# JeremyWesthead/deacon-server

Measured on AMD Instinct MI355X. Metric: Mbp/s filtered (k=31,w=15 vs panhuman-1-sized index), decisions bit-exact vs CPU, higher is better.
Workload: dtype u64

## Files before the change

### deacon-server_amd/_native.py

```python
import ctypes as C
import os
import re
import subprocess

_PKG = os.path.dirname(os.path.abspath(__file__))
LIB_PATH = os.environ.get("DCN_LIB_PATH") or os.path.join(_PKG, "lib", "libdeacon_hip.so")
HEADER_PATH = os.path.join(os.path.dirname(_PKG), "include", "deacon_hip.h")

DCN_OK = 0
DCN_ERR_ARG = -1
DCN_ERR_HIP = -2
DCN_ERR_NOMEM = -3
DCN_ERR_IO = -4
DCN_ERR_FORMAT = -5
DCN_ERR_CAPACITY = -6
DCN_ERR_INTERNAL = -7
N_STATS = 6
N_STAGES = 5
STAGE_NAMES = ("pack", "plan", "scan", "distinct", "finish")
STAT_NAMES = ("total_seqs", "filtered_seqs", "total_bp", "output_bp", "filtered_bp", "output_seq_counter")


class DeaconHipError(RuntimeError):
    def __init__(self, code, message):
        super().__init__(f"deacon_hip error {code}: {message}")
        self.code = code
        self.message = message


class Params(C.Structure):
    _fields_ = [
        ("abs_threshold", C.c_uint64),
        ("rel_threshold", C.c_double),
        ("prefix_length", C.c_uint64),
        ("deplete", C.c_uint32),
        ("reserved", C.c_uint32),
    ]


class LocateParams(C.Structure):
    _fields_ = [
        ("max_gap", C.c_uint32),
        ("min_hits", C.c_uint32),
        ("member_mask", C.c_uint32),
        ("reserved", C.c_uint32),
        ("prefix_length", C.c_uint64),
    ]


class TrackParams(C.Structure):
    _fields_ = [
        ("bin_bases", C.c_uint32),
        ("member_mask", C.c_uint32),
        ("depth_cap", C.c_uint32),
        ("reserved", C.c_uint32),
        ("prefix_length", C.c_uint64),
    ]


class TrackBin(C.Structure):
    _fields_ = [
        ("n_positions", C.c_uint32),
        ("n_keys", C.c_uint32),
        ("n_observed", C.c_uint32),
        ("max_depth", C.c_uint32),
        ("sum_depth", C.c_uint64),
    ]


class PlaceParams(C.Structure):
    _fields_ = [
        ("band_bases", C.c_uint32),
        ("min_votes", C.c_uint32),
        ("prefix_length", C.c_uint64),
        ("reserved", C.c_uint32 * 2),
    ]


class Placement(C.Structure):
    _fields_ = [
        ("record", C.c_uint32),
        ("reverse", C.c_uint32),
        ("votes", C.c_uint32),
        ("n_anchors", C.c_uint32),
        ("n_positions", C.c_uint32),
        ("read_start", C.c_uint32),
        ("read_end", C.c_uint32),
        ("reserved", C.c_uint32),
        ("ref_start", C.c_uint64),
        ("ref_end", C.c_uint64),
    ]


class PlaceSplitParams(C.Structure):
    _fields_ = [
        ("band_bases", C.c_uint32),
        ("min_votes", C.c_uint32),
        ("prefix_length", C.c_uint64),
        ("max_placements", C.c_uint32),
        ("reserved", C.c_uint32 * 3),
    ]


class SplitPlacement(C.Structure):
    _fields_ = Placement._fields_ + [
        ("rank", C.c_uint32),
        ("n_placed", C.c_uint32),
        ("rival_votes", C.c_uint32),
        ("mapq", C.c_uint32),
    ]


PLACE_SPLIT_MAX = 8


class PlacePairParams(C.Structure):
    _fields_ = [
        ("band_bases", C.c_uint32),
        ("min_votes", C.c_uint32),
        ("prefix_length", C.c_uint64),
        ("max_placements", C.c_uint32),
        ("max_insert", C.c_uint32),
        ("hist_bin_bases", C.c_uint32),
        ("reserved", C.c_uint32 * 3),
    ]


class PairPlacement(C.Structure):
    _fields_ = SplitPlacement._fields_ + [
        ("flags", C.c_uint32),
        ("pair_votes", C.c_uint32),
        ("tlen", C.c_int64),
    ]


PAIR_HIST_BINS = 256


def build(force=False, jobs=6):
    csrc = os.path.join(_PKG, "csrc")
    cmd = ["make", "-C", csrc, f"-j{jobs}"]
    if force:
        cmd.append("-B")
    subprocess.check_call(cmd, stdout=subprocess.DEVNULL)
    return LIB_PATH


def declared_symbols():
    text = open(HEADER_PATH).read()
    text = re.sub(r"/\*.*?\*/", "", text, flags=re.S)
    return sorted(set(re.findall(r"\b(dcn_[a-z0-9_]+)\s*\(", text)))


_u8p, _u32p, _u64p = C.POINTER(C.c_uint8), C.POINTER(C.c_uint32), C.POINTER(C.c_uint64)
_vp = C.c_void_p

_SIGNATURES = {
    "dcn_abi_version": (C.c_int, [_u32p, _u32p]),
    "dcn_version": (C.c_char_p, []),
    "dcn_last_error": (C.c_char_p, []),
    "dcn_device_count": (C.c_int, [C.POINTER(C.c_int)]),
    "dcn_set_minimizer_variant": (C.c_int, [C.c_uint32, C.c_uint32, C.c_uint32]),
    "dcn_get_minimizer_variant": (C.c_int, [_u32p, _u32p, _u32p]),
    "dcn_index_from_keys": (C.c_int, [_vp, C.c_uint64, C.c_uint8, C.c_uint8, C.c_int, C.POINTER(_vp)]),
    "dcn_index_from_file": (C.c_int, [C.c_char_p, C.c_int, C.POINTER(_vp)]),
    "dcn_index_build": (C.c_int, [_vp, _vp, C.c_uint32, C.c_uint8, C.c_uint8, C.c_float, C.c_uint64, C.c_int,
                                  C.POINTER(_vp)]),
    "dcn_index_keys": (C.c_int, [_vp, _vp, C.c_uint64, _u64p]),
    "dcn_index_union": (C.c_int, [C.POINTER(_vp), C.c_uint32, C.POINTER(_vp)]),
    "dcn_index_diff": (C.c_int, [_vp, _vp, C.POINTER(_vp)]),
    "dcn_index_intersect": (C.c_int, [C.POINTER(_vp), C.c_uint32, C.POINTER(_vp)]),
    "dcn_index_write_file": (C.c_int, [_vp, C.c_char_p]),
    "dcn_index_header": (C.c_int, [_vp, _u8p, _u8p, _u64p]),
    "dcn_index_contains": (C.c_int, [_vp, _vp, C.c_uint64, _vp]),
    "dcn_index_contains_device": (C.c_int, [_vp, _vp, C.c_uint64, _vp, _vp]),
    "dcn_index_probe_ceiling": (C.c_int, [_vp, _vp, C.c_uint64, C.c_uint32, C.POINTER(C.c_double)]),
    "dcn_index_destroy": (None, [_vp]),
    "dcn_ctx_create": (C.c_int, [_vp, C.c_uint64, C.c_uint32, C.POINTER(_vp)]),
    "dcn_ctx_destroy": (None, [_vp]),
    "dcn_filter_batch": (C.c_int, [_vp, _vp, _vp, _vp, C.c_uint32, C.POINTER(Params), _vp, _vp, _vp]),
    "dcn_filter_batch_submit": (C.c_int, [_vp, _vp, _vp, _vp, C.c_uint32, C.POINTER(Params), _vp, _vp, _vp, _u64p]),
    "dcn_filter_batch_wait": (C.c_int, [_vp, C.c_uint64]),
    "dcn_filter_batch_packed": (C.c_int, [_vp, _vp, _vp, _vp, _vp, C.c_uint32, C.POINTER(Params), _vp, _vp, _vp]),
    "dcn_filter_batch_packed_submit": (C.c_int, [_vp, _vp, _vp, _vp, _vp, C.c_uint32, C.POINTER(Params), _vp, _vp, _vp,
                                                 _u64p]),
    "dcn_pack_ascii": (C.c_int, [_vp, C.c_uint64, _vp, _vp, _u32p]),
    "dcn_stats_allreduce": (C.c_int, [C.POINTER(_vp), C.c_int, _u64p]),
    "dcn_comm_available": (C.c_int, []),
    "dcn_comm_unique_id": (C.c_int, [_vp]),
    "dcn_comm_create": (C.c_int, [_vp, C.c_int, C.c_int, C.c_int, C.POINTER(_vp)]),
    "dcn_stats_allreduce_rccl": (C.c_int, [_vp, C.POINTER(_vp), C.c_int, _u64p]),
    "dcn_comm_destroy": (None, [_vp]),
    "dcn_index_device": (C.c_int, [_vp, C.POINTER(C.c_int)]),
    "dcn_index_memory": (C.c_int, [_vp, C.POINTER(C.c_uint64)]),
    "dcn_index_clone": (C.c_int, [_vp, C.c_int, C.POINTER(_vp)]),
    "dcn_filter_batch_device": (C.c_int, [_vp, _vp, _vp, _vp, C.c_uint32, C.c_uint64, C.c_uint32,
                                          C.POINTER(Params), _vp, _vp, _vp]),
    "dcn_ctx_synchronize": (C.c_int, [_vp]),
    "dcn_ctx_reserve_records": (C.c_int, [_vp, C.c_uint64]),
    "dcn_ctx_stream": (_vp, [_vp]),
    "dcn_host_alloc": (C.c_int, [C.c_uint64, C.POINTER(_vp)]),
    "dcn_host_free": (None, [_vp]),
    "dcn_minimizer_hashes_batch": (C.c_int, [_vp, _vp, _vp, C.c_uint32, C.c_uint64, _vp, _vp, _vp, C.c_uint64]),
    "dcn_should_keep_hashes": (C.c_int, [_vp, _vp, _vp, C.c_uint32, C.POINTER(Params), _vp, _vp, _vp]),
    "dcn_ctx_stats": (C.c_int, [_vp, _u64p]),
    "dcn_ctx_reset_stats": (C.c_int, [_vp]),
    "dcn_ctx_set_profiling": (C.c_int, [_vp, C.c_int]),
    "dcn_ctx_profile": (C.c_int, [_vp, C.POINTER(C.c_double), _u64p]),
    "dcn_index_set_create": (C.c_int, [C.POINTER(_vp), C.c_uint32, C.POINTER(_vp)]),
    "dcn_index_set_destroy": (None, [_vp]),
    "dcn_index_set_info": (C.c_int, [_vp, _u32p, _u8p, _u8p, _u64p, _u64p]),
    "dcn_classify_batch": (C.c_int, [_vp, _vp, _vp, _vp, _vp, C.c_uint32, C.POINTER(Params), _vp, _vp, _vp]),
    "dcn_classify_batch_device": (C.c_int, [_vp, _vp, _vp, _vp, _vp, C.c_uint32, C.c_uint64, C.c_uint32,
                                            C.POINTER(Params), _vp, _vp, _vp]),
    "dcn_index_set_coverage_enable": (C.c_int, [_vp, C.c_int]),
    "dcn_index_set_coverage_reset": (C.c_int, [_vp]),
    "dcn_index_set_coverage": (C.c_int, [_vp, _vp, _vp]),
    "dcn_index_set_coverage_keys": (C.c_int, [_vp, C.c_uint32, _vp, C.c_uint64, _u64p]),
    "dcn_index_set_depth_enable": (C.c_int, [_vp, C.c_int]),
    "dcn_index_set_depth_reset": (C.c_int, [_vp]),
    "dcn_index_set_depth_stats": (C.c_int, [_vp, _vp, _vp, _vp]),
    "dcn_index_set_depth_hist": (C.c_int, [_vp, C.c_uint32, C.c_uint32, _vp]),
    "dcn_index_set_depth_keys": (C.c_int, [_vp, C.c_uint32, _vp, _vp, C.c_uint64, _u64p]),
    "dcn_index_set_select": (C.c_int, [_vp, C.c_uint32, C.c_uint32, C.c_uint32, C.c_uint32, C.c_uint32, _u64p,
                                       C.POINTER(_vp)]),
    "dcn_index_set_overlap": (C.c_int, [_vp, _vp, _vp, _vp]),
    "dcn_index_builder_create": (C.c_int, [C.c_uint8, C.c_uint8, C.c_float, C.c_uint64, C.c_int, C.POINTER(_vp)]),
    "dcn_index_builder_add": (C.c_int, [_vp, _vp, _vp, C.c_uint32]),
    "dcn_index_builder_info": (C.c_int, [_vp, _u64p, _u64p, _u64p, _u64p]),
    "dcn_index_builder_hist": (C.c_int, [_vp, C.c_uint32, _vp]),
    "dcn_index_builder_counts": (C.c_int, [_vp, _vp, _vp, C.c_uint64, _u64p]),
    "dcn_index_builder_finish": (C.c_int, [_vp, C.c_uint32, C.c_uint32, _u64p, C.POINTER(_vp)]),
    "dcn_index_builder_destroy": (None, [_vp]),
    "dcn_locate_batch": (C.c_int, [_vp, _vp, _vp, _vp, C.c_uint32, _vp, _vp, _vp, C.c_uint64]),
    "dcn_depth_track_batch": (C.c_int, [_vp, _vp, _vp, _vp, C.c_uint32, _vp, _vp, _vp, C.c_uint64]),
    "dcn_anchor_map_create": (C.c_int, [_vp, C.POINTER(_vp)]),
    "dcn_anchor_map_add": (C.c_int, [_vp, _vp, _vp, _vp, C.c_uint32, _u32p]),
    "dcn_anchor_map_info": (C.c_int, [_vp, _u32p, _u64p, _u64p, _u64p]),
    "dcn_anchor_map_anchors": (C.c_int, [_vp, _vp, _vp, _vp, C.c_uint64, _u64p]),
    "dcn_place_batch": (C.c_int, [_vp, _vp, _vp, _vp, C.c_uint32, _vp, _vp]),
    "dcn_place_split_batch": (C.c_int, [_vp, _vp, _vp, _vp, C.c_uint32, _vp, _vp, _vp, C.c_uint64, _vp]),
    "dcn_place_pair_batch": (C.c_int, [_vp, _vp, _vp, _vp, C.c_uint32, _vp, _vp, _vp]),
}

_lib = None
ABI = (1, 11)


def lib():
    global _lib
    if _lib is not None:
        return _lib
    if not os.path.exists(LIB_PATH):
        raise ImportError(
            f"{LIB_PATH} is missing: build it with __graft_entry__.build() "
            "(make -C deacon-server_amd/csrc). There is no CPU fallback.")
    L = C.CDLL(LIB_PATH)
    for name, (res, args) in _SIGNATURES.items():
        f = getattr(L, name)
        f.restype = res
        f.argtypes = args
    major, minor = C.c_uint32(), C.c_uint32()
    if L.dcn_abi_version(C.byref(major), C.byref(minor)) != 0 or (major.value, minor.value >= ABI[1]) != (ABI[0], True):
        raise ImportError(f"{LIB_PATH} has ABI {major.value}.{minor.value}; these bindings were written against {ABI[0]}.{ABI[1]} "
                          "(include/deacon_hip.h: DCN_ABI_MAJOR / DCN_ABI_MINOR)")
    _lib = L
    return L


def check(rc):
    if rc != DCN_OK:
        msg = lib().dcn_last_error()
        raise DeaconHipError(rc, msg.decode("utf-8", "replace") if msg else "")
    return rc
```

### deacon-server_amd/csrc/ctx.hip

```cpp
#include "dcn_ctx.h"
#include "dcn_host_pool.h"

#include <atomic>
#include <cstdlib>
#include <cstring>
#include <mutex>
#include <new>

using dcn_host::HostPool;

namespace dcn_impl {

int alloc_records(dcn_ctx *c, uint64_t n_records) {
    n_records = (n_records + 63) / 64 * 64;
    if (n_records > (1ull << 29)) return dcn_fail(DCN_ERR_CAPACITY, "more than 2^29 hit records in global sets per batch: use smaller batches");
    if (c->d_set_slots) hipFree(c->d_set_slots);
    c->d_set_slots = nullptr;
    c->rec_capacity = 0;
    DCN_TRY(dev_alloc(&c->d_set_slots, 4 * n_records + 64, "set_slots"));
    c->rec_capacity = n_records;
    return DCN_OK;
}

void free_slot_buffers(dcn_slot &sl) {
    if (sl.owns_buffers) {
        void *dev[] = {sl.d_ascii, sl.d_packed, sl.d_invmask, sl.d_offsets, sl.d_unit_id, sl.d_keep, sl.d_hits, sl.d_total};
        for (void *p : dev)
            if (p) hipFree(p);
    }
    if (sl.d_report) hipFree(sl.d_report);
    if (sl.d_off32) hipFree(sl.d_off32);
    if (sl.d_mask_pairs) hipFree(sl.d_mask_pairs);
    void *host[] = {sl.h_keep, sl.h_hits, sl.h_total, sl.h_report, sl.h_off32, sl.h_mask_pairs};
    for (void *p : host)
        if (p) hipHostFree(p);
    if (sl.done) hipEventDestroy(sl.done);
    for (hipEvent_t e : sl.ev_h2d) hipEventDestroy(e);
    for (hipEvent_t e : sl.ev_comp) hipEventDestroy(e);
    sl = dcn_slot();
}

static void free_ctx(dcn_ctx *c) {
    if (!c) return;
    hipSetDevice(c->device);
    if (c->stream) hipStreamSynchronize(c->stream);
    if (c->copy_stream) hipStreamSynchronize(c->copy_stream);
    if (c->d2h_stream) hipStreamSynchronize(c->d2h_stream);
    if (c->pack_stream) {
        hipStreamSynchronize(c->pack_stream);
        hipStreamDestroy(c->pack_stream);
    }
    for (int i = 0; i < 2; ++i) {
        if (c->pack_done[i]) hipEventDestroy(c->pack_done[i]);
        if (c->buf_free[i]) hipEventDestroy(c->buf_free[i]);
    }
    if (c->plan_done) hipEventDestroy(c->plan_done);
    if (c->d_packed_b) hipFree(c->d_packed_b);
    if (c->d_invmask_b) hipFree(c->d_invmask_b);
    if (c->d_pack_status) hipFree(c->d_pack_status);
    for (auto &sl : c->slots) free_slot_buffers(sl);
    void *dev[] = {c->d_ascii, c->d_offsets, c->d_unit_id, c->d_packed, c->d_invmask,
                   c->d_read_tiles, c->d_read_tile_first, c->d_unit_first_read, c->d_unit_tile_first, c->d_unit_tile_count, c->d_tiles,
                   c->d_keep, c->d_unit_state, c->d_hits, c->d_total, c->d_unit_scratch, c->d_caps,
                   c->d_set_off, c->d_tile_hits, c->d_pending, c->d_big, c->d_rec_hash, c->d_set_slots, c->d_status, c->d_report, c->d_dump_hash,
                   c->d_dump_pos, c->d_dump_count, c->d_dump_valid, c->d_tile_read_pos,
                   c->d_cls_big, c->d_cls_n_big, c->d_cls_match, c->d_cls_hits, c->d_cls_total,
                   c->d_loc_bits, c->d_loc_labels, c->d_loc_counts, c->d_loc_big, c->d_loc_n_big, c->d_loc_block_sums,
                   c->d_loc_seg_offsets, c->d_loc_segs, c->d_trk_bin_offsets, c->d_trk_piece_offsets, c->d_trk_bins,
                   c->d_plc_words, c->d_plc_abits, c->d_plc_big, c->d_plc_n_big, c->d_plc_out,
                   c->d_pls_rbits, c->d_pls_n_rounds, c->d_pls_read_counts, c->d_pls_counts, c->d_pls_block_sums,
                   c->d_pls_offsets, c->d_pls_rounds, c->d_pls_out, c->d_ppr_out, c->d_ppr_hist};
    for (void *p : dev)
        if (p && !((char *)p >= c->d_slab && (char *)p < c->d_slab + c->slab_bytes)) hipFree(p);
    if (c->d_slab) hipFree(c->d_slab);
    for (int i = 0; i < dcn_ctx::N_STAGE; ++i) {
        if (c->h_stage[i]) hipHostFree(c->h_stage[i]);
        if (c->stage_free[i]) hipEventDestroy(c->stage_free[i]);
    }
    for (int i = 0; i < dcn_ctx::N_EV; ++i) {
        if (c->ev_h2d[i]) hipEventDestroy(c->ev_h2d[i]);
        if (c->ev_comp[i]) hipEventDestroy(c->ev_comp[i]);
    }
    if (c->h_report) hipHostFree(c->h_report);
    for (int i = 0; i < dcn_ctx::PROF_RING; ++i)
        for (int j = 0; j <= DCN_N_STAGES; ++j)
            if (c->prof_ev[i][j]) hipEventDestroy(c->prof_ev[i][j]);
    if (c->copy_done) hipEventDestroy(c->copy_done);
    if (c->stream) hipStreamDestroy(c->stream);
    if (c->copy_stream) hipStreamDestroy(c->copy_stream);
    if (c->d2h_stream) hipStreamDestroy(c->d2h_stream);
    delete c;
}

static int prof_harvest(dcn_ctx *c, int only_slot = -1) {
    for (int i = 0; i < dcn_ctx::PROF_RING; ++i) {
        if (!c->prof_used[i] || (only_slot >= 0 && i != only_slot)) continue;
        const int first = c->prof_scan_only[i] ? DCN_STAGE_SCAN : 0, last = c->prof_scan_only[i] ? DCN_STAGE_SCAN : DCN_N_STAGES - 1;
        DCN_HIP(hipEventSynchronize(c->prof_ev[i][last + 1]));
        for (int j = first; j <= last; ++j) {
            float ms = 0.f;
            DCN_HIP(hipEventElapsedTime(&ms, c->prof_ev[i][j], c->prof_ev[i][j + 1]));
            c->prof_ms[j] += ms;
        }
        c->prof_batches++;
        c->prof_used[i] = false;
    }
    return DCN_OK;
}

int prof_begin(dcn_ctx *c, int *slot) {
    *slot = -1;
    if (!c->profiling) return DCN_OK;
    int i = c->prof_next;
    c->prof_next = (i + 1) % dcn_ctx::PROF_RING;
    if (c->prof_used[i]) DCN_TRY(prof_harvest(c, i));
    for (int j = 0; j <= DCN_N_STAGES; ++j)
        if (!c->prof_ev[i][j]) DCN_HIP(hipEventCreate(&c->prof_ev[i][j]));
    c->prof_scan_only[i] = c->profiling == 2;
    if (c->profiling == 1) DCN_HIP(hipEventRecord(c->prof_ev[i][0], c->stream));
    *slot = i;
    return DCN_OK;
}

int check_params(const dcn_params *p) {
    if (!p) return dcn_fail(DCN_ERR_ARG, "params is NULL");
    if (p->reserved != 0) return dcn_fail(DCN_ERR_ARG, "params.reserved must be 0");
    if (p->deplete > 1) return dcn_fail(DCN_ERR_ARG, "params.deplete must be 0 or 1");
    return DCN_OK;
}

static bool ensure_pack_ahead(dcn_ctx *c) {
    if (c->pack_ahead_state != 0) return c->pack_ahead_state > 0;
    c->pack_ahead_state = -1;
    if (!getenv("DCN_PACK_AHEAD") || getenv("DCN_NO_PACK_AHEAD")) return false;
    int prio_low = 0, prio_high = 0;
    (void)hipDeviceGetStreamPriorityRange(&prio_low, &prio_high);
    bool ok = hipStreamCreateWithPriority(&c->pack_stream, hipStreamNonBlocking, prio_high) == hipSuccess;
    ok = ok && hipEventCreateWithFlags(&c->plan_done, hipEventDisableTiming) == hipSuccess;
    for (int i = 0; ok && i < 2; ++i)
        ok = hipEventCreateWithFlags(&c->pack_done[i], hipEventDisableTiming) == hipSuccess &&
             hipEventCreateWithFlags(&c->buf_free[i], hipEventDisableTiming) == hipSuccess;
    ok = ok && hipMalloc((void **)&c->d_packed_b, packed_words(c->max_bases) * sizeof(uint32_t)) == hipSuccess &&
         hipMalloc((void **)&c->d_invmask_b, mask_words(c->max_bases) * sizeof(uint32_t)) == hipSuccess &&
         hipMalloc((void **)&c->d_pack_status, 2 * sizeof(dcn_status)) == hipSuccess;
    if (ok) {
        ok = hipMemset(c->d_packed_b, 0, packed_words(c->max_bases) * sizeof(uint32_t)) == hipSuccess &&
             hipMemset(c->d_invmask_b, 0, mask_words(c->max_bases) * sizeof(uint32_t)) == hipSuccess &&
             hipDeviceSynchronize() == hipSuccess;
    }
    if (!ok) {
        (void)hipGetLastError();
        if (c->d_packed_b) hipFree(c->d_packed_b);
        if (c->d_invmask_b) hipFree(c->d_invmask_b);
        if (c->d_pack_status) hipFree(c->d_pack_status);
        c->d_packed_b = c->d_invmask_b = nullptr;
        c->d_pack_status = nullptr;
        return false;
    }
    c->pack_ahead_state = 1;
    return true;
}

static dcn_scan_args scan_args(const dcn_ctx *c, const dcn_index *index, uint32_t *packed, uint32_t *invmask, uint64_t stream_bases);

int enqueue_batch(dcn_ctx *c, const BatchView &v, const dcn_params *params, bool pack_ahead) {
    hipStream_t st = c->stream;
    const dcn_index *idx = c->index;
    if (c->scratch_dirty) DCN_HIP(hipMemsetAsync(c->d_unit_scratch, 0, (uint64_t)c->max_reads * 4 * sizeof(uint32_t), st));
    c->scratch_dirty = true;
    DCN_HIP(hipMemsetAsync(c->d_status, 0, sizeof(dcn_status), st));

    int prof_slot = -1;
    DCN_TRY(prof_begin(c, &prof_slot));
    uint32_t *packed = v.d_packed + DCN_FRONT_PAD, *invmask = v.d_invmask + DCN_FRONT_PAD;
    int ahead_buf = -1;
    const uint32_t *newline_flag = nullptr;
    if (v.d_ascii && pack_ahead && c->profiling != 1 && ensure_pack_ahead(c)) {
        ahead_buf = c->pack_buf;
        c->pack_buf ^= 1;
        if (ahead_buf == 1) {
            packed = c->d_packed_b + DCN_FRONT_PAD;
            invmask = c->d_invmask_b + DCN_FRONT_PAD;
        }
        dcn_status *ps = c->d_pack_status + ahead_buf;
        DCN_HIP(hipStreamWaitEvent(c->pack_stream, c->buf_free[ahead_buf], 0));
        if (!getenv("DCN_PACK_AHEAD_EARLY")) DCN_HIP(hipStreamWaitEvent(c->pack_stream, c->plan_done, 0));
        DCN_HIP(hipMemsetAsync(ps, 0, sizeof(dcn_status), c->pack_stream));
        DCN_TRY(dcn_launch_pack_beside(v.d_ascii, v.b0, v.b1, packed, invmask, ps, c->pack_stream));
        DCN_HIP(hipEventRecord(c->pack_done[ahead_buf], c->pack_stream));
        DCN_HIP(hipStreamWaitEvent(st, c->pack_done[ahead_buf], 0));
        newline_flag = &ps->any_newline;
    } else if (v.d_ascii) {
        DCN_TRY(dcn_launch_pack(v.d_ascii, v.b0, v.b1, packed, invmask, c->d_status, st));
    }
    DCN_PROF_MARK(DCN_STAGE_PACK);

    const uint32_t n_reads = v.n_reads, n_units = v.n_units;
    dcn_plan_args pa = plan_args(c, idx, v.d_ascii, v.d_offsets, v.d_unit_id, n_reads, n_units, params->prefix_length);
    pa.unit_base = v.unit_base;
    pa.unit_state = c->d_unit_state;
    pa.unit_scratch = c->d_unit_scratch;
    pa.scratch_stride = c->max_reads;
    pa.newline_flag = newline_flag;
    pa.stream_bases = v.stream_bases;
    pa.check_offsets = 1;
    pa.max_tiles = c->max_tiles;
    DCN_TRY(dcn_launch_plan(pa, st));
    if (pack_ahead && c->pack_ahead_state == 1) DCN_HIP(hipEventRecord(c->plan_done, st));
    DCN_PROF_MARK(DCN_STAGE_PLAN);

    const UnitScratch us = unit_scratch(c);
    dcn_scan_args sa = scan_args(c, idx, packed, invmask, v.stream_bases);
    sa.unit_tile_first = c->d_unit_tile_first;
    sa.unit_tile_count = c->d_unit_tile_count;
    sa.abs_threshold = params->abs_threshold;
    sa.rel_threshold = params->rel_threshold;
    sa.deplete = params->deplete;
    sa.early_out_max_items = 0;
    static const bool no_early_out = getenv("DCN_NO_EARLY_OUT") != nullptr, no_early_out_pairs = getenv("DCN_NO_EARLY_OUT_PAIRS") != nullptr;
    if (!v.d_hits && !v.d_total && params->abs_threshold >= 1 && params->abs_threshold <= 4 && !no_early_out) {
        uint32_t lo = 0, hi = 65535;
        while (lo < hi) {
            uint32_t mid = (lo + hi + 1) / 2;
            if (dcn_required_hits(params->abs_threshold, params->rel_threshold, mid) == params->abs_threshold) lo = mid;
            else hi = mid - 1;
        }
        sa.early_out_max_items = lo;
        sa.early_out_pairs = no_early_out_pairs ? 0u : 1u;
    }
    sa.keep = v.d_keep;
    sa.hits = v.d_hits;
    sa.total = v.d_total;
    sa.unit_state = c->d_unit_state;
    sa.g_total = us.g_total;
    sa.g_hitcnt = us.g_hitcnt;
    sa.g_zero = us.g_zero;
    sa.rec_hash = c->d_rec_hash;
    sa.rec_shift = c->rec_shift;
    sa.tile_windows = c->tile_windows;
    sa.tile_hits = c->d_tile_hits;
    sa.pending = c->d_pending;
    sa.status = c->d_status;
    DCN_TRY(dcn_launch_scan(sa, tile_bound(c, n_reads, v.b1 - v.b0), false, st));
    DCN_PROF_MARK(DCN_STAGE_SCAN);

    const bool decisions_only = !v.d_hits && !v.d_total && !getenv("DCN_NO_EARLY_OUT");
    const dcn_distinct_args da = distinct_args(c, n_units, params, c->d_rec_hash, c->rec_shift, decisions_only ? us.g_total : nullptr);
    DCN_TRY(dcn_launch_distinct(da, st));
    DCN_PROF_MARK(DCN_STAGE_DISTINCT);

    const dcn_finish_args fa = finish_args(c, n_units, params, v.d_unit_id ? c->d_unit_first_read : nullptr, v.d_offsets, v.d_keep,
                                           v.d_hits, v.d_total, v.d_report);
    DCN_TRY(dcn_launch_finish(fa, st));
    c->scratch_dirty = false;
    if (pack_ahead && c->pack_ahead_state == 1) DCN_HIP(hipEventRecord(c->buf_free[ahead_buf >= 0 ? ahead_buf : 0], st));
    DCN_PROF_MARK(DCN_STAGE_FINISH);
    if (prof_slot >= 0) c->prof_used[prof_slot] = true;
    return DCN_OK;
}

int grow_run_slots(dcn_ctx *c) {
    if (c->rec_shift == 0) return DCN_OK;
    const bool in_slab = c->d_rec_hash && (char *)c->d_rec_hash >= c->d_slab && (char *)c->d_rec_hash < c->d_slab + c->slab_bytes;
    if (c->d_rec_hash && !in_slab) hipFree(c->d_rec_hash);
    c->d_rec_hash = nullptr;
    const uint32_t old_shift = c->rec_shift;
    c->rec_shift = 0;
    int rc = dev_alloc(&c->d_rec_hash, c->max_bases + 128, "rec_hash (one slot per window)");
    if (rc != DCN_OK) {
        c->rec_shift = old_shift;
        int rc2 = dev_alloc(&c->d_rec_hash, (c->max_bases >> old_shift) + 256, "rec_hash");
        return rc2 != DCN_OK ? rc2 : rc;
    }
    static std::atomic<bool> said{false};
    if (!said.exchange(true) && getenv("DCN_QUIET") == nullptr)
        std::fprintf(stderr, "deacon-hip: a unit's hits outgrew its run of the record array; this context now keeps one slot per window "
                             "(%.2f GB instead of %.2f GB of device memory)\n", (c->max_bases + 128) * 8e-9,
                     ((c->max_bases >> old_shift) + 256) * 8e-9);
    return DCN_OK;
}

int overflow_error(const dcn_ctx *c, uint64_t need) {
    return dcn_fail(DCN_ERR_CAPACITY, "hit-record scratch overflow: need " + std::to_string(need) +
                                          " records, have " + std::to_string(c->rec_capacity) +
                                          " (dcn_ctx_reserve_records)");
}

int sync_and_check(dcn_ctx *c, uint64_t *needed_records) {
    DCN_HIP(hipStreamSynchronize(c->stream));
    if (needed_records) *needed_records = 0;
    if (c->profiling) DCN_TRY(prof_harvest(c));
    if (!c->batch_pending) return DCN_OK;
    c->batch_pending = false;
    DCN_HIP(hipMemcpy(c->h_report, c->d_report, sizeof(dcn_batch_report), hipMemcpyDeviceToHost));
    if (c->h_report->bounds) {
        DCN_HIP(hipMemsetAsync(c->d_report, 0, offsetof(dcn_batch_report, stats), c->stream));
        return dcn_fail(DCN_ERR_INTERNAL, "scan kernel: index out of range in phase B (DCN_DEBUG_BOUNDS build)");
    }
    if (c->h_report->bad_offsets) {
        DCN_HIP(hipMemsetAsync(c->d_report, 0, offsetof(dcn_batch_report, stats), c->stream));
        return dcn_fail(DCN_ERR_ARG, "d_offsets of a batch since the last synchronize were not non-decreasing within [0, n_bases] when the "
                                     "device read them (were they written, and ordered before the context's stream, when "
                                     "dcn_filter_batch_device was called?): the outputs and counters of those batches are undefined");
    }
    if (c->h_report->overflow) {
        const uint64_t need = c->h_report->need;
        const bool runs = (c->h_report->overflow & 2u) != 0, sets = (c->h_report->overflow & 1u) != 0;
        DCN_HIP(hipMemsetAsync(c->d_report, 0, offsetof(dcn_batch_report, stats), c->stream));
        if (runs) DCN_TRY(grow_run_slots(c));
        if (needed_records) *needed_records = sets ? need : 0;
        if (!sets)
            return dcn_fail(DCN_ERR_CAPACITY, "a unit had more hits in one wave than its run of the record array holds; the context "
                                              "now keeps one slot per window: enqueue the batches since the last synchronize again");
        return overflow_error(c, need);
    }
    return DCN_OK;
}

bool is_pinned_host(const void *p) {
    if (!p) return false;
    hipPointerAttribute_t attr;
    if (hipPointerGetAttributes(&attr, p) != hipSuccess) {
        (void)hipGetLastError();
        return false;
    }
    return attr.type == hipMemoryTypeHost;
}

template <typename Fill>
static int staged_h2d_fill(dcn_ctx *c, void *d_dst, uint64_t bytes, uint64_t piece_align, Fill fill) {
    uint8_t *dst = (uint8_t *)d_dst;
    const uint64_t piece = c->stage_bytes / piece_align * piece_align;
    for (uint64_t off = 0; off < bytes; off += piece) {
        const int which = c->stage_next;
        c->stage_next = (which + 1) % dcn_ctx::N_STAGE;
        const uint64_t m = std::min<uint64_t>(piece, bytes - off);
        DCN_HIP(hipEventSynchronize(c->stage_free[which]));
        fill(c->h_stage[which], off, m);
        DCN_HIP(hipMemcpyAsync(dst + off, c->h_stage[which], m, hipMemcpyHostToDevice, c->copy_stream));
        DCN_HIP(hipEventRecord(c->stage_free[which], c->copy_stream));
    }
    return DCN_OK;
}

int staged_h2d(dcn_ctx *c, void *d_dst, const void *h_src, uint64_t bytes, int pinned) {
    if (bytes == 0) return DCN_OK;
    if (pinned < 0) pinned = is_pinned_host(h_src) ? 1 : 0;
    if (pinned) {
        DCN_HIP(hipMemcpyAsync(d_dst, h_src, bytes, hipMemcpyHostToDevice, c->copy_stream));
        return DCN_OK;
    }
    const uint8_t *src = (const uint8_t *)h_src;
    return staged_h2d_fill(c, d_dst, bytes, 64, [&](uint8_t *stage, uint64_t first, uint64_t n) {
        HostPool::get().copy(stage, src + first, n);
    });
}


int slots_busy(const dcn_ctx *c) {
    int n = 0;
    for (const auto &sl : c->slots) n += sl.busy ? 1 : 0;
    return n;
}

static std::mutex g_ctx_devices_mu;
static int g_ctx_per_device[64] = {0};
static void note_ctx_device(int device, int delta) {
    int n_devices = 0;
    {
        std::lock_guard<std::mutex> g(g_ctx_devices_mu);
        if (device >= 0 && device < 64) g_ctx_per_device[device] += delta;
        for (int d = 0; d < 64; ++d) n_devices += g_ctx_per_device[d] > 0;
    }
    if (delta > 0) HostPool::get().ensure_devices(n_devices);
}

int check_idle(const dcn_ctx *c) {
    if (slots_busy(c) || c->batch_pending) return dcn_fail(DCN_ERR_ARG, "batches are in flight on this context: wait for them first");
    return DCN_OK;
}

int check_ctx_matches(const dcn_ctx *c, const dcn_index *other, const char *noun) {
    const dcn_index *ix = c->index;
    const std::string n = noun;
    if (ix->k != other->k || ix->w != other->w)
        return dcn_fail(DCN_ERR_ARG, "the context's index (k=" + std::to_string((int)ix->k) + ", w=" + std::to_string((int)ix->w) +
                                         ") and " + n + " (k=" + std::to_string((int)other->k) + ", w=" + std::to_string((int)other->w) +
                                         ") differ");
    if (ix->device != other->device) return dcn_fail(DCN_ERR_ARG, "the context and " + n + " live on different devices");
    if (ix->variant != other->variant)
        return dcn_fail(DCN_ERR_ARG, "the context's index and " + n + " were created under different minimizer rules");
    return check_idle(c);
}

int check_device_batch(const dcn_ctx *c, uint32_t n_reads, uint64_t n_bases, uint32_t n_units, const uint32_t *d_unit_id) {
    if (n_reads > c->max_reads) return dcn_fail(DCN_ERR_CAPACITY, "n_reads exceeds the context's max_batch_reads");
    if (n_bases > c->max_bases) return dcn_fail(DCN_ERR_CAPACITY, "n_bases exceeds the context's max_batch_bases");
    if (n_units == 0 || n_units > n_reads || (!d_unit_id && n_units != n_reads))
        return dcn_fail(DCN_ERR_ARG, "n_units inconsistent with n_reads / d_unit_id");
    return DCN_OK;
}

int check_offsets_walk(const uint64_t *offsets, uint32_t n, const char *noun, const char *too_long) {
    if (offsets[0] != 0) return dcn_fail(DCN_ERR_ARG, std::string(noun) + "[0] must be 0");
    for (uint32_t r = 0; r < n; ++r) {
        if (offsets[r + 1] < offsets[r]) return dcn_fail(DCN_ERR_ARG, std::string(noun) + " must be non-decreasing");
        if (offsets[r + 1] - offsets[r] > 0xFFFFFFF0ull) return dcn_fail(DCN_ERR_ARG, too_long);
    }
    return DCN_OK;
}

int validate_host_batch(const dcn_ctx *c, const uint64_t *offsets, uint32_t n_reads) {
    if (n_reads > c->max_reads) return dcn_fail(DCN_ERR_CAPACITY, "n_reads exceeds the context's max_batch_reads");
    DCN_TRY(check_idle(c));
    DCN_TRY(check_offsets_walk(offsets, n_reads, "offsets", "read longer than 2^32 bases"));
    if (offsets[n_reads] > c->max_bases) return dcn_fail(DCN_ERR_CAPACITY, "batch exceeds the context's max_batch_bases");
    return DCN_OK;
}

int ensure_dump_buffers(dcn_ctx *c) {
    if (c->d_dump_hash) return DCN_OK;
    DCN_TRY(dev_alloc(&c->d_dump_hash, c->max_bases + 2, "dump_hash"));
    DCN_TRY(dev_alloc(&c->d_dump_pos, c->max_bases + 2, "dump_pos"));
    DCN_TRY(dev_alloc(&c->d_dump_valid, c->max_bases + 2, "dump_valid"));
    DCN_TRY(dev_alloc(&c->d_dump_count, c->max_tiles, "dump_count"));
    return DCN_OK;
}

int ensure_position_bitmap(dcn_ctx *c) {
    if (c->d_loc_bits) return DCN_OK;
    return dev_alloc(&c->d_loc_bits, (c->max_bases + 31) / 32 + 1, "position bitmap");
}

int ensure_position_words(dcn_ctx *c) {
    if (c->d_loc_labels) return DCN_OK;
    return dev_alloc(&c->d_loc_labels, c->max_bases + 2, "position words");
}

UnitScratch unit_scratch(const dcn_ctx *c) {
    uint32_t *const s = c->d_unit_scratch;
    const uint64_t n = c->max_reads;
    return {s, s + n, s + 2 * n, s + 3 * n};
}

int stage_done(dcn_ctx *c) {
    DCN_HIP(hipEventRecord(c->copy_done, c->copy_stream));
    DCN_HIP(hipStreamWaitEvent(c->stream, c->copy_done, 0));
    return DCN_OK;
}

int stage_batch(dcn_ctx *c, const uint8_t *bases, uint64_t n_bases, const uint64_t *offsets, uint32_t n_reads,
                const uint32_t *unit_id_or_null) {
    DCN_TRY(staged_h2d(c, c->d_ascii, bases, n_bases));
    DCN_TRY(staged_h2d(c, c->d_offsets, offsets, (uint64_t)(n_reads + 1) * sizeof(uint64_t)));
    if (unit_id_or_null) DCN_TRY(staged_h2d(c, c->d_unit_id, unit_id_or_null, (uint64_t)n_reads * sizeof(uint32_t)));
    return stage_done(c);
}

dcn_plan_args plan_args(const dcn_ctx *c, const dcn_index *index, const uint8_t *d_ascii, const uint64_t *d_offsets,
                        const uint32_t *d_unit_id, uint32_t n_reads, uint32_t n_units, uint64_t prefix_length) {
    dcn_plan_args pa = {};
    pa.ascii = d_ascii;
    pa.offsets = d_offsets;
    pa.unit_id = d_unit_id;
    pa.n_reads = n_reads;
    pa.n_units = n_units;
    pa.k = index->k;
    pa.w = index->w;
    pa.prefix_length = prefix_length;
    pa.tile_windows = c->tile_windows;
    pa.unit_first_read = c->d_unit_first_read;
    pa.unit_tile_first = c->d_unit_tile_first;
    pa.unit_tile_count = c->d_unit_tile_count;
    pa.tile_cursor = &c->d_status->n_tiles;
    pa.tiles = c->d_tiles;
    pa.status = c->d_status;
    return pa;
}

static dcn_scan_args scan_args(const dcn_ctx *c, const dcn_index *index, uint32_t *packed, uint32_t *invmask, uint64_t stream_bases) {
    dcn_scan_args sa;
    memset(&sa, 0, sizeof(sa));
    sa.packed = packed;
    sa.invmask = invmask;
    sa.tiles = c->d_tiles;
    sa.n_tiles = &c->d_status->n_tiles;
    sa.table = index->view();
    sa.k = index->k;
    sa.variant = index->variant;
    sa.w = index->w;
    sa.stream_bases = stream_bases;
    sa.status = c->d_status;
    return sa;
}

dcn_scan_args dump_scan_args(const dcn_ctx *c, const dcn_index *index, uint64_t n_bases) {
    dcn_scan_args sa = scan_args(c, index, c->d_packed + DCN_FRONT_PAD, c->d_invmask + DCN_FRONT_PAD, n_bases);
    sa.dump_hash = c->d_dump_hash;
    sa.dump_pos = c->d_dump_pos;
    sa.dump_valid = c->d_dump_valid;
    sa.dump_count = c->d_dump_count;
    return sa;
}

uint32_t tile_bound(const dcn_ctx *c, uint32_t n_reads, uint64_t n_bases) {
    return (uint32_t)std::min<uint64_t>((uint64_t)n_reads + n_bases / c->tile_windows + 1, c->max_tiles);
}

dcn_dump_view dump_view(const dcn_ctx *c, uint32_t max_tiles, uint64_t n_bases) {
    dcn_dump_view v = {};
    v.tiles = c->d_tiles;
    v.n_tiles = &c->d_status->n_tiles;
    v.hash = c->d_dump_hash;
    v.valid = c->d_dump_valid;
    v.pos = c->d_dump_pos;
    v.count = c->d_dump_count;
    v.max_tiles = max_tiles;
    v.n_bases = n_bases;
    return v;
}

int dump_front_end(dcn_ctx *c, const dcn_index *index, const uint8_t *d_ascii, const uint64_t *d_offsets,
                   const uint32_t *d_unit_id, uint32_t n_reads, uint32_t n_units, uint64_t n_bases, uint64_t prefix_length,
                   bool plan_checks_offsets, int *prof_slot_out, dcn_dump_view *view) {
    hipStream_t st = c->stream;
    int prof_slot = -1;
    DCN_TRY(prof_begin(c, &prof_slot));
    *prof_slot_out = prof_slot;
    DCN_TRY(dcn_launch_pack(d_ascii, 0, n_bases, c->d_packed + DCN_FRONT_PAD, c->d_invmask + DCN_FRONT_PAD, c->d_status, st));
    DCN_PROF_MARK(DCN_STAGE_PACK);
    dcn_plan_args pa = plan_args(c, index, d_ascii, d_offsets, d_unit_id, n_reads, n_units, prefix_length);
    pa.read_tiles = c->d_read_tiles;
    pa.read_tile_first = c->d_read_tile_first;
    if (plan_checks_offsets) {
        pa.stream_bases = n_bases;
        pa.check_offsets = 1;
        pa.max_tiles = c->max_tiles;
    }
    DCN_TRY(dcn_launch_plan(pa, st));
    DCN_PROF_MARK(DCN_STAGE_PLAN);
    dcn_scan_args sa = dump_scan_args(c, index, n_bases);
    sa.dump_abs = 1;
    const uint32_t max_tiles = tile_bound(c, n_reads, n_bases);
    DCN_TRY(dcn_launch_scan(sa, max_tiles, true, st));
    DCN_PROF_MARK(DCN_STAGE_SCAN);
    *view = dump_view(c, max_tiles, n_bases);
    return DCN_OK;
}

int record_run_end(dcn_ctx *c, int prof_slot) {
    if (prof_slot >= 0) c->prof_used[prof_slot] = true;
    if (c->pack_ahead_state == 1) {
        DCN_HIP(hipEventRecord(c->plan_done, c->stream));
        for (int i = 0; i < 2; ++i) DCN_HIP(hipEventRecord(c->buf_free[i], c->stream));
    }
    return DCN_OK;
}

int finish_run(dcn_ctx *c, int prof_slot) {
    DCN_TRY(record_run_end(c, prof_slot));
    return sync_and_check(c, nullptr);
}

dcn_distinct_args distinct_args(const dcn_ctx *c, uint32_t n_units, const dcn_params *params, const uint64_t *rec_hash,
                                uint32_t rec_shift, uint32_t *g_total_or_null) {
    const UnitScratch us = unit_scratch(c);
    dcn_distinct_args da = {};
    da.tiles = c->d_tiles;
    da.n_tiles = &c->d_status->n_tiles;
    da.unit_tile_first = c->d_unit_tile_first;
    da.unit_tile_count = c->d_unit_tile_count;
    da.unit_state = c->d_unit_state;
    da.tile_hits = c->d_tile_hits;
    da.pending = c->d_pending;
    da.rec_hash = rec_hash;
    da.rec_shift = rec_shift;
    da.g_hitcnt = us.g_hitcnt;
    da.g_distinct = us.g_distinct;
    da.set_off = c->d_set_off;
    da.set_slots = c->d_set_slots;
    da.set_capacity = 4 * c->rec_capacity + 64;
    da.n_units = n_units;
    da.status = c->d_status;
    da.caps = c->d_caps;
    da.big = c->d_big;
    da.g_total = g_total_or_null;
    da.abs_threshold = params->abs_threshold;
    da.rel_threshold = params->rel_threshold;
    return da;
}

dcn_finish_args finish_args(const dcn_ctx *c, uint32_t n_units, const dcn_params *params, const uint32_t *unit_first_read,
                            const uint64_t *offsets, uint8_t *keep, uint32_t *hits, uint32_t *total, dcn_batch_report *report) {
    const UnitScratch us = unit_scratch(c);
    dcn_finish_args fa = {};
    fa.n_units = n_units;
    fa.unit_first_read = unit_first_read;
    fa.offsets = offsets;
    fa.unit_state = c->d_unit_state;
    fa.g_total = us.g_total;
    fa.g_hitcnt = us.g_hitcnt;
    fa.g_distinct = us.g_distinct;
    fa.g_zero = us.g_zero;
    fa.abs_threshold = params->abs_threshold;
    fa.rel_threshold = params->rel_threshold;
    fa.deplete = params->deplete;
    fa.keep = keep;
    fa.hits = hits;
    fa.total = total;
    fa.report = report;
    fa.status = c->d_status;
    return fa;
}

}

using namespace dcn_impl;

extern "C" int dcn_ctx_create(const dcn_index *index, uint64_t max_batch_bases, uint32_t max_batch_reads,
                              dcn_ctx **out) {
    if (!out) return dcn_fail(DCN_ERR_ARG, "out is NULL");
    *out = nullptr;
    if (!index) return dcn_fail(DCN_ERR_ARG, "index is NULL");
    if (max_batch_bases == 0 || max_batch_reads == 0) return dcn_fail(DCN_ERR_ARG, "batch limits must be > 0");
    if (max_batch_reads > 0xFFFFFF00u) return dcn_fail(DCN_ERR_ARG, "max_batch_reads too large");
    dcn_ctx *c = new (std::nothrow) dcn_ctx();
    if (!c) return dcn_fail(DCN_ERR_NOMEM, "host allocation failed");
    c->index = index;
    c->device = index->device;
    c->max_bases = max_batch_bases;
    c->max_reads = max_batch_reads;
    if (const char *tw = getenv("DCN_TILE_WINDOWS")) {
        long v = strtol(tw, nullptr, 10);
        if (v >= 16 && v <= (long)DCN_MAX_TILE_WINDOWS) c->tile_windows = (uint32_t)v;
    }
    uint64_t mt = (uint64_t)max_batch_reads + max_batch_bases / c->tile_windows + 1;
    if (mt > 0xFFFFFF00ull) {
        delete c;
        return dcn_fail(DCN_ERR_ARG, "batch limits imply more than 2^32 tiles");
    }
    c->max_tiles = (uint32_t)mt;
    c->chunk_bases = 64ull << 20;
    if (const char *cb = getenv("DCN_CHUNK_BASES")) {
        long long v = atoll(cb);
        if (v >= 1024) c->chunk_bases = (uint64_t)v;
    }
    int rc = DCN_OK;
    auto fail = [&](int code) {
        free_ctx(c);
        return code;
    };
    if (hipSetDevice(c->device) != hipSuccess) return fail(dcn_fail(DCN_ERR_HIP, "hipSetDevice failed"));
    bool ok = hipStreamCreateWithFlags(&c->stream, hipStreamNonBlocking) == hipSuccess &&
              hipStreamCreateWithFlags(&c->copy_stream, hipStreamNonBlocking) == hipSuccess &&
              hipStreamCreateWithFlags(&c->d2h_stream, hipStreamNonBlocking) == hipSuccess &&
              hipEventCreateWithFlags(&c->copy_done, hipEventDisableTiming) == hipSuccess;
    for (int i = 0; ok && i < dcn_ctx::N_STAGE; ++i)
        ok = hipEventCreateWithFlags(&c->stage_free[i], hipEventDisableTiming) == hipSuccess;
    for (int i = 0; ok && i < dcn_ctx::N_EV; ++i)
        ok = hipEventCreateWithFlags(&c->ev_h2d[i], hipEventDisableTiming) == hipSuccess &&
             hipEventCreateWithFlags(&c->ev_comp[i], hipEventDisableTiming) == hipSuccess;
    if (!ok) return fail(dcn_fail(DCN_ERR_HIP, "stream/event creation failed"));
    c->rec_shift = 2;
    if (index->w <= 7) c->rec_shift = 0;
    if (const char *rs = getenv("DCN_REC_SHIFT")) c->rec_shift = (uint32_t)std::min(3, std::max(0, atoi(rs)));
    uint64_t MR = max_batch_reads;
    const bool slab = getenv("DCN_CTX_SLAB") != nullptr;
    uint64_t slab_off = 0;
    for (int pass = slab ? 0 : 1; pass < 2; ++pass) {
        if (slab && pass == 1) {
            c->slab_bytes = slab_off;
            if (hipMalloc((void **)&c->d_slab, c->slab_bytes) != hipSuccess) {
                c->d_slab = nullptr;
                c->slab_bytes = 0;
                return fail(dcn_fail(DCN_ERR_NOMEM, "hipMalloc of the context slab failed"));
            }
            slab_off = 0;
        }
#define A(ptr, count, what)                                                                                   \
    if (slab) {                                                                                               \
        if (pass == 1) c->ptr = reinterpret_cast<decltype(c->ptr)>(c->d_slab + slab_off);                     \
        slab_off += (std::max<uint64_t>((count), 1) * sizeof(*c->ptr) + (2u << 20) - 1) / (2u << 20) * (2u << 20); \
    } else if ((rc = dev_alloc(&c->ptr, (count), what)) != DCN_OK)                                            \
        return fail(rc)
    A(d_ascii, max_batch_bases + 64, "ascii");
    A(d_offsets, MR + 1, "offsets");
    A(d_unit_id, MR, "unit_id");
    A(d_packed, packed_words(max_batch_bases), "packed");
    A(d_invmask, mask_words(max_batch_bases), "invmask");
    A(d_read_tiles, MR, "read_tiles");
    A(d_read_tile_first, MR + 1, "read_tile_first");
    A(d_unit_first_read, MR + 1, "unit_first_read");
    A(d_unit_tile_first, MR + 1, "unit_tile_first");
    A(d_unit_tile_count, MR + 1, "unit_tile_count");
    A(d_tiles, mt, "tiles");
    A(d_keep, MR, "keep");
    A(d_unit_state, MR, "unit_state");
    A(d_hits, MR, "hits");
    A(d_total, MR, "total");
    A(d_unit_scratch, MR * 4, "unit_scratch");
    A(d_caps, MR, "caps");
    A(d_set_off, MR + 1, "set_off");
    A(d_tile_hits, mt, "tile_hits");
    A(d_pending, MR, "pending");
    A(d_big, MR + mt / 64 + 1, "big");
    A(d_rec_hash, (max_batch_bases >> c->rec_shift) + 256, "rec_hash");
    A(d_status, 1, "status");
    A(d_report, 1, "report");
#undef A
    }
    uint64_t recs = std::min<uint64_t>(std::max<uint64_t>(max_batch_bases / 16, 1u << 16), 1ull << 29);
    if (const char *rc_env = getenv("DCN_RECORD_CAPACITY")) recs = std::min<uint64_t>(std::max<uint64_t>(strtoull(rc_env, nullptr, 10), 64), 1ull << 29);
    if ((rc = alloc_records(c, recs)) != DCN_OK) return fail(rc);
    c->stage_bytes = std::min<uint64_t>(std::max<uint64_t>(max_batch_bases + 64, 4096), 32ull << 20);
    if (const char *sb = getenv("DCN_STAGE_BYTES"))
        c->stage_bytes = std::min<uint64_t>(std::max<uint64_t>(strtoull(sb, nullptr, 10), 4096), 32ull << 20);
    for (int i = 0; i < dcn_ctx::N_STAGE; ++i)
        if (hipHostMalloc((void **)&c->h_stage[i], c->stage_bytes, hipHostMallocDefault) != hipSuccess)
            return fail(dcn_fail(DCN_ERR_NOMEM, "pinned staging allocation failed"));
    if (hipHostMalloc((void **)&c->h_report, sizeof(dcn_batch_report), hipHostMallocDefault) != hipSuccess)
        return fail(dcn_fail(DCN_ERR_NOMEM, "pinned status allocation failed"));
    if (hipMemset(c->d_packed, 0, packed_words(max_batch_bases) * sizeof(uint32_t)) != hipSuccess ||
        hipMemset(c->d_invmask, 0, mask_words(max_batch_bases) * sizeof(uint32_t)) != hipSuccess ||
        hipMemset(c->d_status, 0, sizeof(dcn_status)) != hipSuccess ||
        hipMemset(c->d_unit_scratch, 0, (uint64_t)max_batch_reads * 4 * sizeof(uint32_t)) != hipSuccess ||
        hipMemset(c->d_report, 0, sizeof(dcn_batch_report)) != hipSuccess ||
        hipDeviceSynchronize() != hipSuccess)
        return fail(dcn_fail(DCN_ERR_HIP, "hipMemset failed"));
    note_ctx_device(c->device, +1);
    *out = c;
    return DCN_OK;
}

extern "C" void dcn_ctx_destroy(dcn_ctx *ctx) {
    if (ctx) note_ctx_device(ctx->device, -1);
    free_ctx(ctx);
}

extern "C" void *dcn_ctx_stream(dcn_ctx *ctx) { return ctx ? (void *)ctx->stream : nullptr; }

extern "C" int dcn_ctx_reserve_records(dcn_ctx *ctx, uint64_t n_records) {
    if (!ctx) return dcn_fail(DCN_ERR_ARG, "ctx is NULL");
    if (slots_busy(ctx)) return dcn_fail(DCN_ERR_ARG, "host batches are in flight: wait for them first");
    DCN_HIP(hipSetDevice(ctx->device));
    DCN_HIP(hipStreamSynchronize(ctx->stream));
    if (n_records <= ctx->rec_capacity) return DCN_OK;
    return alloc_records(ctx, n_records);
}

extern "C" int dcn_ctx_synchronize(dcn_ctx *ctx) {
    if (!ctx) return dcn_fail(DCN_ERR_ARG, "ctx is NULL");
    DCN_HIP(hipSetDevice(ctx->device));
    return sync_and_check(ctx, nullptr);
}

extern "C" int dcn_filter_batch_device(dcn_ctx *ctx, const uint8_t *d_bases, const uint64_t *d_offsets,
                                       const uint32_t *d_unit_id, uint32_t n_reads, uint64_t n_bases,
                                       uint32_t n_units, const dcn_params *params, uint8_t *d_keep, uint32_t *d_hits,
                                       uint32_t *d_total) {
    if (!ctx) return dcn_fail(DCN_ERR_ARG, "ctx is NULL");
    DCN_TRY(check_params(params));
    if (n_reads == 0) return DCN_OK;
    if (!d_bases || !d_offsets || !d_keep) return dcn_fail(DCN_ERR_ARG, "d_bases/d_offsets/d_keep is NULL");
    DCN_TRY(check_device_batch(ctx, n_reads, n_bases, n_units, d_unit_id));
    if (ctx->slots[0].busy) return dcn_fail(DCN_ERR_ARG, "a host batch is in flight on this context: wait for it first");
    DCN_HIP(hipSetDevice(ctx->device));
    BatchView v;
    v.d_ascii = d_bases;
    v.d_packed = ctx->d_packed;
    v.d_invmask = ctx->d_invmask;
    v.d_offsets = d_offsets;
    v.d_unit_id = d_unit_id;
    v.n_reads = n_reads;
    v.n_units = n_units;
    v.b0 = 0;
    v.b1 = n_bases;
    v.stream_bases = n_bases;
    v.d_keep = d_keep;
    v.d_hits = d_hits;
    v.d_total = d_total;
    v.d_report = ctx->d_report;
    DCN_TRY(enqueue_batch(ctx, v, params, true));
    ctx->batch_pending = true;
    return DCN_OK;
}

extern "C" int dcn_ctx_set_profiling(dcn_ctx *ctx, int enable) {
    if (!ctx) return dcn_fail(DCN_ERR_ARG, "ctx is NULL");
    DCN_HIP(hipSetDevice(ctx->device));
    DCN_HIP(hipStreamSynchronize(ctx->stream));
    for (int i = 0; i < dcn_ctx::PROF_RING; ++i) ctx->prof_used[i] = false;
    for (int j = 0; j < DCN_N_STAGES; ++j) ctx->prof_ms[j] = 0.0;
    ctx->prof_batches = 0;
    ctx->profiling = enable == 2 ? 2 : (enable != 0 ? 1 : 0);
    return DCN_OK;
}

extern "C" int dcn_ctx_profile(dcn_ctx *ctx, double stage_ms[DCN_N_STAGES], uint64_t *n_batches) {
    if (!ctx || !stage_ms) return dcn_fail(DCN_ERR_ARG, "ctx/stage_ms is NULL");
    if (ctx->profiling) {
        DCN_HIP(hipSetDevice(ctx->device));
        DCN_TRY(prof_harvest(ctx));
    }
    for (int j = 0; j < DCN_N_STAGES; ++j) stage_ms[j] = ctx->prof_ms[j];
    if (n_batches) *n_batches = ctx->prof_batches;
    return DCN_OK;
}

extern "C" int dcn_ctx_stats(dcn_ctx *ctx, uint64_t counters[DCN_N_STATS]) {
    if (!ctx || !counters) return dcn_fail(DCN_ERR_ARG, "ctx/counters is NULL");
    DCN_HIP(hipSetDevice(ctx->device));
    DCN_HIP(hipStreamSynchronize(ctx->stream));
    DCN_HIP(hipMemcpy(ctx->h_report, ctx->d_report, sizeof(dcn_batch_report), hipMemcpyDeviceToHost));
    for (int i = 0; i < DCN_N_STATS; ++i) counters[i] = ctx->h_report->stats[i] + ctx->host_stats[i];
    return DCN_OK;
}

extern "C" int dcn_ctx_reset_stats(dcn_ctx *ctx) {
    if (!ctx) return dcn_fail(DCN_ERR_ARG, "ctx is NULL");
    DCN_HIP(hipSetDevice(ctx->device));
    DCN_HIP(hipStreamSynchronize(ctx->stream));
    DCN_HIP(hipMemsetAsync(ctx->d_report->stats, 0, sizeof(unsigned long long) * DCN_N_STATS, ctx->stream));
    DCN_HIP(hipStreamSynchronize(ctx->stream));
    for (int i = 0; i < DCN_N_STATS; ++i) ctx->host_stats[i] = 0;
    return DCN_OK;
}

extern "C" int dcn_stats_allreduce(dcn_ctx *const *ctxs, int n_ctx, uint64_t counters[DCN_N_STATS]) {
    if (!counters || (n_ctx > 0 && !ctxs) || n_ctx < 0) return dcn_fail(DCN_ERR_ARG, "ctxs/counters is NULL");
    for (int i = 0; i < DCN_N_STATS; ++i) counters[i] = 0;
    for (int j = 0; j < n_ctx; ++j) {
        uint64_t one[DCN_N_STATS];
        DCN_TRY(dcn_ctx_stats(ctxs[j], one));
        for (int i = 0; i < DCN_N_STATS; ++i) counters[i] += one[i];
    }
    return DCN_OK;
}
```

### deacon-server_amd/csrc/dcn_ctx.h

```cpp
#pragma once

#include "dcn_dump_sweep.h"
#include "dcn_internal.h"
#include "dcn_plan.h"

#include <algorithm>
#include <functional>
#include <vector>

struct dcn_split_round;

struct dcn_mask_range {
    uint64_t g0 = 0, g1 = 0, pairs_off = 0;
    uint32_t n = 0;
};

struct dcn_chunk {
    uint32_t r0 = 0, r1 = 0, u0 = 0, u1 = 0;
    uint64_t b0 = 0, b1 = 0;
    uint64_t max_len = 0;
    std::vector<dcn_mask_range> mask_ranges;
};

struct dcn_slot {
    bool allocated = false, busy = false, owns_buffers = false;
    uint64_t ticket = 0;
    uint8_t *d_ascii = nullptr;
    uint32_t *d_packed = nullptr, *d_invmask = nullptr;
    uint64_t *d_offsets = nullptr;
    uint32_t *d_off32 = nullptr, *h_off32 = nullptr;
    bool off32 = false;
    bool lean = false;
    uint2 *d_mask_pairs = nullptr, *h_mask_pairs = nullptr;
    uint64_t mask_pairs_cap = 0, mask_pairs_used = 0;
    uint32_t *d_unit_id = nullptr;
    uint8_t *d_keep = nullptr;
    uint32_t *d_hits = nullptr, *d_total = nullptr;
    dcn_batch_report *d_report = nullptr;
    uint8_t *h_keep = nullptr;
    uint32_t *h_hits = nullptr, *h_total = nullptr;
    dcn_batch_report *h_report = nullptr;
    hipEvent_t done = nullptr;
    std::vector<hipEvent_t> ev_h2d, ev_comp;
    dcn_params params = {};
    bool device_pack = false;
    bool has_units = false, counts = false;
    uint32_t n_reads = 0, n_units = 0;
    uint64_t n_bases = 0;
    uint8_t *u_keep = nullptr;
    uint32_t *u_hits = nullptr, *u_total = nullptr;
    bool keep_direct = false, hits_direct = false, total_direct = false;
    std::vector<dcn_chunk> chunks;
};

struct dcn_ctx {
    const dcn_index *index = nullptr;
    int device = 0;
    hipStream_t stream = nullptr, copy_stream = nullptr, d2h_stream = nullptr;
    hipStream_t pack_stream = nullptr;
    uint32_t *d_packed_b = nullptr, *d_invmask_b = nullptr;
    dcn_status *d_pack_status = nullptr;
    hipEvent_t pack_done[2] = {}, buf_free[2] = {}, plan_done = nullptr;
    int pack_buf = 0, pack_ahead_state = 0;
    static constexpr int N_STAGE = 3, N_EV = 8, N_SLOTS = 2;
    hipEvent_t copy_done = nullptr, stage_free[N_STAGE] = {};
    hipEvent_t ev_h2d[N_EV] = {}, ev_comp[N_EV] = {};
    int ev_next = 0, stage_next = 0;
    uint64_t max_bases = 0;
    uint32_t max_reads = 0;
    uint32_t tile_windows = 256;
    uint32_t max_tiles = 0;
    uint64_t chunk_bases = 0;
    uint8_t *d_ascii = nullptr;
    uint64_t *d_offsets = nullptr;
    uint32_t *d_unit_id = nullptr;
    uint32_t *d_packed = nullptr, *d_invmask = nullptr;
    uint32_t *d_read_tiles = nullptr, *d_read_tile_first = nullptr;
    uint32_t *d_unit_first_read = nullptr, *d_unit_tile_first = nullptr, *d_unit_tile_count = nullptr;
    dcn_tile *d_tiles = nullptr;
    uint8_t *d_keep = nullptr, *d_unit_state = nullptr;
    uint32_t *d_hits = nullptr, *d_total = nullptr;
    uint32_t *d_unit_scratch = nullptr;
    bool scratch_dirty = false;
    uint32_t *d_caps = nullptr, *d_set_off = nullptr;
    uint64_t *d_rec_hash = nullptr;
    uint32_t rec_shift = 0;
    char *d_slab = nullptr;
    uint64_t slab_bytes = 0;
    uint32_t *d_tile_hits = nullptr, *d_pending = nullptr;
    uint2 *d_big = nullptr;
    uint64_t rec_capacity = 0;
    uint64_t *d_set_slots = nullptr;
    dcn_status *d_status = nullptr;
    dcn_batch_report *d_report = nullptr;
    dcn_batch_report *h_report = nullptr;
    uint64_t host_stats[DCN_N_STATS] = {};
    uint8_t *h_stage[N_STAGE] = {};
    uint64_t stage_bytes = 0;
    dcn_slot slots[N_SLOTS];
    uint64_t next_ticket = 1;
    uint64_t *d_dump_hash = nullptr;
    uint32_t *d_dump_pos = nullptr, *d_dump_count = nullptr, *d_tile_read_pos = nullptr;
    uint8_t *d_dump_valid = nullptr;
    uint32_t *d_cls_big = nullptr, *d_cls_n_big = nullptr;
    uint32_t *d_cls_match = nullptr, *d_cls_hits = nullptr, *d_cls_total = nullptr;
    uint32_t cls_hits_members = 0;
    uint32_t *d_loc_bits = nullptr, *d_loc_labels = nullptr;
    uint32_t *d_loc_counts = nullptr, *d_loc_big = nullptr, *d_loc_n_big = nullptr;
    unsigned long long *d_loc_block_sums = nullptr;
    uint64_t *d_loc_seg_offsets = nullptr;
    dcn_segment *d_loc_segs = nullptr;
    uint64_t loc_seg_cap = 0;
    uint64_t *d_trk_bin_offsets = nullptr, *d_trk_piece_offsets = nullptr;
    dcn_track_bin *d_trk_bins = nullptr;
    uint64_t trk_bin_cap = 0;
    uint64_t *d_plc_words = nullptr;
    uint32_t *d_plc_abits = nullptr, *d_plc_big = nullptr, *d_plc_n_big = nullptr;
    dcn_placement *d_plc_out = nullptr;
    uint32_t *d_pls_rbits = nullptr, *d_pls_n_rounds = nullptr, *d_pls_read_counts = nullptr, *d_pls_counts = nullptr;
    unsigned long long *d_pls_block_sums = nullptr;
    uint64_t *d_pls_offsets = nullptr;
    dcn_split_round *d_pls_rounds = nullptr;
    dcn_split_placement *d_pls_out = nullptr;
    uint64_t pls_round_cap = 0, pls_out_cap = 0;
    dcn_pair_placement *d_ppr_out = nullptr;
    unsigned long long *d_ppr_hist = nullptr;
    bool batch_pending = false;
    bool lean = false;
    static constexpr int PROF_RING = 64;
    int profiling = 0;
    hipEvent_t prof_ev[PROF_RING][DCN_N_STAGES + 1] = {};
    bool prof_used[PROF_RING] = {}, prof_scan_only[PROF_RING] = {};
    int prof_next = 0;
    double prof_ms[DCN_N_STAGES] = {};
    uint64_t prof_batches = 0;
};

bool dcn_host_pack_is_wide();
bool dcn_host_pack_groups(const uint8_t *ascii, uint64_t n_bases, uint64_t g0, uint64_t g1, uint32_t *packed,
                          uint32_t *mask);

#define DCN_TRY(expr)              \
    do {                           \
        int _rc = (expr);          \
        if (_rc != DCN_OK) return _rc; \
    } while (0)

#define DCN_PROF_MARK(stage)                                                                                      \
    do {                                                                                                          \
        if (prof_slot >= 0 && (c->profiling == 1 || (stage) == DCN_STAGE_PLAN || (stage) == DCN_STAGE_SCAN))      \
            DCN_HIP(hipEventRecord(c->prof_ev[prof_slot][(stage) + 1], st));                                      \
    } while (0)

#pragma GCC visibility push(hidden)
namespace dcn_impl {

template <typename T>
int dev_alloc(T **p, uint64_t count, const char *what) {
    hipError_t e = hipMalloc((void **)p, std::max<uint64_t>(count, 1) * sizeof(T));
    if (e != hipSuccess) {
        *p = nullptr;
        return dcn_fail(DCN_ERR_NOMEM, std::string("hipMalloc ") + what + ": " + hipGetErrorString(e));
    }
    return DCN_OK;
}

template <typename T>
int dev_alloc_zeroed(T **p, uint64_t count, const char *what) {
    *p = nullptr;
    T *d = nullptr;
    hipError_t e = hipMalloc((void **)&d, count * sizeof(T));
    if (e == hipSuccess) e = hipMemset(d, 0, count * sizeof(T));
    if (e == hipSuccess) e = hipDeviceSynchronize();
    if (e != hipSuccess) {
        if (d) hipFree(d);
        return dcn_hip_fail(e, what);
    }
    *p = d;
    return DCN_OK;
}

struct DevMem {
    void *p = nullptr;
    ~DevMem() {
        if (p) hipFree(p);
    }
    int alloc(uint64_t bytes, bool zero, const char *what) {
        hipError_t e = hipMalloc(&p, std::max<uint64_t>(bytes, 8));
        if (e == hipSuccess && zero) e = hipMemset(p, 0, std::max<uint64_t>(bytes, 8));
        return e == hipSuccess ? DCN_OK : dcn_hip_fail(e, what);
    }
    int clear(const char *what) {
        const hipError_t e = hipMemset(p, 0, 8);
        return e == hipSuccess ? DCN_OK : dcn_hip_fail(e, what);
    }
    int read(void *h, uint64_t bytes, const char *what) const {
        const hipError_t e = hipMemcpy(h, p, bytes, hipMemcpyDeviceToHost);
        return e == hipSuccess ? DCN_OK : dcn_hip_fail(e, what);
    }
    template <typename T>
    T *as() const {
        return (T *)p;
    }
};

inline int read_count(const DevMem &d_n, const char *what, unsigned long long *n) { return d_n.read(n, sizeof(*n), what); }

inline uint64_t packed_words(uint64_t max_bases) { return DCN_FRONT_PAD + 2 * ((max_bases + 31) / 32) + DCN_TAIL_PAD; }
inline uint64_t mask_words(uint64_t max_bases) { return DCN_FRONT_PAD + (max_bases + 31) / 32 + DCN_TAIL_PAD; }

struct BatchView {
    const uint8_t *d_ascii = nullptr;
    uint32_t *d_packed = nullptr, *d_invmask = nullptr;
    const uint64_t *d_offsets = nullptr;
    const uint32_t *d_unit_id = nullptr;
    uint32_t unit_base = 0;
    uint32_t n_reads = 0, n_units = 0;
    uint64_t b0 = 0, b1 = 0;
    uint64_t stream_bases = 0;
    uint8_t *d_keep = nullptr;
    uint32_t *d_hits = nullptr, *d_total = nullptr;
    dcn_batch_report *d_report = nullptr;
};

int same_params(const dcn_index *a, const dcn_index *b);
int check_kw(uint8_t k, uint8_t w);

constexpr uint32_t DCN_BUILD_MAX_PIECES = 1u << 16;
uint64_t build_chunk_bases();
using build_sweep_fn = std::function<int(uint64_t nb, bool continues)>;
struct build_times {
    double front_end_s = 0, staging_s = 0, growth_s = 0, finish_s = 0, finish_table_s = 0;
};
double build_now();
int build_timing_begin(dcn_ctx *c);
int build_times_print(const char *which, dcn_ctx *c, const build_times &t);
int build_run_chunks(dcn_ctx *c, const dcn_index *idx, const uint8_t *bases, const uint64_t *offsets, uint32_t n_seqs,
                     uint64_t chunk_bases, const build_sweep_fn &sweep, build_times *times = nullptr);

int check_set(const dcn_index *set);

int alloc_records(dcn_ctx *c, uint64_t n_records);
void free_slot_buffers(dcn_slot &sl);
int prof_begin(dcn_ctx *c, int *slot);
int check_params(const dcn_params *p);
int enqueue_batch(dcn_ctx *c, const BatchView &v, const dcn_params *params, bool pack_ahead = false);
int grow_run_slots(dcn_ctx *c);
int overflow_error(const dcn_ctx *c, uint64_t need);
int sync_and_check(dcn_ctx *c, uint64_t *needed_records);
bool is_pinned_host(const void *p);
int staged_h2d(dcn_ctx *c, void *d_dst, const void *h_src, uint64_t bytes, int pinned = -1);
int slots_busy(const dcn_ctx *c);

int check_idle(const dcn_ctx *c);
int check_ctx_matches(const dcn_ctx *c, const dcn_index *other, const char *noun);
int check_device_batch(const dcn_ctx *c, uint32_t n_reads, uint64_t n_bases, uint32_t n_units, const uint32_t *d_unit_id);
int check_offsets_walk(const uint64_t *offsets, uint32_t n, const char *noun, const char *too_long);
int validate_host_batch(const dcn_ctx *c, const uint64_t *offsets, uint32_t n_reads);

int ensure_dump_buffers(dcn_ctx *c);
int ensure_position_bitmap(dcn_ctx *c);
int ensure_position_words(dcn_ctx *c);
struct UnitScratch {
    uint32_t *g_total, *g_hitcnt, *g_distinct, *g_zero;
};
UnitScratch unit_scratch(const dcn_ctx *c);
int stage_batch(dcn_ctx *c, const uint8_t *bases, uint64_t n_bases, const uint64_t *offsets, uint32_t n_reads,
                const uint32_t *unit_id_or_null);
int stage_done(dcn_ctx *c);
dcn_plan_args plan_args(const dcn_ctx *c, const dcn_index *index, const uint8_t *d_ascii, const uint64_t *d_offsets,
                        const uint32_t *d_unit_id, uint32_t n_reads, uint32_t n_units, uint64_t prefix_length);
dcn_scan_args dump_scan_args(const dcn_ctx *c, const dcn_index *index, uint64_t n_bases);
uint32_t tile_bound(const dcn_ctx *c, uint32_t n_reads, uint64_t n_bases);
dcn_dump_view dump_view(const dcn_ctx *c, uint32_t max_tiles, uint64_t n_bases);

int dump_front_end(dcn_ctx *c, const dcn_index *index, const uint8_t *d_ascii, const uint64_t *d_offsets,
                   const uint32_t *d_unit_id, uint32_t n_reads, uint32_t n_units, uint64_t n_bases, uint64_t prefix_length,
                   bool plan_checks_offsets, int *prof_slot, dcn_dump_view *view);
int record_run_end(dcn_ctx *c, int prof_slot);
int finish_run(dcn_ctx *c, int prof_slot);
dcn_distinct_args distinct_args(const dcn_ctx *c, uint32_t n_units, const dcn_params *params, const uint64_t *rec_hash,
                                uint32_t rec_shift, uint32_t *g_total_or_null);
dcn_finish_args finish_args(const dcn_ctx *c, uint32_t n_units, const dcn_params *params, const uint32_t *unit_first_read,
                            const uint64_t *offsets, uint8_t *keep, uint32_t *hits, uint32_t *total, dcn_batch_report *report);

}
#pragma GCC visibility pop
```

### deacon-server_amd/csrc/dcn_internal.h

```cpp
#pragma once

#include <hip/hip_runtime.h>
#include <stdint.h>

#include <string>

#include "../../include/deacon_hip.h"

void dcn_set_error(const std::string &msg);
int dcn_fail(int code, const std::string &msg);

#define DCN_HIP(expr)                                                                              \
    do {                                                                                           \
        hipError_t _e = (expr);                                                                    \
        if (_e != hipSuccess)                                                                      \
            return dcn_fail(_e == hipErrorOutOfMemory ? DCN_ERR_NOMEM : DCN_ERR_HIP,               \
                            std::string(#expr) + ": " + hipGetErrorString(_e));                    \
    } while (0)

inline int dcn_hip_fail(hipError_t e, const char *what) {
    return dcn_fail(e == hipErrorOutOfMemory ? DCN_ERR_NOMEM : DCN_ERR_HIP, std::string(what) + ": " + hipGetErrorString(e));
}

template <typename F>
int dcn_device_tally(uint64_t count, unsigned long long *h, const char *what, F sweep) {
    unsigned long long *d = nullptr;
    hipError_t e = hipMalloc((void **)&d, count * sizeof(unsigned long long));
    if (e != hipSuccess) return dcn_hip_fail(e, what);
    int rc = DCN_OK;
    e = hipMemset(d, 0, count * sizeof(unsigned long long));
    if (e == hipSuccess) rc = sweep(d);
    if (e == hipSuccess && rc == DCN_OK) e = hipMemcpy(h, d, count * sizeof(unsigned long long), hipMemcpyDeviceToHost);
    hipFree(d);
    if (rc != DCN_OK) return rc;
    return e == hipSuccess ? DCN_OK : dcn_hip_fail(e, what);
}

void dcn_host_parallel_copy(void *dst, const void *src, size_t n);

#ifndef DCN_GROUP_SLOTS
#define DCN_GROUP_SLOTS 2
#endif
constexpr int DCN_SLOTS_PER_KEY = DCN_GROUP_SLOTS == 2 ? 4 : 2;
constexpr int DCN_SLOTS_PER_KEY_ROOMY = 2 * DCN_SLOTS_PER_KEY;
constexpr uint64_t DCN_ROOMY_MAX_GROUPS = 1ull << 31;

struct dcn_table_view {
    const uint64_t *slots;
    uint32_t group_shift;
    uint32_t group_mask;
    uint32_t has_zero;
};

constexpr uint32_t DCN_VARIANT_DEFAULT = (1u << 16) | (16u << 8) | 0u;
uint32_t dcn_current_variant();

struct dcn_index {
    uint32_t variant = dcn_current_variant();
    int device = 0;
    uint8_t k = 0, w = 0;
    uint64_t n_keys = 0;
    uint64_t n_groups = 0;
    uint64_t *d_slots = nullptr;
    bool has_zero = false;
    uint32_t *d_labels = nullptr;
    uint32_t n_members = 0;
    uint32_t zero_label = 0;
    uint32_t *d_cov = nullptr;
    uint64_t cov_words = 0;
    uint64_t cov_keys[32] = {};
    uint32_t *d_depth = nullptr;
    uint64_t depth_words = 0;
    uint64_t *d_anchor = nullptr;
    uint32_t anchor_records = 0;
    dcn_table_view view() const {
        dcn_table_view v;
        v.slots = d_slots;
        uint32_t bits = 0;
        while ((1ull << bits) < n_groups) ++bits;
        v.group_shift = 32 - bits;
        v.group_mask = (uint32_t)(n_groups - 1);
        v.has_zero = has_zero ? 1u : 0u;
        return v;
    }
};

__host__ __device__ inline uint32_t dcn_group_of(uint64_t key, uint32_t group_shift, uint32_t group_mask) {
    uint32_t lo = (uint32_t)key, hi = (uint32_t)(key >> 32);
    uint32_t x = (lo ^ ((hi << 15) | (hi >> 17))) * 0x9E3779B1u;
    return group_shift >= 32 ? 0u : ((x >> group_shift) & group_mask);
}

constexpr int DCN_WAVE = 64;
constexpr int DCN_LCAP = 40;
constexpr uint32_t DCN_FRONT_PAD = 64;
constexpr uint32_t DCN_TAIL_PAD = 256;
constexpr uint32_t DCN_MAX_TILE_WINDOWS = 2048;

struct dcn_tile {
    uint64_t scan_start;
    uint32_t unit;
    uint32_t nwf;
    __host__ __device__ uint32_t n_windows() const { return nwf & 0x3FFFFFFFu; }
    __host__ __device__ uint32_t carry() const { return nwf >> 31; }
    __host__ __device__ bool whole_unit() const { return (nwf >> 30) & 1u; }
};
static_assert(sizeof(dcn_tile) == 16, "tile descriptor");

struct dcn_status {
    uint32_t rec_overflow;
    uint32_t n_tiles;
    uint32_t any_records;
    uint32_t n_big;
    uint32_t any_scattered;
    uint32_t n_pending;
    uint32_t any_newline;
    uint32_t bounds;
    uint32_t run_overflow;
    uint32_t bad_offsets;
    unsigned long long set_cursor;
};

struct dcn_batch_report {
    uint32_t overflow;
    uint32_t bounds;
    uint32_t bad_offsets;
    uint32_t reserved_;
    unsigned long long need;
    unsigned long long stats[DCN_N_STATS];
};

struct dcn_scan_args {
    const uint32_t *packed;
    const uint32_t *invmask;
    const dcn_tile *tiles;
    const uint32_t *tile_read_pos;
    const uint32_t *n_tiles;
    uint32_t *unit_tile_first;
    uint32_t *unit_tile_count;
    dcn_table_view table;
    uint32_t k, w;
    uint64_t stream_bases;
    uint64_t abs_threshold;
    double rel_threshold;
    uint32_t deplete;
    uint32_t early_out_max_items;
    uint32_t early_out_pairs;
    uint8_t *keep;
    uint32_t *hits, *total;
    uint8_t *unit_state;
    uint32_t *g_total;
    uint32_t *g_hitcnt;
    uint32_t *g_zero;
    uint64_t *rec_hash;
    uint32_t rec_shift;
    uint32_t tile_windows;
    uint32_t *tile_hits;
    uint32_t *pending;
    dcn_status *status;
    uint64_t *dump_hash;
    uint32_t *dump_pos;
    uint8_t *dump_valid;
    uint32_t *dump_count;
    uint32_t dump_abs;
    uint32_t variant;
    uint32_t nt_rot;
    uint32_t cmp_mask;
    uint32_t nt_combine_xor;
};

int dcn_launch_pack(const uint8_t *d_ascii, uint64_t base_begin, uint64_t base_end, uint32_t *d_packed,
                    uint32_t *d_invmask, dcn_status *status, hipStream_t stream, bool index_side = false,
                    uint32_t block_threads = 256);
int dcn_launch_pack_beside(const uint8_t *d_ascii, uint64_t base_begin, uint64_t base_end, uint32_t *d_packed, uint32_t *d_invmask,
                           dcn_status *status, hipStream_t stream);
int dcn_launch_scan(const dcn_scan_args &args, uint32_t max_tiles, bool dump, hipStream_t stream);

int dcn_table_build(dcn_index *idx, const uint64_t *host_keys, uint64_t n);
int dcn_table_contains(const dcn_index *idx, const uint64_t *host_keys, uint64_t n, uint8_t *out);
int dcn_table_contains_device(const dcn_index *idx, const uint64_t *d_keys, uint64_t n, uint8_t *d_out,
                              hipStream_t stream);
int dcn_table_probe_ceiling(const dcn_index *idx, const uint64_t *d_keys, uint64_t n, uint32_t reps, double *best,
                            hipStream_t stream);
int dcn_table_insert_varint9(dcn_index *idx, const uint64_t *d_raw, uint64_t n, unsigned long long *d_new,
                             uint32_t *d_zero, uint32_t *d_bad, hipStream_t stream);
uint64_t dcn_table_groups_for(uint64_t n_keys);
int dcn_table_alloc(dcn_index *idx, uint64_t n_keys_capacity);
int dcn_table_reserve(dcn_index *idx, uint64_t n_keys_capacity);
int dcn_table_insert_dump(dcn_index *idx, const uint64_t *d_hash, const uint8_t *d_valid, const uint32_t *d_abs_pos,
                          uint64_t n_slots, const uint8_t *d_ascii, float entropy_threshold, hipStream_t stream);
int dcn_table_count_valid(const uint8_t *d_valid, uint64_t n, uint64_t *count, hipStream_t stream);
int dcn_table_export(const dcn_index *idx, uint64_t *host_out, uint64_t capacity, uint64_t *n_out);
int dcn_table_merge(dcn_index *dst, const dcn_index *src, const dcn_index *minus);
hipError_t dcn_table_malloc(uint64_t **p, uint64_t bytes);
int dcn_table_clone_by_keys(const dcn_index *src, dcn_index *dst);


__host__ __device__ inline uint64_t dcn_required_hits(uint64_t abs_threshold, double rel_threshold,
                                                      uint64_t total) {
    uint64_t rel_required = 0;
    if (total != 0) {
        double r = round(rel_threshold * (double)total);
        if (!(r > 0.0)) rel_required = 0;
        else if (r >= 18446744073709551616.0) rel_required = ~0ull;
        else rel_required = (uint64_t)r;
        if (rel_required < 1) rel_required = 1;
    }
    return abs_threshold > rel_required ? abs_threshold : rel_required;
}

__host__ __device__ inline bool dcn_decide(uint64_t hits, uint64_t total, uint64_t abs_threshold,
                                           double rel_threshold, uint32_t deplete) {
    uint64_t required = dcn_required_hits(abs_threshold, rel_threshold, total);
    return deplete ? (hits < required) : (hits >= required);
}
```

### deacon-server_amd/csrc/plan.hip

```cpp
#include "dcn_internal.h"
#include "dcn_plan.h"
#include "dcn_probe.h"

#include <algorithm>

namespace {

__device__ inline uint32_t effective_windows(const uint8_t *ascii, uint64_t off, uint64_t len, uint64_t prefix,
                                             uint32_t k, uint32_t l) {
    if (len < k) return 0;
    uint64_t n = (prefix > 0 && len > prefix) ? prefix : len;
    if (ascii && n > 0 && ascii[off + n - 1] == '\n') n -= 1;
    return n >= l ? (uint32_t)(n - l + 1) : 0;
}

__device__ inline void write_tile(const dcn_plan_args &a, uint32_t first, uint32_t j, uint64_t off, uint32_t nwin,
                                  uint32_t unit, bool whole_unit = false) {
    uint32_t wstart = j * a.tile_windows;
    uint32_t carry = j > 0 ? 1u : 0u;
    if (a.check_offsets && first + j >= a.max_tiles) {
        a.status->bad_offsets = 1;
        return;
    }
    dcn_tile t;
    t.scan_start = off + wstart - carry;
    t.unit = unit;
    t.nwf = min(a.tile_windows, nwin - wstart) | (carry << 31) | (whole_unit ? 1u << 30 : 0u);
    a.tiles[first + j] = t;
    if (a.tile_read_pos) a.tile_read_pos[first + j] = wstart - carry;
}

template <uint32_t PLAN_CH>
__global__ __launch_bounds__(256) void plan_kernel(dcn_plan_args a) {
    constexpr uint32_t PLAN_READS = 256 * PLAN_CH;
    constexpr uint32_t OWN = 4;
    __shared__ uint32_t s_tiles[PLAN_READS];
    __shared__ uint32_t s_first[PLAN_READS];
    __shared__ uint32_t s_wave[4], s_wave1[4];
    __shared__ uint32_t s_base;
    __shared__ uint32_t long_reads[PLAN_READS];
    __shared__ uint32_t n_long;
    const uint32_t tid = threadIdx.x;
    const uint32_t block_first = blockIdx.x * PLAN_READS;
    const uint32_t block_end = min(a.n_reads, block_first + PLAN_READS);
    if (tid == 0) n_long = 0;
    const uint8_t *ascii = (a.ascii && (a.newline_flag ? *a.newline_flag : a.status->any_newline)) ? a.ascii : nullptr;
    uint32_t nwin[PLAN_CH], nt[PLAN_CH], loc[PLAN_CH];
    const bool two_classes = a.unit_id == nullptr;
    uint32_t carry = 0;
    uint32_t carry1 = 0;
#pragma unroll
    for (uint32_t c = 0; c < PLAN_CH; ++c) {
        const uint32_t r = block_first + c * 256 + tid;
        nwin[c] = 0;
        nt[c] = 0;
        if (r < a.n_reads) {
            uint64_t off = a.offsets[r], end = a.offsets[r + 1];
            if (a.check_offsets && (end < off || end > a.stream_bases)) {
                a.status->bad_offsets = 1;
                end = off = 0;
            }
            nwin[c] = effective_windows(ascii, off, end - off, a.prefix_length, a.k, a.k + a.w - 1);
            nt[c] = (nwin[c] + a.tile_windows - 1) / a.tile_windows;
        }
        const bool single = two_classes && nt[c] == 1;
        const uint32_t own = single ? 0u : nt[c], own1 = single ? 1u : 0u;
        uint32_t inc = own, inc1 = own1;
#pragma unroll
        for (int d = 1; d < 64; d <<= 1) {
            uint32_t o = __shfl_up(inc, d, 64), o1 = __shfl_up(inc1, d, 64);
            if ((int)(tid & 63) >= d) {
                inc += o;
                inc1 += o1;
            }
        }
        __syncthreads();
        if ((tid & 63) == 63) {
            s_wave[tid >> 6] = inc;
            s_wave1[tid >> 6] = inc1;
        }
        __syncthreads();
        uint32_t wave_base = 0, chunk_total = 0, wave_base1 = 0, chunk_total1 = 0;
#pragma unroll
        for (uint32_t i = 0; i < 4; ++i) {
            if (i < (tid >> 6)) {
                wave_base += s_wave[i];
                wave_base1 += s_wave1[i];
            }
            chunk_total += s_wave[i];
            chunk_total1 += s_wave1[i];
        }
        loc[c] = single ? (0x80000000u | (carry1 + wave_base1 + inc1 - 1u)) : (carry + wave_base + inc - own);
        carry += chunk_total;
        carry1 += chunk_total1;
        s_tiles[c * 256 + tid] = nt[c];
    }
    if (tid == 0) s_base = (carry + carry1) ? atomicAdd(a.tile_cursor, carry + carry1) : 0u;
    __syncthreads();
#pragma unroll
    for (uint32_t c = 0; c < PLAN_CH; ++c) {
        if (loc[c] & 0x80000000u) loc[c] = carry + (loc[c] & 0x7FFFFFFFu);
        s_first[c * 256 + tid] = s_base + loc[c];
    }
    __syncthreads();
#pragma unroll
    for (uint32_t c = 0; c < PLAN_CH; ++c) {
        const uint32_t r = block_first + c * 256 + tid;
        if (r >= a.n_reads) continue;
        const uint32_t first = s_base + loc[c];
        if (a.read_tiles) {
            a.read_tiles[r] = nt[c];
            a.read_tile_first[r] = first;
        }
        uint32_t u = r;
        bool unit_head = true;
        if (a.unit_id) {
            u = a.unit_id[r] - a.unit_base;
            if (a.check_offsets) {
                const uint32_t prev = r ? a.unit_id[r - 1] : a.unit_base - 1u;
                if (u >= a.n_units || a.unit_id[r] - prev > 1u || (r == a.n_reads - 1 && u != a.n_units - 1)) {
                    a.status->bad_offsets = 1;
                    if (u >= a.n_units) u = 0;
                }
            }
            unit_head = r == 0 || a.unit_id[r - 1] != a.unit_id[r];
            if (unit_head) a.unit_first_read[u] = r;
            if (r == a.n_reads - 1) a.unit_first_read[a.n_units] = a.n_reads;
        }
        if (unit_head) {
            uint32_t count = nt[c];
            if (a.unit_id) {
                uint32_t q = r + 1;
                while (q < a.n_reads && a.unit_id[q] - a.unit_base == u) {
                    if (q >= block_end) {
                        count = 0xFFFFFFFFu;
                        break;
                    }
                    count += s_tiles[q - block_first];
                    ++q;
                }
            }
            if (a.unit_id || nt[c] != 1) {
                a.unit_tile_first[u] = first;
                a.unit_tile_count[u] = count;
            }
            if (a.unit_state) a.unit_state[u] = 0;
        }
        const uint64_t off = a.offsets[r];
        for (uint32_t j = 0; j < min(nt[c], OWN); ++j) write_tile(a, first, j, off, nwin[c], u, !a.unit_id && nt[c] == 1);
        if (nt[c] > OWN) long_reads[atomicAdd(&n_long, 1u)] = c * 256 + tid;
    }
    __syncthreads();
    for (uint32_t q = 0; q < n_long; ++q) {
        const uint32_t li = long_reads[q], lr = block_first + li;
        const uint32_t lnt = s_tiles[li], lfirst = s_first[li];
        uint32_t lu = a.unit_id ? a.unit_id[lr] - a.unit_base : lr;
        if (a.check_offsets && lu >= a.n_units) lu = 0;
        const uint64_t loff = a.offsets[lr];
        const uint32_t lnwin = effective_windows(ascii, loff, a.offsets[lr + 1] - loff, a.prefix_length, a.k, a.k + a.w - 1);
        for (uint32_t j = OWN + tid; j < lnt; j += blockDim.x) write_tile(a, lfirst, j, loff, lnwin, lu);
    }
}

#ifndef DCN_LDS_SET_LOG2
#define DCN_LDS_SET_LOG2 11
#endif
constexpr uint32_t DCN_LDS_SET_SLOTS = 1u << DCN_LDS_SET_LOG2;
constexpr uint32_t DCN_LDS_SET_MAX = DCN_LDS_SET_SLOTS * 7 / 10 - 33;
constexpr uint32_t DCN_LDS_WALK_MAX_TILES = 1024;

__device__ inline uint32_t set_slot_of(uint64_t h, uint32_t cap) {
    uint32_t lo = (uint32_t)h, hi = (uint32_t)(h >> 32);
    return ((lo ^ ((hi << 13) | (hi >> 19))) * 0x85EBCA6Bu) & (cap - 1);
}

__global__ __launch_bounds__(64) void unit_distinct_kernel(dcn_distinct_args a) {
    __shared__ unsigned long long set[DCN_LDS_SET_SLOTS];
    if (a.status->run_overflow) return;
    const uint32_t NP = a.status->n_pending;
    const uint32_t lane = threadIdx.x;
    uint32_t nu = 0, nfirst = 0, ncount = 0, nH = 0, ntot = 0;
    auto fetch = [&](uint32_t i) {
        if (i < NP) {
            nu = a.pending[i];
            nfirst = a.unit_tile_first[nu];
            ncount = a.unit_tile_count[nu];
            nH = a.g_hitcnt[nu];
            ntot = a.g_total ? a.g_total[nu] : 0u;
        }
    };
    fetch(blockIdx.x);
    for (uint32_t i = blockIdx.x; i < NP; i += gridDim.x) {
        const uint32_t u = nu, first = nfirst, count = ncount, H = nH, tot = ntot;
        fetch(i + gridDim.x);
        if (H == 0) {
            if (lane == 0) a.caps[u] = 0;
            continue;
        }
        uint32_t enough = 0xFFFFFFFFu;
        if (a.g_total) {
            const uint64_t req = dcn_required_hits(a.abs_threshold, a.rel_threshold, tot);
            if ((uint64_t)H < req) {
                if (lane == 0) {
                    a.g_distinct[u] = 0;
                    a.caps[u] = 0;
                }
                continue;
            }
            enough = req > 0xFFFFFFFEull ? 0xFFFFFFFEu : (uint32_t)req;
        }
        const uint32_t Hset = H < enough ? H : enough;
        if (count == 0xFFFFFFFFu || Hset > DCN_LDS_SET_MAX || count > DCN_LDS_WALK_MAX_TILES) {
            uint32_t cap = 64;
            while (cap < 2u * H && cap < (1u << 31)) cap <<= 1;
            unsigned long long off = 0;
            if (lane == 0) off = atomicAdd(&a.status->set_cursor, (unsigned long long)cap);
            off = (unsigned long long)__shfl((long long)off, 0, 64);
            const bool fits = off + cap <= a.set_capacity;
            const uint32_t n_items = count == 0xFFFFFFFFu ? 0u : (count + 63) / 64;
            uint32_t item0 = 0;
            if (lane == 0) {
                a.set_off[u] = (uint32_t)off;
                a.caps[u] = fits ? cap : 0u;
                if (!fits) a.status->rec_overflow = 1;
                else if (n_items) item0 = atomicAdd(&a.status->n_big, n_items);
                if (fits && count == 0xFFFFFFFFu) a.status->any_scattered = 1;
            }
            item0 = __shfl(item0, 0, 64);
            if (fits)
                for (uint32_t q = lane; q < n_items; q += 64) a.big[item0 + q] = make_uint2(u, 64 * q);
            continue;
        }
        const uint32_t most = enough == 0xFFFFFFFFu ? Hset : (Hset + 256u < H ? Hset + 256u : H);
        uint32_t cap = 64;
        while (cap < 2u * most && cap < DCN_LDS_SET_SLOTS) cap <<= 1;
        auto tile_run = [&](uint32_t t, uint32_t &n, uint64_t &slot0) {
            n = 0;
            slot0 = 0;
            if (t < count) {
                n = a.tile_hits[first + t];
                const dcn_tile tl = a.tiles[first + t];
                slot0 = (tl.scan_start + tl.carry()) >> a.rec_shift;
            }
        };
        uint32_t n;
        uint64_t slot0;
        tile_run(lane, n, slot0);
        for (uint32_t q = lane; q < cap; q += 64) set[q] = 0;
        __syncthreads();
        uint32_t distinct = 0;
        for (uint32_t t0 = 0; t0 < count && distinct < enough; t0 += 64) {
            if (t0) tile_run(t0 + lane, n, slot0);
            unsigned long long runs = __ballot(n != 0);
            while (runs && distinct < enough) {
                const int r = __ffsll((long long)runs) - 1;
                runs &= runs - 1;
                const uint32_t rn = __shfl(n, r, 64);
                const uint64_t rs = (uint64_t)__shfl((long long)slot0, r, 64);
                for (uint32_t j0 = 0; j0 < rn && distinct < enough; j0 += 256) {
                    uint64_t h[4];
#pragma unroll
                    for (int q = 0; q < 4; ++q) {
                        const uint32_t j = j0 + q * 64 + lane;
                        h[q] = j < rn ? a.rec_hash[rs + j] : 0ull;
                    }
#pragma unroll
                    for (int q = 0; q < 4; ++q) {
                        bool fresh = false;
                        if (h[q] != 0) {
                            uint32_t sl = set_slot_of(h[q], cap);
                            for (;;) {
                                unsigned long long old = atomicCAS(&set[sl], 0ull, (unsigned long long)h[q]);
                                if (old == 0) {
                                    fresh = true;
                                    break;
                                }
                                if (old == h[q]) break;
                                sl = (sl + 1) & (cap - 1);
                            }
                        }
                        distinct += (uint32_t)__popcll(__ballot(fresh));
                    }
                }
            }
        }
        __syncthreads();
        if (lane == 0) {
            a.g_distinct[u] = distinct;
            a.caps[u] = 0;
        }
    }
}

__device__ inline uint32_t insert_run(const uint64_t *rec_hash, uint64_t slot0, uint32_t n, unsigned long long *region,
                                      uint32_t cap, uint32_t lane) {
    uint32_t fresh_n = 0;
    for (uint32_t j0 = 0; j0 < n; j0 += 256) {
        uint64_t h[4];
        uint32_t sl[4];
        unsigned long long old[4];
#pragma unroll
        for (int q = 0; q < 4; ++q) {
            const uint32_t j = j0 + q * 64 + lane;
            h[q] = j < n ? rec_hash[slot0 + j] : 0ull;
        }
#pragma unroll
        for (int q = 0; q < 4; ++q) {
            sl[q] = set_slot_of(h[q], cap);
            old[q] = h[q] ? atomicCAS(&region[sl[q]], 0ull, (unsigned long long)h[q]) : h[q];
        }
#pragma unroll
        for (int q = 0; q < 4; ++q) {
            bool fresh = false;
            if (h[q] != 0) {
                unsigned long long o = old[q];
                for (;;) {
                    if (o == 0) {
                        fresh = true;
                        break;
                    }
                    if (o == h[q]) break;
                    sl[q] = (sl[q] + 1) & (cap - 1);
                    o = atomicCAS(&region[sl[q]], 0ull, (unsigned long long)h[q]);
                }
            }
            fresh_n += (uint32_t)__popcll(__ballot(fresh));
        }
    }
    return fresh_n;
}

__global__ __launch_bounds__(256) void distinct_clear_kernel(uint64_t *set_slots, uint64_t capacity, const dcn_status *status) {
    if (status->set_cursor == 0 || status->rec_overflow || status->run_overflow) return;
    uint64_t total = status->set_cursor;
    if (total > capacity) total = capacity;
    uint64_t stride = (uint64_t)gridDim.x * blockDim.x;
    for (uint64_t i = (uint64_t)blockIdx.x * blockDim.x + threadIdx.x; i < total; i += stride) set_slots[i] = 0;
}

__global__ __launch_bounds__(256) void big_insert_kernel(dcn_distinct_args a) {
    if (a.status->set_cursor == 0 || a.status->rec_overflow || a.status->run_overflow) return;
    const uint32_t NB = a.status->n_big;
    const uint32_t lane = threadIdx.x & 63;
    const uint32_t gwave = (blockIdx.x * blockDim.x + threadIdx.x) >> 6, n_waves = (gridDim.x * blockDim.x) >> 6;
    for (uint32_t bi = gwave; bi < NB; bi += n_waves) {
        const uint2 item = a.big[bi];
        const uint32_t u = item.x;
        const uint32_t first = a.unit_tile_first[u], count = a.unit_tile_count[u];
        const uint32_t cap = a.caps[u];
        unsigned long long *region = (unsigned long long *)(a.set_slots + a.set_off[u]);
        const uint32_t t = item.y + lane;
        uint32_t n = 0;
        uint64_t slot0 = 0;
        if (t < count) {
            n = a.tile_hits[first + t];
            const dcn_tile tl = a.tiles[first + t];
            slot0 = (tl.scan_start + tl.carry()) >> a.rec_shift;
        }
        uint32_t fresh_n = 0;
        unsigned long long runs = __ballot(n != 0);
        while (runs) {
            const int r = __ffsll((long long)runs) - 1;
            runs &= runs - 1;
            fresh_n += insert_run(a.rec_hash, (uint64_t)__shfl((long long)slot0, r, 64), __shfl(n, r, 64), region, cap, lane);
        }
        if (lane == 0 && fresh_n) atomicAdd(&a.g_distinct[u], fresh_n);
    }
    if (a.status->any_scattered == 0) return;
    const uint32_t NT = *a.n_tiles;
    for (uint32_t t = gwave; t < NT; t += n_waves) {
        const dcn_tile tl = a.tiles[t];
        if (a.unit_state[tl.unit] || a.unit_tile_count[tl.unit] != 0xFFFFFFFFu) continue;
        const uint32_t cap = a.caps[tl.unit];
        const uint32_t n = a.tile_hits[t];
        if (!cap || !n) continue;
        const uint32_t fresh_n = insert_run(a.rec_hash, (tl.scan_start + tl.carry()) >> a.rec_shift, n,
                                            (unsigned long long *)(a.set_slots + a.set_off[tl.unit]), cap, lane);
        if (lane == 0 && fresh_n) atomicAdd(&a.g_distinct[tl.unit], fresh_n);
    }
}

__global__ __launch_bounds__(256) void finish_kernel(dcn_finish_args a) {
    unsigned long long st[DCN_N_STATS] = {0, 0, 0, 0, 0, 0};
    const uint32_t stride = gridDim.x * blockDim.x;
    for (uint32_t u0 = blockIdx.x * blockDim.x + threadIdx.x; u0 < a.n_units; u0 += 4 * stride) {
        uint8_t state[4], kept[4];
        uint32_t r0[4], r1[4];
        uint64_t o0[4], o1[4];
#pragma unroll
        for (int q = 0; q < 4; ++q) {
            const uint32_t u = u0 + q * stride;
            state[q] = 2;
            if (u < a.n_units) {
                state[q] = a.unit_state[u];
                kept[q] = a.keep[u];
                r0[q] = a.unit_first_read ? a.unit_first_read[u] : u;
                r1[q] = a.unit_first_read ? a.unit_first_read[u + 1] : u + 1;
            }
        }
#pragma unroll
        for (int q = 0; q < 4; ++q) {
            o0[q] = o1[q] = 0;
            if (state[q] != 2 && a.offsets && !a.status->bad_offsets) {
                o0[q] = a.offsets[r0[q]];
                o1[q] = a.offsets[r1[q]];
            }
        }
#pragma unroll
        for (int q = 0; q < 4; ++q) {
            if (state[q] == 2) continue;
            const uint32_t u = u0 + q * stride;
            bool keep;
            if (state[q]) {
                keep = kept[q] != 0;
            } else {
                uint32_t tot = a.g_total[u], hc = a.g_distinct[u] + (a.g_zero[u] ? 1u : 0u);
                a.g_total[u] = 0;
                a.g_hitcnt[u] = 0;
                a.g_distinct[u] = 0;
                a.g_zero[u] = 0;
                keep = dcn_decide(hc, tot, a.abs_threshold, a.rel_threshold, a.deplete);
                a.keep[u] = keep ? 1 : 0;
                if (a.hits) a.hits[u] = hc;
                if (a.total) a.total[u] = tot;
            }
            if (a.offsets) {
                unsigned long long nseq = r1[q] - r0[q], bp = o1[q] - o0[q];
                st[DCN_STAT_TOTAL_SEQS] += nseq;
                st[DCN_STAT_TOTAL_BP] += bp;
                if (keep) {
                    st[DCN_STAT_OUTPUT_BP] += bp;
                    st[DCN_STAT_OUTPUT_SEQ_COUNTER] += nseq;
                } else {
                    st[DCN_STAT_FILTERED_SEQS] += nseq;
                    st[DCN_STAT_FILTERED_BP] += bp;
                }
            }
        }
    }
    if (a.status->bounds && blockIdx.x == 0 && threadIdx.x == 0) a.report->bounds = a.status->bounds;
    if (a.status->bad_offsets) {
        if (blockIdx.x == 0 && threadIdx.x == 0) a.report->bad_offsets = 1;
        return;
    }
    if (a.status->rec_overflow || a.status->run_overflow) {
        if (blockIdx.x == 0 && threadIdx.x == 0) {
            atomicOr(&a.report->overflow, (a.status->rec_overflow ? 1u : 0u) | (a.status->run_overflow ? 2u : 0u));
            if (a.status->rec_overflow) atomicMax(&a.report->need, (a.status->set_cursor + 3) / 4);
        }
        return;
    }
    if (!a.offsets) return;
    __shared__ unsigned long long red[DCN_N_STATS][4];
    int lane = threadIdx.x & 63, wave = threadIdx.x >> 6;
#pragma unroll
    for (int c = 0; c < DCN_N_STATS; ++c) {
        unsigned long long v = st[c];
#pragma unroll
        for (int d = 32; d >= 1; d >>= 1) v += __shfl_xor(v, d, 64);
        if (lane == 0) red[c][wave] = v;
    }
    __syncthreads();
    if (threadIdx.x < DCN_N_STATS) {
        unsigned long long v = red[threadIdx.x][0] + red[threadIdx.x][1] + red[threadIdx.x][2] + red[threadIdx.x][3];
        if (v) atomicAdd(&a.report->stats[threadIdx.x], v);
    }
}

__global__ __launch_bounds__(256) void probe_hashes_kernel(dcn_probe_hashes_args a) {
    uint64_t stride = (uint64_t)gridDim.x * blockDim.x;
    for (uint64_t i = (uint64_t)blockIdx.x * blockDim.x + threadIdx.x; i < a.n_hashes; i += stride) {
        uint64_t h = a.hashes[i];
        if (h == 0) {
            if (a.table.has_zero) {
                uint32_t lo = 0, hi = a.n_units - 1;
                while (lo < hi) {
                    uint32_t mid = lo + (hi - lo + 1) / 2;
                    if (a.hash_offsets[mid] <= i) lo = mid;
                    else hi = mid - 1;
                }
                a.g_zero[lo] = 1;
            }
        } else if (!dcn_table_contains_dev(a.table, h)) {
            a.hashes[i] = 0;
        }
    }
}

__global__ __launch_bounds__(256) void hash_units_kernel(dcn_probe_hashes_args a) {
    uint32_t u = blockIdx.x * blockDim.x + threadIdx.x;
    if (u == 0) {
        *a.n_tiles = a.n_units;
        a.status->any_records = 1;
        a.status->n_pending = a.n_units;
    }
    if (u >= a.n_units) return;
    const uint64_t n = a.hash_offsets[u + 1] - a.hash_offsets[u];
    dcn_tile t;
    t.scan_start = a.hash_offsets[u];
    t.unit = u;
    t.nwf = (uint32_t)n & 0x3FFFFFFFu;
    a.tiles[u] = t;
    a.tile_hits[u] = (uint32_t)n;
    a.unit_tile_first[u] = u;
    a.unit_tile_count[u] = 1;
    a.unit_state[u] = 0;
    a.pending[u] = u;
    a.g_total[u] = (uint32_t)n;
    a.g_hitcnt[u] = (uint32_t)n;
    a.g_distinct[u] = 0;
    a.g_zero[u] = 0;
}

inline uint32_t blocks_for(uint64_t n, uint32_t cap = 256 * 16) {
    uint64_t b = (n + 255) / 256;
    if (b < 1) b = 1;
    return (uint32_t)(b > cap ? cap : b);
}

}

int dcn_launch_plan(const dcn_plan_args &a, hipStream_t stream) {
    if (a.n_reads >= (1u << 19))
        hipLaunchKernelGGL(plan_kernel<8>, dim3((a.n_reads + 2047) / 2048), dim3(256), 0, stream, a);
    else
        hipLaunchKernelGGL(plan_kernel<1>, dim3((a.n_reads + 255) / 256), dim3(256), 0, stream, a);
    DCN_HIP(hipGetLastError());
    return DCN_OK;
}

int dcn_launch_distinct(const dcn_distinct_args &a, hipStream_t stream) {
    hipLaunchKernelGGL(unit_distinct_kernel, dim3(std::max(1u, std::min(a.n_units, 256u * 10u))), dim3(64), 0, stream, a);
    hipLaunchKernelGGL(distinct_clear_kernel, dim3(1024), dim3(256), 0, stream, a.set_slots, a.set_capacity, a.status);
    hipLaunchKernelGGL(big_insert_kernel, dim3(2048), dim3(256), 0, stream, a);
    DCN_HIP(hipGetLastError());
    return DCN_OK;
}

int dcn_launch_finish(const dcn_finish_args &a, hipStream_t stream) {
    hipLaunchKernelGGL(finish_kernel, dim3(blocks_for(a.n_units, 1024)), dim3(256), 0, stream, a);
    DCN_HIP(hipGetLastError());
    return DCN_OK;
}

int dcn_launch_probe_hashes(const dcn_probe_hashes_args &a, hipStream_t stream) {
    hipLaunchKernelGGL(hash_units_kernel, dim3((a.n_units + 255) / 256), dim3(256), 0, stream, a);
    if (a.n_hashes)
        hipLaunchKernelGGL(probe_hashes_kernel, dim3(blocks_for(a.n_hashes)), dim3(256), 0, stream, a);
    DCN_HIP(hipGetLastError());
    return DCN_OK;
}
```

### deacon-server_amd/csrc/scan.hip

```cpp
#include "dcn_internal.h"
#include "dcn_probe.h"

#include <atomic>

namespace {

__device__ __constant__ uint32_t NT_F[4] = {0x95c60474u, 0x62a02b4cu, 0x82572324u, 0x4be24456u};

__device__ inline uint32_t rotl32(uint32_t x, uint32_t r) { return __funnelshift_l(x, x, r); }

#ifndef DCN_WAVE_OPS_SHFL
#define DCN_WAVE_OPS_SHFL 0
#endif
template <bool MAX>
__device__ inline uint32_t wave_scan_dpp(uint32_t v) {
    auto op = [](uint32_t x, uint32_t y) { return MAX ? max(x, y) : x + y; };
    v = op(v, (uint32_t)__builtin_amdgcn_update_dpp(0, (int)v, 0x111, 0xf, 0xf, false));
    v = op(v, (uint32_t)__builtin_amdgcn_update_dpp(0, (int)v, 0x112, 0xf, 0xf, false));
    v = op(v, (uint32_t)__builtin_amdgcn_update_dpp(0, (int)v, 0x114, 0xf, 0xf, false));
    v = op(v, (uint32_t)__builtin_amdgcn_update_dpp(0, (int)v, 0x118, 0xf, 0xf, false));
    v = op(v, (uint32_t)__builtin_amdgcn_update_dpp(0, (int)v, 0x142, 0xa, 0xf, false));
    v = op(v, (uint32_t)__builtin_amdgcn_update_dpp(0, (int)v, 0x143, 0xc, 0xf, false));
    return v;
}

__device__ inline uint32_t wave_inclusive_scan_u32(uint32_t v, int lane) {
#if DCN_WAVE_OPS_SHFL
#pragma unroll
    for (int d = 1; d < 64; d <<= 1) {
        uint32_t o = __shfl_up(v, d, 64);
        if (lane >= d) v += o;
    }
    return v;
#else
    (void)lane;
    return wave_scan_dpp<false>(v);
#endif
}

__device__ inline uint32_t wave_max_u32(uint32_t v) {
#if DCN_WAVE_OPS_SHFL
#pragma unroll
    for (int d = 32; d >= 1; d >>= 1) v = max(v, __shfl_xor(v, d, 64));
    return v;
#else
    return (uint32_t)__builtin_amdgcn_readlane((int)wave_scan_dpp<true>(v), 63);
#endif
}

__device__ inline uint32_t wave_last_u32(uint32_t incl) {
#if DCN_WAVE_OPS_SHFL
    return __shfl(incl, 63, 64);
#else
    return (uint32_t)__builtin_amdgcn_readlane((int)incl, 63);
#endif
}

#ifndef DCN_LIST_BY_LANE
#define DCN_LIST_BY_LANE 1
#endif
#if DCN_LIST_BY_LANE
#define DCN_LIST_AT(lane_, entry_) list[lane_][entry_]
#else
#define DCN_LIST_AT(lane_, entry_) list[entry_][lane_]
#endif
constexpr int DCN_LSTRIDE = 42;
static_assert(DCN_LSTRIDE >= DCN_LCAP && (DCN_LSTRIDE / 2) % 2 == 1 && DCN_LSTRIDE % 2 == 0, "odd dword stride");
constexpr int DCN_RCAP = 256;

struct WaveShared {
    uint4 tab[16];
#if DCN_LIST_BY_LANE
    uint16_t list[DCN_WAVE][DCN_LSTRIDE];
#else
    uint16_t list[DCN_LCAP + 2][DCN_WAVE];
#endif
    uint64_t ring_hash[DCN_RCAP];
    uint32_t total[DCN_WAVE];
    uint32_t hits[DCN_WAVE];
    uint32_t items[DCN_WAVE];
    uint16_t hraw[DCN_WAVE];
    uint32_t ucap[DCN_WAVE];
    uint32_t unit_of[DCN_WAVE];
    uint16_t start[DCN_WAVE + 2];
    uint32_t uhits[DCN_WAVE];
    uint64_t run_base[DCN_WAVE];
    uint8_t local[DCN_WAVE];
    uint8_t lok[DCN_WAVE];
};

#ifndef DCN_EXP
#define DCN_EXP 0
#endif
#ifndef DCN_MIN_WAVES
#define DCN_MIN_WAVES 4
#endif
#ifndef DCN_FAST_EXTRA_ROUNDS
#define DCN_FAST_EXTRA_ROUNDS 4
#endif
#ifndef DCN_MIN_WAVES_FAST
#define DCN_MIN_WAVES_FAST 4
#endif

template <bool B>
struct BoolTag {
    static constexpr bool value = B;
};
template <int N>
struct IntTag {
    static constexpr int value = N;
};
#ifndef DCN_EXPORT_UNIFORM
#define DCN_EXPORT_UNIFORM 0
#endif
#ifndef DCN_PIPE_B
#define DCN_PIPE_B 0
#endif
#ifndef DCN_U_FINAL
#define DCN_U_FINAL 1
#endif

template <int W, bool K128, bool DUMP, bool FAST, bool VAR = false>
__global__ __launch_bounds__(DCN_WAVE, FAST ? DCN_MIN_WAVES_FAST : DCN_MIN_WAVES) void scan_kernel(dcn_scan_args a) {
    static_assert(!VAR || (W == 0 && !FAST), "the variant path is the generic-w counting / dump kernel");
    __shared__ WaveShared sh;
    extern __shared__ __align__(16) uint2 dyn_ring[];

    const int lane = threadIdx.x;
    const uint32_t NT = a.status->bad_offsets ? 0u : *a.n_tiles;
    const uint32_t wave_first = blockIdx.x * DCN_WAVE;
    if (wave_first >= NT) return;
    const uint32_t k = a.k;
    const uint32_t w = W > 0 ? (uint32_t)W : a.w;
    const uint32_t l = k + w - 1;

    const uint32_t tile_idx = wave_first + lane;
    const bool have_tile = tile_idx < NT;
    dcn_tile t = a.tiles[have_tile ? tile_idx : NT - 1];
    if (!have_tile) t.nwf = 0;
    const uint32_t carry = t.carry();
    const uint32_t nwc = t.n_windows() ? t.n_windows() + carry : 0;
    const uint32_t tile_read_pos = (DUMP && have_tile && a.tile_read_pos) ? a.tile_read_pos[tile_idx] : 0u;
    const uint32_t unit_prev = __shfl_up(t.unit, 1, 64);
    const uint64_t start_prev = (uint64_t)__shfl_up((long long)t.scan_start, 1, 64);
    const bool head = lane == 0 || t.unit != unit_prev || t.scan_start < start_prev;
    const unsigned long long head_mask = __ballot(head);
    const uint32_t uslot = (uint32_t)__popcll(head_mask & ((2ull << lane) - 1)) - 1;
    sh.total[lane] = 0;
    sh.hits[lane] = 0;
    sh.items[lane] = 0;
    sh.hraw[lane] = 0;
    sh.lok[lane] = 0;
    sh.uhits[lane] = 0;
    sh.ucap[lane] = 0;
    if (head) {
        sh.unit_of[uslot] = t.unit;
        sh.run_base[uslot] = (t.scan_start + carry) >> a.rec_shift;
        bool loc = false;
        if (!DUMP) {
            if (t.whole_unit()) {
                loc = true;
            } else {
                uint32_t first = a.unit_tile_first[t.unit], count = a.unit_tile_count[t.unit];
                loc = count != 0xFFFFFFFFu && first >= wave_first && first + count <= wave_first + DCN_WAVE;
            }
        }
        sh.local[uslot] = loc ? 1 : 0;
    }
    const uint32_t ROT = VAR ? a.nt_rot : 1u;
    const uint32_t ROTR = (32u - ROT) & 31u;
    if (lane < 16) {
        uint32_t in = lane & 3, out = lane >> 2;
        uint4 e;
        e.x = NT_F[in];
        e.y = rotl32(NT_F[in ^ 2], (ROT * (k - 1)) & 31);
        e.z = rotl32(NT_F[out], (ROT * k) & 31);
        e.w = rotl32(NT_F[out ^ 2], ROTR);
        sh.tab[lane] = e;
    }
    __syncthreads();
    if (!DUMP) {
        const uint32_t head_lane = 63u - (uint32_t)__clzll(head_mask & ((2ull << lane) - 1));
        const uint64_t first_win = (uint64_t)__shfl((long long)(t.scan_start + carry), head_lane, 64);
        const uint32_t slack = t.n_windows() < a.tile_windows ? l - 1 : 0u;
        if (have_tile && t.n_windows()) atomicMax(&sh.ucap[uslot], (uint32_t)(t.scan_start + carry + t.n_windows() + slack - first_win));
        __syncthreads();
        if (head) sh.ucap[uslot] = (uint32_t)(((first_win + sh.ucap[uslot]) >> a.rec_shift) - (first_win >> a.rec_shift));
        __syncthreads();
    }

    const uint32_t *packed = a.packed;
    const int64_t s = (int64_t)t.scan_start;

    uint32_t fw = 0, rc = 0, tg = 0;
    {
        const int64_t q_in = s >> 4;
        const uint32_t sh_in = (uint32_t)(s & 15) * 2;
        uint32_t cur = 0;
        for (uint32_t tt = 0; tt + 1 < k; ++tt) {
            if ((tt & 15) == 0) cur = __funnelshift_r(packed[q_in + (tt >> 4)], packed[q_in + (tt >> 4) + 1], sh_in);
            uint32_t c = (cur >> (2 * (tt & 15))) & 3;
            uint4 e = sh.tab[c];
            fw = rotl32(fw, VAR ? ROT : 1u) ^ e.x;
            rc = rotl32(rc, VAR ? ROTR : 31u) ^ e.y;
            tg += c >> 1;
        }
    }
    uint32_t zprev = 0, wprev = 0;

    uint32_t cnt = 0;
    uint32_t emitted_before = 0;
    bool first_pending = carry;
    uint32_t prev = 0xFFFFFFFFu;
    uint32_t n_ring = 0;
    bool go_global = false;
    bool any_rec = false;
    const uint32_t nk = nwc ? nwc + w - 1 : 0;
    const uint32_t jmax = wave_max_u32(nk);

    auto flush = [&](auto u_tag, bool final_flush) {
        constexpr int U = decltype(u_tag)::value;
#ifdef DCN_PHASEB_PRIO
        __builtin_amdgcn_s_setprio(DCN_PHASEB_PRIO);
#endif
        const uint32_t skip0 = (first_pending && cnt > 0) ? 1u : 0u;
        const uint32_t us_skip = uslot | (skip0 << 8);
        const uint32_t cnt_eff = cnt - skip0;
        uint32_t incl = wave_inclusive_scan_u32(cnt_eff, lane);
        uint32_t M = wave_last_u32(incl);
        sh.start[lane] = (uint16_t)(incl - cnt_eff);
        if (lane == 63) sh.start[64] = (uint16_t)M;
        if (!DUMP && cnt_eff) atomicAdd(&sh.items[uslot], cnt_eff);
        if (!final_flush) go_global = true;
        __syncthreads();
        if (!DUMP && head) {
            bool ok = sh.local[uslot] && !go_global && sh.items[uslot] <= (uint32_t)(DCN_RCAP - DCN_WAVE);
            sh.lok[uslot] = ok ? 1 : 0;
        }
        __syncthreads();
        constexpr int NPW = K128 ? 5 : 3;
        constexpr int NMW = K128 ? 3 : 2;
        constexpr bool PIPE = DCN_PIPE_B && U == 1;
        struct Item {
            bool act;
            uint32_t lo, idx, rel, o_uslot;
            uint64_t p;
            uint32_t mw[NMW], pw[NPW];
        };
        auto fetch = [&](uint32_t E, Item &it) {
            const uint32_t e = E + lane;
            it.act = e < M;
            uint32_t l_ = 0, h_ = 63;
#pragma unroll
            for (int step = 0; step < 6; ++step) {
                const uint32_t mid = (l_ + h_ + 1) >> 1;
                const bool le = sh.start[mid] <= e;
                l_ = le ? mid : l_;
                h_ = le ? h_ : mid - 1;
            }
            it.lo = l_;
            it.idx = it.act ? e - sh.start[l_] : 0;
            const uint32_t o_pk = __shfl(us_skip, l_, 64);
            const uint32_t o_skip = o_pk >> 8;
#ifdef DCN_DEBUG_BOUNDS
            if (it.act && (l_ > 63u || it.idx + o_skip >= (uint32_t)DCN_LCAP + 2u)) {
                a.status->bounds = 1;
                it.act = false;
                it.idx = 0;
            }
#endif
            it.rel = sh.DCN_LIST_AT(l_, it.idx + o_skip);
            const long long o_s = __shfl((long long)s, l_, 64);
            it.o_uslot = o_pk & 0xFFu;
            it.p = (uint64_t)(o_s + it.rel);
#ifdef DCN_DEBUG_BOUNDS
            if (it.act && it.p + k > a.stream_bases) {
                a.status->bounds = 2;
                it.act = false;
                it.p = 0;
            }
#endif
            if (it.act) {
                const uint32_t *mp = a.invmask + (it.p >> 5);
                const uint32_t *pp = packed + (it.p >> 4);
#pragma unroll
                for (int q = 0; q < NMW; ++q) it.mw[q] = mp[q];
#pragma unroll
                for (int q = 0; q < NPW; ++q) it.pw[q] = pp[q];
            }
        };
        Item cur, nxt;
        if (PIPE && M) fetch(0, cur);
        for (uint32_t E = 0; E < ((DCN_EXP & 2) ? 0u : M); E += DCN_WAVE * U) {
            bool act[U];
            uint32_t lo[U], hi[U];
#pragma unroll
            for (int u = 0; u < U; ++u) {
                act[u] = E + u * DCN_WAVE + lane < M;
                lo[u] = 0;
                hi[u] = 63;
            }
            if (!PIPE) {
#pragma unroll
            for (int it = 0; it < 6; ++it) {
#pragma unroll
                for (int u = 0; u < U; ++u) {
                    uint32_t e = E + u * DCN_WAVE + lane;
                    uint32_t mid = (lo[u] + hi[u] + 1) >> 1;
                    bool le = sh.start[mid] <= e;
                    lo[u] = le ? mid : lo[u];
                    hi[u] = le ? hi[u] : mid - 1;
                }
            }
            }
            uint64_t p[U];
            uint32_t o_uslot[U], idx[U], rel[U];
            uint32_t mw[U][NMW], pw[U][NPW];
            if (PIPE) {
                act[0] = cur.act;
                lo[0] = cur.lo;
                idx[0] = cur.idx;
                rel[0] = cur.rel;
                o_uslot[0] = cur.o_uslot;
                p[0] = cur.p;
#pragma unroll
                for (int q = 0; q < NMW; ++q) mw[0][q] = cur.mw[q];
#pragma unroll
                for (int q = 0; q < NPW; ++q) pw[0][q] = cur.pw[q];
            }
#pragma unroll
            for (int u = 0; u < (PIPE ? 0 : U); ++u) {
                uint32_t e = E + u * DCN_WAVE + lane;
                idx[u] = act[u] ? e - sh.start[lo[u]] : 0;
                const uint32_t o_pk = __shfl(us_skip, lo[u], 64);
                const uint32_t o_skip = o_pk >> 8;
#ifdef DCN_DEBUG_BOUNDS
                if (act[u] && (lo[u] > 63u || idx[u] + o_skip >= (uint32_t)DCN_LCAP + 2u)) {
                    a.status->bounds = 1;
                    act[u] = false;
                    idx[u] = 0;
                }
#endif
                rel[u] = sh.DCN_LIST_AT(lo[u], idx[u] + o_skip);
                long long o_s = __shfl((long long)s, lo[u], 64);
                o_uslot[u] = o_pk & 0xFFu;
                p[u] = (uint64_t)(o_s + rel[u]);
#ifdef DCN_DEBUG_BOUNDS
                if (act[u] && p[u] + k > a.stream_bases) {
                    a.status->bounds = 2;
                    act[u] = false;
                    p[u] = 0;
                }
#endif
            }
#pragma unroll
            for (int u = 0; u < (PIPE ? 0 : U); ++u) {
                if (act[u]) {
                    const uint32_t *mp = a.invmask + (p[u] >> 5);
                    const uint32_t *pp = packed + (p[u] >> 4);
#pragma unroll
                    for (int q = 0; q < NMW; ++q) mw[u][q] = (DCN_EXP & 16) ? 0u : mp[q];
#pragma unroll
                    for (int q = 0; q < NPW; ++q) pw[u][q] = pp[q];
                }
            }
            bool valid[U];
            uint64_t hash[U];
#pragma unroll
            for (int u = 0; u < U; ++u) {
                valid[u] = false;
                hash[u] = 0;
                if (act[u]) {
                    uint32_t msh = (uint32_t)(p[u] & 31);
                    if constexpr (K128) {
                        uint64_t mbits = ((uint64_t)__funnelshift_r(mw[u][1], mw[u][NMW - 1], msh) << 32) |
                                         __funnelshift_r(mw[u][0], mw[u][1], msh);
                        valid[u] = (mbits & ((~0ull) >> (64 - k))) == 0;
                    } else {
                        valid[u] = (__funnelshift_r(mw[u][0], mw[u][1], msh) & (0xFFFFFFFFu >> (32 - k))) == 0;
                    }
                    uint32_t psh = (uint32_t)(p[u] & 15) * 2;
                    uint64_t lo64 = ((uint64_t)__funnelshift_r(pw[u][1], pw[u][2], psh) << 32) |
                                    __funnelshift_r(pw[u][0], pw[u][1], psh);
                    if constexpr (K128) {
                        uint64_t hi64 = ((uint64_t)__funnelshift_r(pw[u][3], pw[u][NPW - 1], psh) << 32) |
                                        __funnelshift_r(pw[u][2], pw[u][3], psh);
                        hash[u] = dcn_kmer_hash128_bits(lo64, hi64, k);
                    } else {
                        hash[u] = dcn_kmer_hash64_bits(lo64, k);
                    }
                }
            }
            if (DUMP) {
#pragma unroll
                for (int u = 0; u < U; ++u) {
                    uint32_t o_eb = __shfl(emitted_before, lo[u], 64);
                    uint32_t o_rp = __shfl(tile_read_pos, lo[u], 64);
                    uint32_t o_carry = __shfl(carry, lo[u], 64);
                    long long o_s = __shfl((long long)s, lo[u], 64);
                    if (act[u]) {
                        uint64_t slot = (uint64_t)o_s + o_carry + o_eb + idx[u];
                        a.dump_hash[slot] = valid[u] ? hash[u] : 0;
                        a.dump_pos[slot] = a.dump_abs ? (uint32_t)p[u] : o_rp + rel[u];
                        a.dump_valid[slot] = valid[u] ? 1 : 0;
                    }
                }
                if (PIPE) {
                    if (E + DCN_WAVE < M) fetch(E + DCN_WAVE, nxt);
                    cur = nxt;
                }
                continue;
            }
            uint32_t grp[U];
            dcn_group g[U];
#pragma unroll
            for (int u = 0; u < U; ++u) {
                grp[u] = dcn_group_of(hash[u], a.table.group_shift, a.table.group_mask);
                if (valid[u] && !(DCN_EXP & 1)) g[u] = dcn_load_group(a.table, grp[u]);
            }
            if (PIPE && E + DCN_WAVE < M) fetch(E + DCN_WAVE, nxt);
            bool hit[U];
#pragma unroll
            for (int u = 0; u < U; ++u) {
                hit[u] = false;
                if (valid[u]) {
                    if (DCN_EXP & 1) {
                        hit[u] = (hash[u] & 1) != 0;
                    } else if (hash[u] == 0) {
                        hit[u] = a.table.has_zero != 0;
                    } else {
                        int r = dcn_group_resolve(g[u], hash[u]);
                        while (r < 0) {
                            grp[u] = (grp[u] + 1) & a.table.group_mask;
                            r = dcn_group_resolve(dcn_load_group(a.table, grp[u]), hash[u]);
                        }
                        hit[u] = r == 1;
                    }
                } else if (act[u]) {
                    atomicSub(&sh.total[o_uslot[u]], 1u);
                }
            }
#pragma unroll
            for (int u = 0; u < U; ++u) {
                const bool lok = hit[u] && sh.lok[o_uslot[u]];
                const unsigned long long hb = __ballot(lok);
                if (hb) {
                    const unsigned long long lt = (1ull << lane) - 1;
                    const uint32_t nh = (uint32_t)__popcll(hb);
                    const uint32_t rank = (uint32_t)__popcll(hb & lt);
                    const uint32_t x = n_ring + rank;
                    if (lok) sh.ring_hash[x & (DCN_RCAP - 1)] = hash[u];
                    const unsigned long long below = hb & lt;
                    const uint32_t prev_lane = below ? 63u - (uint32_t)__clzll(below) : (uint32_t)lane;
                    const uint32_t prev_us = __shfl(o_uslot[u], prev_lane, 64);
                    const bool run_head = lok && (below == 0 || prev_us != o_uslot[u]);
                    const unsigned long long hm_all = __ballot(run_head);
                    const unsigned long long hm = hm_all & (lt | (1ull << lane));
                    const uint32_t head_lane = hm ? 63u - (uint32_t)__clzll(hm) : 0u;
                    const uint32_t rank_head = (uint32_t)__popcll(hb & ((1ull << head_lane) - 1));
                    const uint32_t run = lok ? sh.hraw[o_uslot[u]] + (rank - rank_head) : 0u;
                    __syncthreads();
                    bool dup = false;
                    for (uint32_t d0 = 0; __any(d0 < ((DCN_EXP & 8) ? 0u : run)); d0 += 4) {
                        uint64_t v0 = sh.ring_hash[(x - d0 - 1) & (DCN_RCAP - 1)];
                        uint64_t v1 = sh.ring_hash[(x - d0 - 2) & (DCN_RCAP - 1)];
                        uint64_t v2 = sh.ring_hash[(x - d0 - 3) & (DCN_RCAP - 1)];
                        uint64_t v3 = sh.ring_hash[(x - d0 - 4) & (DCN_RCAP - 1)];
                        dup |= (d0 + 0 < run && v0 == hash[u]) | (d0 + 1 < run && v1 == hash[u]) |
                               (d0 + 2 < run && v2 == hash[u]) | (d0 + 3 < run && v3 == hash[u]);
                    }
                    const unsigned long long db = __ballot(dup);
                    if (run_head) {
                        const unsigned long long later = hm_all & ~((2ull << lane) - 1);
                        const unsigned long long upto = later ? ((1ull << (__ffsll((long long)later) - 1)) - 1) : ~0ull;
                        const unsigned long long rm = hb & upto & ~lt;
                        sh.hraw[o_uslot[u]] += (uint32_t)__popcll(rm);
                        sh.hits[o_uslot[u]] += (uint32_t)__popcll(rm & ~db);
                    }
                    n_ring += nh;
                    __syncthreads();
                }
                {
                    const bool rec = hit[u] && !lok;
                    const unsigned long long rb = (DCN_EXP & 256) ? 0ull : __ballot(rec);
#if DCN_EXPORT_UNIFORM
                    const uint32_t us0 = rb ? (uint32_t)__builtin_amdgcn_readlane((int)o_uslot[u], __ffsll((long long)rb) - 1) : 0u;
                    const bool one_unit = rb && __ballot(rec && o_uslot[u] != us0) == 0;
                    if (one_unit) {
                        const unsigned long long lt = (1ull << lane) - 1;
                        any_rec = true;
                        const uint32_t base = sh.uhits[us0];
                        if (rec) {
                            const uint32_t at = base + (uint32_t)__popcll(rb & lt);
                            if (at < sh.ucap[us0]) {
                                if (!(DCN_EXP & 512)) a.rec_hash[sh.run_base[us0] + at] = hash[u];
                            } else {
                                a.status->run_overflow = 1;
                            }
                            if (hash[u] == 0) a.g_zero[sh.unit_of[us0]] = 1;
                            if ((rb & lt) == 0) sh.uhits[us0] = base + (uint32_t)__popcll(rb);
                        }
                    } else
#endif
                    if (rb) {
                        const unsigned long long lt = (1ull << lane) - 1;
                        const unsigned long long below = rb & lt;
                        const uint32_t prev_lane = below ? 63u - (uint32_t)__clzll(below) : (uint32_t)lane;
                        const uint32_t prev_us = __shfl(o_uslot[u], prev_lane, 64);
                        const bool run_head = rec && (below == 0 || prev_us != o_uslot[u]);
                        const unsigned long long hm_all = __ballot(run_head);
                        const unsigned long long hm = hm_all & (lt | (1ull << lane));
                        const uint32_t head_lane = hm ? 63u - (uint32_t)__clzll(hm) : 0u;
                        const uint32_t rank = (uint32_t)__popcll(below) - (uint32_t)__popcll(rb & ((1ull << head_lane) - 1));
                        any_rec = true;
                        if (rec) {
                            const uint32_t at = sh.uhits[o_uslot[u]] + rank;
                            if (at < sh.ucap[o_uslot[u]]) {
                                if (!(DCN_EXP & 512)) a.rec_hash[sh.run_base[o_uslot[u]] + at] = hash[u];
                            } else {
                                a.status->run_overflow = 1;
                            }
                            if (hash[u] == 0) a.g_zero[sh.unit_of[o_uslot[u]]] = 1;
                        }
                        if (run_head) {
                            const unsigned long long later = hm_all & ~((2ull << lane) - 1);
                            const unsigned long long upto = later ? ((1ull << (__ffsll((long long)later) - 1)) - 1) : ~0ull;
                            sh.uhits[o_uslot[u]] += (uint32_t)__popcll(rb & upto & ~lt);
                        }
                    }
                }
            }
            if (PIPE) cur = nxt;
        }
        if (!DUMP && cnt_eff) atomicAdd(&sh.total[uslot], cnt_eff);
        emitted_before += cnt_eff;
        if (skip0) first_pending = false;
        cnt = 0;
        __syncthreads();
#ifdef DCN_PHASEB_PRIO
        __builtin_amdgcn_s_setprio(0);
#endif
    };

    constexpr uint32_t STEP = W > 0 ? (uint32_t)W : 8u;
    static_assert(STEP < DCN_LCAP && STEP <= 16, "a block's bits must fit one word and the list must outlast a block");
    uint32_t ringL[STEP], ringR[STEP];
    uint32_t pl = 0xFFFFFFFFu, pr = 0;
    if (W > 0) {
#pragma unroll
        for (uint32_t r = 0; r < STEP; ++r) {
            ringL[r] = 0xFFFFFFFFu;
            ringR[r] = 0;
        }
    } else if (VAR) {
        for (uint32_t r = 0; r < w; ++r)
            reinterpret_cast<ulonglong2 *>(dyn_ring)[r * DCN_WAVE + lane] = make_ulonglong2(~0ull, 0ull);
    } else {
        for (uint32_t r = 0; r < w; ++r) dyn_ring[r * DCN_WAVE + lane] = make_uint2(0xFFFFFFFFu, 0u);
    }
    uint32_t gslot = 0;
    uint32_t keymask = 0xFFFF0000u;
    asm volatile("" : "+v"(keymask));
    const uint32_t lhalf = l >> 1;

    int64_t b_in = 2 * (s + (int64_t)(k - 1)), b_k = 2 * s, b_l = 2 * (s - (int64_t)(w - 1));
    int64_t wi_in = b_in >> 5, wi_k = b_k >> 5, wi_l = b_l >> 5;
    uint32_t so_in = (uint32_t)(b_in & 31), so_k = (uint32_t)(b_k & 31), so_l = (uint32_t)(b_l & 31);
    uint32_t ra_in = packed[wi_in], rb_in = packed[wi_in + 1];
    uint32_t ra_k = packed[wi_k], rb_k = packed[wi_k + 1];
    uint32_t ra_l = packed[wi_l], rb_l = packed[wi_l + 1];
    uint32_t w_in = __funnelshift_r(ra_in, rb_in, so_in);
    uint32_t w_k = __funnelshift_r(ra_k, rb_k, so_k);
    uint32_t w_l = __funnelshift_r(ra_l, rb_l, so_l);
    auto advance_streams = [&]() {
        so_in += 2 * STEP; wi_in += so_in >> 5; so_in &= 31;
        so_k += 2 * STEP; wi_k += so_k >> 5; so_k &= 31;
        so_l += 2 * STEP; wi_l += so_l >> 5; so_l &= 31;
        if (DCN_EXP & 128) {
            ra_in = rb_in ^ 0x5A5A5A5Au; rb_in = ra_k + 0x1234567u; ra_k = rb_l; rb_k = ra_l ^ ra_in; ra_l = rb_k; rb_l = rb_in;
            return;
        }
        ra_in = packed[wi_in]; rb_in = packed[wi_in + 1];
        if (DCN_EXP & 64) {
            ra_k = ra_in; rb_k = rb_in; ra_l = ra_in; rb_l = rb_in;
        } else {
            ra_k = packed[wi_k]; rb_k = packed[wi_k + 1];
            ra_l = packed[wi_l]; rb_l = packed[wi_l + 1];
        }
    };
    advance_streams();
    {
        if (W > 0) {
            uint32_t m = (w - 1) >= 16 ? 0xAAAAAAAAu : (0xAAAAAAAAu & ((1u << (2 * (w - 1))) - 1u));
            tg += __popc(w_l & m);
        } else {
            for (uint32_t b = 1; b < w; ++b) {
                int64_t p = s - (int64_t)b;
                tg += (packed[p >> 4] >> (2 * (uint32_t)(p & 15) + 1)) & 1u;
            }
        }
    }
    uint4 e_nx = sh.tab[(w_in & 3) | ((w_k & 3) << 2)];

    auto block = [&](auto first_tag, const uint32_t jb) {
        constexpr bool FIRST = decltype(first_tag)::value;
        const uint32_t te = (w_in & 0x33333333u) | ((w_k & 0x33333333u) << 2);
        const uint32_t to = ((w_in >> 2) & 0x33333333u) | (w_k & 0xCCCCCCCCu);
        uint32_t nw_in = 0, nw_k = 0, nw_l = 0;
#pragma unroll
        for (uint32_t r = 0; r < STEP; ++r) {
            const uint32_t j = jb + r;
            const uint4 e = e_nx;
            if (r + 1 < STEP) {
                const uint32_t tsel = ((r + 1) & 1) ? to : te;
                const uint32_t n = (r + 1) >> 1;
                const uint32_t addr16 = n == 0 ? ((tsel << 4) & 0xF0u) : ((tsel >> (4 * n - 4)) & 0xF0u);
                e_nx = *reinterpret_cast<const uint4 *>(reinterpret_cast<const char *>(sh.tab) + addr16);
            } else {
                nw_in = __funnelshift_r(ra_in, rb_in, so_in);
                nw_k = __funnelshift_r(ra_k, rb_k, so_k);
                nw_l = __funnelshift_r(ra_l, rb_l, so_l);
                e_nx = sh.tab[(nw_in & 3) | ((nw_k & 3) << 2)];
                advance_streams();
            }
            const uint32_t hi_in = (w_in >> (2 * r + 1)) & 1;
            const uint32_t hl = (w_l >> (2 * r + 1)) & 1;
            fw = __builtin_amdgcn_bitop3_b32(rotl32(fw, VAR ? ROT : 1u), zprev, e.x, 0x96);
            rc = __builtin_amdgcn_bitop3_b32(rotl32(rc, VAR ? ROTR : 31u), wprev, e.y, 0x96);
            zprev = e.z;
            wprev = e.w;
            const uint32_t h = (VAR && a.nt_combine_xor) ? (fw ^ rc) : (fw + rc);
            const uint32_t jlow = j & 0xFFFFu;
            const uint32_t lk = __builtin_amdgcn_bitop3_b32(h, keymask, jlow, 0xEA);
            const uint32_t rk = __builtin_amdgcn_bitop3_b32(h, keymask, jlow, 0xAE);
            uint32_t lmin, rmax;
            if constexpr (W > 0) {
                ringL[r] = lk;
                ringR[r] = rk;
                pl = min(pl, lk);
                pr = max(pr, rk);
                if (r == W - 1) {
#pragma unroll
                    for (int qq = W - 2; qq >= 0; --qq) {
                        ringL[qq] = min(ringL[qq], ringL[qq + 1]);
                        ringR[qq] = max(ringR[qq], ringR[qq + 1]);
                    }
                    lmin = ringL[0];
                    rmax = ringR[0];
                    pl = 0xFFFFFFFFu;
                    pr = 0;
                } else {
                    lmin = min(pl, ringL[(r + 1) % STEP]);
                    rmax = max(pr, ringR[(r + 1) % STEP]);
                }
            } else if constexpr (VAR) {
                ulonglong2 *ring64 = reinterpret_cast<ulonglong2 *>(dyn_ring);
                ring64[gslot * DCN_WAVE + lane] = make_ulonglong2(((unsigned long long)(h & a.cmp_mask) << 32) | j,
                                                                  ((unsigned long long)(~h & a.cmp_mask) << 32) | j);
                gslot = gslot + 1 == w ? 0 : gslot + 1;
                unsigned long long lmin64 = ~0ull, rmax64 = 0ull;
                for (uint32_t qq = 0; qq < w; ++qq) {
                    ulonglong2 v = ring64[qq * DCN_WAVE + lane];
                    lmin64 = v.x < lmin64 ? v.x : lmin64;
                    rmax64 = v.y > rmax64 ? v.y : rmax64;
                }
                lmin = (uint32_t)lmin64;
                rmax = (uint32_t)rmax64;
            } else {
                dyn_ring[gslot * DCN_WAVE + lane] = make_uint2(lk, rk);
                gslot = gslot + 1 == w ? 0 : gslot + 1;
                lmin = 0xFFFFFFFFu;
                rmax = 0;
                for (uint32_t qq = 0; qq < w; ++qq) {
                    uint2 v = dyn_ring[qq * DCN_WAVE + lane];
                    lmin = min(lmin, v.x);
                    rmax = max(rmax, v.y);
                }
            }
            tg += hi_in;
            if constexpr (W > 0) {
                if (!FIRST || r == STEP - 1) {
                    const uint32_t sel = ((tg > lhalf) ? lmin : rmax) & 0xFFFFu;
                    const bool emit = FIRST ? (nwc > 0) : ((j - (w - 1) < nwc) && sel != prev);
                    if (!(DCN_EXP & 4)) sh.DCN_LIST_AT(lane, cnt) = (uint16_t)sel;
                    cnt += emit ? 1u : 0u;
                    prev = sel;
                }
            } else {
                const uint32_t sel = ((tg > lhalf) ? lmin : rmax) & 0xFFFFu;
                const uint32_t i = j - (w - 1);
                const bool in_range = i < nwc;
                const bool emit = in_range && sel != prev;
                sh.DCN_LIST_AT(lane, cnt) = (uint16_t)sel;
                cnt += emit ? 1u : 0u;
                prev = in_range ? sel : prev;
            }
            tg -= hl;
        }
        w_in = nw_in;
        w_k = nw_k;
        w_l = nw_l;
    };

    if (jmax > 0) {
        block(BoolTag<true>{}, 0);
        if (__any(cnt > DCN_LCAP - STEP)) flush(IntTag<1>{}, false);
        for (uint32_t jb = STEP; jb < jmax; jb += STEP) {
            block(BoolTag<false>{}, jb);
            if (__any(cnt > DCN_LCAP - STEP)) flush(IntTag<1>{}, false);
        }
    }
    if (FAST && !DUMP && !go_global) {
        const uint32_t skip0 = (first_pending && cnt > 0) ? 1u : 0u;
        const uint32_t cnt_eff = cnt - skip0;
        const unsigned long long tile_mask = __ballot(have_tile);
        const unsigned long long up1 = lane < 63 ? 1ull << (lane + 1) : 0ull, down1 = lane > 0 ? 1ull << (lane - 1) : 0ull;
        const bool prev_head = (head_mask & down1) != 0;
        const bool next_mate = (tile_mask & up1) != 0 && (head_mask & up1) == 0;
        const uint32_t uh = head ? (uint32_t)lane : (uint32_t)lane - 1u;
        const uint32_t partner = head ? (next_mate ? (uint32_t)lane + 1u : (uint32_t)lane) : (uint32_t)lane - 1u;
        const uint32_t partner_cnt = __shfl(cnt_eff, partner, 64);
        const uint32_t cnt_unit = cnt_eff + (partner != (uint32_t)lane ? partner_cnt : 0u);
        const bool own = !have_tile || ((head || (prev_head && a.early_out_pairs)) && sh.local[uslot] && cnt_unit <= a.early_out_max_items);
        if (__all(own)) {
            const uint32_t need = (uint32_t)a.abs_threshold;
            uint64_t seen0 = 0, seen1 = 0, seen2 = 0;
            uint32_t nh = 0;
            auto probe_item = [&](uint64_t p, bool actv, uint64_t &hash) -> bool {
                bool hit = false;
                hash = 0;
                if (actv) {
                    const uint32_t *mp = a.invmask + (p >> 5);
                    const uint32_t *pp = packed + (p >> 4);
                    const uint32_t m0 = mp[0], m1 = mp[1], m2 = K128 ? mp[2] : 0u;
                    uint32_t pw[K128 ? 5 : 3];
#pragma unroll
                    for (int q = 0; q < (K128 ? 5 : 3); ++q) pw[q] = pp[q];
                    const uint32_t msh = (uint32_t)(p & 31);
                    bool valid;
                    if constexpr (K128) {
                        const uint64_t mbits = ((uint64_t)__funnelshift_r(m1, m2, msh) << 32) | __funnelshift_r(m0, m1, msh);
                        valid = (mbits & ((~0ull) >> (64 - k))) == 0;
                    } else {
                        valid = (__funnelshift_r(m0, m1, msh) & (0xFFFFFFFFu >> (32 - k))) == 0;
                    }
                    const uint32_t psh = (uint32_t)(p & 15) * 2;
                    const uint64_t lo64 = ((uint64_t)__funnelshift_r(pw[1], pw[2], psh) << 32) | __funnelshift_r(pw[0], pw[1], psh);
                    if constexpr (K128) {
                        const uint64_t hi64 = ((uint64_t)__funnelshift_r(pw[3], pw[4], psh) << 32) | __funnelshift_r(pw[2], pw[3], psh);
                        hash = dcn_kmer_hash128_bits(lo64, hi64, k);
                    } else {
                        hash = dcn_kmer_hash64_bits(lo64, k);
                    }
                    if (valid) {
                        if (hash == 0) {
                            hit = a.table.has_zero != 0;
                        } else {
                            uint32_t grp = dcn_group_of(hash, a.table.group_shift, a.table.group_mask);
                            int r = dcn_group_resolve(dcn_load_group(a.table, grp), hash);
                            while (r < 0) {
                                grp = (grp + 1) & a.table.group_mask;
                                r = dcn_group_resolve(dcn_load_group(a.table, grp), hash);
                            }
                            hit = r == 1;
                        }
                    }
                }
                return hit;
            };
            auto note_hit = [&](uint64_t hash) {
                const bool dup = (nh > 0 && hash == seen0) | (nh > 1 && hash == seen1) | (nh > 2 && hash == seen2);
                if (!dup) {
                    seen2 = nh == 2 ? hash : seen2;
                    seen1 = nh == 1 ? hash : seen1;
                    seen0 = nh == 0 ? hash : seen0;
                    ++nh;
                }
            };
            const uint32_t maxc = wave_max_u32(cnt_eff);
            const uint32_t R1 = min(need + (uint32_t)DCN_FAST_EXTRA_ROUNDS, maxc);
            for (uint32_t j = 0; j < R1; ++j) {
                const bool actv = j < cnt_eff && nh < need;
                if (!__any(actv)) break;
                uint64_t hash;
                const uint32_t rel = sh.DCN_LIST_AT(lane, (actv ? j : 0u) + skip0);
                const bool hit = probe_item((uint64_t)(s + rel), actv, hash);
                const bool p_hit = __shfl((int)hit, partner, 64) != 0;
                const uint64_t p_hash = (uint64_t)__shfl((long long)hash, partner, 64);
                const bool paired_lane = partner != (uint32_t)lane;
                const bool h1 = head ? hit : p_hit, h2 = head ? (paired_lane && p_hit) : hit;
                const uint64_t v1 = head ? hash : p_hash, v2 = head ? p_hash : hash;
                if (h1 && nh < need) note_hit(v1);
                if (h2 && nh < need) note_hit(v2);
            }
            const uint32_t rem = (nh < need && cnt_eff > R1) ? cnt_eff - R1 : 0u;
            const uint32_t incl = wave_inclusive_scan_u32(rem, lane);
            const uint32_t M = wave_last_u32(incl);
            if (M) {
                sh.start[lane] = (uint16_t)(incl - rem);
                if (lane == 63) sh.start[64] = (uint16_t)M;
                __syncthreads();
                for (uint32_t E = 0; E < M; E += DCN_WAVE) {
                    const uint32_t e = E + lane;
                    const bool act = e < M;
                    uint32_t lo = 0, hi = 63;
#pragma unroll
                    for (int it = 0; it < 6; ++it) {
                        const uint32_t mid = (lo + hi + 1) >> 1;
                        const bool le = sh.start[mid] <= e;
                        lo = le ? mid : lo;
                        hi = le ? hi : mid - 1;
                    }
                    const uint32_t idx = act ? e - sh.start[lo] + R1 : 0u;
                    const uint32_t o_skip = __shfl(skip0, lo, 64);
                    const uint32_t o_nh = __shfl(nh, lo, 64);
                    const long long o_s = __shfl((long long)s, lo, 64);
                    const uint32_t rel = sh.DCN_LIST_AT(lo, idx + o_skip);
                    uint64_t hash;
                    const bool hit = probe_item((uint64_t)(o_s + rel), act && o_nh < need, hash);
                    unsigned long long hb = __ballot(hit);
                    while (hb) {
                        const int src = __ffsll((long long)hb) - 1;
                        hb &= hb - 1;
                        const uint64_t h = (uint64_t)__shfl((long long)hash, src, 64);
                        const uint32_t o = __shfl(lo, src, 64);
                        const uint32_t o_uh = __shfl(uh, o, 64);
                        if (uh == o_uh && nh < need) note_hit(h);
                    }
                }
            }
            if (have_tile && head) {
                a.keep[t.unit] = (a.deplete ? nh < need : nh >= need) ? 1 : 0;
                a.unit_state[t.unit] = 1;
            }
            return;
        }
    }
    flush(IntTag<DCN_U_FINAL>{}, true);
    if (DUMP) {
        if (have_tile) a.dump_count[tile_idx] = emitted_before;
        return;
    }

    if (any_rec && lane == 0) a.status->any_records = 1;
    {
        const bool pending = have_tile && !sh.lok[uslot] && !(DCN_EXP & 1024);
        bool enrol = false;
        if (pending) {
            const uint32_t th = head ? sh.uhits[uslot] : 0u;
            a.tile_hits[tile_idx] = th;
            if (th) enrol = atomicAdd(&a.g_hitcnt[t.unit], th) == 0u;
        }
        const unsigned long long em = __ballot(enrol);
        if (em) {
            uint32_t base = 0;
            if (lane == 0) base = atomicAdd(&a.status->n_pending, (uint32_t)__popcll(em));
            base = __shfl(base, 0, 64);
            if (enrol) {
                a.pending[base + (uint32_t)__popcll(em & ((1ull << lane) - 1))] = t.unit;
                if (t.whole_unit()) {
                    a.unit_tile_first[t.unit] = tile_idx;
                    a.unit_tile_count[t.unit] = 1;
                }
            }
        }
    }

    if (head && have_tile) {
        uint32_t tot = sh.total[uslot];
        if (sh.lok[uslot]) {
            uint32_t hc = sh.hits[uslot];
            a.keep[t.unit] = dcn_decide(hc, tot, a.abs_threshold, a.rel_threshold, a.deplete) ? 1 : 0;
            if (a.hits) a.hits[t.unit] = hc;
            if (a.total) a.total[t.unit] = tot;
            a.unit_state[t.unit] = 1;
        } else if (tot) {
            atomicAdd(&a.g_total[t.unit], tot);
        }
    }
}

template <int W, bool VAR = false>
int launch_w(const dcn_scan_args &args, uint32_t blocks, bool dump, bool k128, size_t dyn, hipStream_t stream) {
#define DCN_LAUNCH(K128_, DUMP_, FAST_)                                                               \
    do {                                                                                              \
        auto kern = scan_kernel<W, K128_, DUMP_, FAST_ && !VAR, VAR>;                                 \
        if (dyn > 0) {                                                                                \
            hipError_t e = hipFuncSetAttribute(reinterpret_cast<const void *>(kern),                  \
                                               hipFuncAttributeMaxDynamicSharedMemorySize, (int)dyn); \
            if (e != hipSuccess) return dcn_fail(DCN_ERR_HIP, std::string("dyn LDS: ") + hipGetErrorString(e)); \
        }                                                                                             \
        hipLaunchKernelGGL(kern, dim3(blocks), dim3(DCN_WAVE), dyn, stream, args);                    \
    } while (0)
    const bool fast = !dump && args.early_out_max_items != 0;
    if (k128) {
        if (dump) DCN_LAUNCH(true, true, false);
        else if (fast) DCN_LAUNCH(true, false, true);
        else DCN_LAUNCH(true, false, false);
    } else {
        if (dump) DCN_LAUNCH(false, true, false);
        else if (fast) DCN_LAUNCH(false, false, true);
        else DCN_LAUNCH(false, false, false);
    }
#undef DCN_LAUNCH
    DCN_HIP(hipGetLastError());
    return DCN_OK;
}

}

namespace {
std::atomic<uint32_t> g_variant{DCN_VARIANT_DEFAULT};
}

uint32_t dcn_current_variant() { return g_variant.load(); }

int dcn_set_minimizer_variant(uint32_t nt_rot, uint32_t cmp_bits, uint32_t combine) {
    if (nt_rot < 1 || nt_rot > 31) return dcn_fail(DCN_ERR_ARG, "minimizer variant: rotation must be 1..31");
    if (cmp_bits != 16 && cmp_bits != 32) return dcn_fail(DCN_ERR_ARG, "minimizer variant: 16 or 32 hash bits are compared");
    if (combine > 1) return dcn_fail(DCN_ERR_ARG, "minimizer variant: combine is 0 (fw + rc) or 1 (fw ^ rc)");
    g_variant.store((nt_rot << 16) | (cmp_bits << 8) | combine);
    return DCN_OK;
}

int dcn_get_minimizer_variant(uint32_t *nt_rot, uint32_t *cmp_bits, uint32_t *combine) {
    const uint32_t v = g_variant.load();
    if (nt_rot) *nt_rot = v >> 16;
    if (cmp_bits) *cmp_bits = (v >> 8) & 0xFF;
    if (combine) *combine = v & 0xFF;
    return DCN_OK;
}

int dcn_launch_scan(const dcn_scan_args &args_in, uint32_t max_tiles, bool dump, hipStream_t stream) {
    if (max_tiles == 0) return DCN_OK;
    uint32_t blocks = (max_tiles + DCN_WAVE - 1) / DCN_WAVE;
    bool k128 = args_in.k > 32;
    const uint32_t v = args_in.variant ? args_in.variant : DCN_VARIANT_DEFAULT;
    if (v != DCN_VARIANT_DEFAULT) {
        dcn_scan_args args = args_in;
        args.nt_rot = v >> 16;
        args.cmp_mask = ((v >> 8) & 0xFF) == 32 ? 0xFFFFFFFFu : 0xFFFF0000u;
        args.nt_combine_xor = v & 0xFF;
        args.early_out_max_items = 0;
        if (args.w > 128) return dcn_fail(DCN_ERR_ARG, "minimizer variant: w <= 128 (two u64 keys per window slot in LDS)");
        size_t dyn = (size_t)args.w * DCN_WAVE * sizeof(ulonglong2);
        return launch_w<0, true>(args, blocks, dump, k128, dyn, stream);
    }
    const dcn_scan_args &args = args_in;
    switch (args.w) {
    case 15: return launch_w<15>(args, blocks, dump, k128, 0, stream);
    case 11: return launch_w<11>(args, blocks, dump, k128, 0, stream);
    case 1: return launch_w<1>(args, blocks, dump, k128, 0, stream);
    default: {
        size_t dyn = (size_t)args.w * DCN_WAVE * sizeof(uint2);
        return launch_w<0>(args, blocks, dump, k128, dyn, stream);
    }
    }
}
```

### deacon-server_amd/filter.py

```python
import ctypes as C
import os

import numpy as np

from . import _native as N
from ._native import DeaconHipError, Params

DEFAULT_KMER_LENGTH = 31
DEFAULT_WINDOW_SIZE = 15


def _ptr(a):
    return a.ctypes.data_as(C.c_void_p) if a is not None else None


def _as_u8(seq):
    if isinstance(seq, np.ndarray):
        return np.ascontiguousarray(seq, dtype=np.uint8)
    if isinstance(seq, str):
        seq = seq.encode()
    return np.frombuffer(bytes(seq), dtype=np.uint8)


def concat_reads(reads):
# ... 439 lines not shown


class Locator(_Context):

    def __init__(self, index, max_gap=None, min_hits=1, prefix_length=0, member_mask=0xFFFFFFFF,
                 max_batch_bases=1 << 26, max_batch_reads=1 << 20):
        self.index = index
        w = index.w if hasattr(index, "w") else index.window_size
        self.max_gap = 2 * int(w) - 1 if max_gap is None else int(max_gap)
        self.min_hits = int(min_hits)
        self.prefix_length = int(prefix_length)
        self.member_mask = int(member_mask)
        super().__init__(index._h, max_batch_bases, max_batch_reads)

    def _params(self):
        return N.LocateParams(self.max_gap, self.min_hits, self.member_mask, 0, self.prefix_length)

    def locate_batch(self, bases, offsets):
        bases, offsets, n_reads = _batch(bases, offsets)
        seg_offsets = np.zeros(n_reads + 1, np.uint64)
        p = self._params()
        cap = getattr(self, "_last_total", 0)
        segs = np.zeros(max(cap, 1), SEGMENT_DTYPE)
        for _ in range(2):
            rc = N.lib().dcn_locate_batch(self._h, self.index._h, _ptr(bases) if len(bases) else None, _ptr(offsets),
                                          n_reads, C.byref(p), _ptr(seg_offsets), _ptr(segs) if cap else None, cap)
            if rc != N.DCN_ERR_CAPACITY:
                break
            cap = int(seg_offsets[n_reads])
            segs = np.zeros(cap, SEGMENT_DTYPE)
        N.check(rc)
        self._last_total = int(seg_offsets[n_reads])
        return seg_offsets, segs[:int(seg_offsets[n_reads])]


TRACK_BIN_DTYPE = np.dtype([("n_positions", np.uint32), ("n_keys", np.uint32), ("n_observed", np.uint32),
                            ("max_depth", np.uint32), ("sum_depth", np.uint64)])


class DepthTracker(_Context):

    def __init__(self, index_set, max_batch_bases=1 << 26, max_batch_reads=1 << 20, bin_bases=1000, member=None,
                 depth_cap=0, prefix_length=0):
        self.index_set = index_set
        self.bin_bases = int(bin_bases)
        if member is None:
            self.member_mask = (1 << index_set.n) - 1
        elif isinstance(member, (int, np.integer)):
            if int(member) < 0:
                raise ValueError(f"member {member} out of range")
            self.member_mask = 1 << int(member)
        else:
            self.member_mask = index_set._mask(member)
        self.depth_cap = int(depth_cap)
        self.prefix_length = int(prefix_length)
        if not (0 <= self.bin_bases <= 0xFFFFFFFF and 0 <= self.member_mask <= 0xFFFFFFFF and 0 <= self.depth_cap <= 0xFFFFFFFF):
            raise ValueError("bin_bases / member / depth_cap out of range")
        super().__init__(index_set._h, max_batch_bases, max_batch_reads)

    def _params(self):
        return N.TrackParams(self.bin_bases, self.member_mask, self.depth_cap, 0, self.prefix_length)

    def track_batch(self, bases, offsets):
        bases, offsets, n_reads = _batch(bases, offsets)
        bin_offsets = np.zeros(n_reads + 1, np.uint64)
        p = self._params()
        rc = N.lib().dcn_depth_track_batch(self._h, self.index_set._h, _ptr(bases) if len(bases) else None, _ptr(offsets),
                                           n_reads, C.byref(p), _ptr(bin_offsets), None, 0)
        if rc != N.DCN_ERR_CAPACITY:
            N.check(rc)
            return bin_offsets, np.zeros(0, TRACK_BIN_DTYPE)
        total = int(bin_offsets[n_reads])
        bins = np.zeros(total, TRACK_BIN_DTYPE)
        N.check(N.lib().dcn_depth_track_batch(self._h, self.index_set._h, _ptr(bases) if len(bases) else None,
                                              _ptr(offsets), n_reads, C.byref(p), _ptr(bin_offsets), _ptr(bins), total))
        return bin_offsets, bins

    def track(self, seqs):
        seqs = list(seqs)
        bases, offsets = concat_reads(seqs)
        bo, bins = self.track_batch(bases, offsets)
        return [bins[int(bo[r]):int(bo[r + 1])] for r in range(len(seqs))]


PLACEMENT_DTYPE = np.dtype([("record", np.uint32), ("reverse", np.uint32), ("votes", np.uint32), ("n_anchors", np.uint32),
                            ("n_positions", np.uint32), ("read_start", np.uint32), ("read_end", np.uint32),
                            ("reserved", np.uint32), ("ref_start", np.uint64), ("ref_end", np.uint64)])
UNPLACED = 0xFFFFFFFF
SPLIT_PLACEMENT_DTYPE = np.dtype(PLACEMENT_DTYPE.descr + [("rank", np.uint32), ("n_placed", np.uint32),
                                                          ("rival_votes", np.uint32), ("mapq", np.uint32)])
PAIR_PLACEMENT_DTYPE = np.dtype(SPLIT_PLACEMENT_DTYPE.descr + [("flags", np.uint32), ("pair_votes", np.uint32),
                                                               ("tlen", np.int64)])
PAIR_PROPER, PAIR_RESCUED, PAIR_MATE_PLACED = 1, 2, 4


class AnchorMap(Index):

    def __init__(self, index):
        h = C.c_void_p()
        N.check(N.lib().dcn_anchor_map_create(index._h, C.byref(h)))
        super().__init__(h, index.device)
        self._ctx = None

    def clone(self, device):
        h = C.c_void_p()
        N.check(N.lib().dcn_index_clone(self._h, int(device), C.byref(h)))
        return Index(h, int(device))

    def _context(self, n_bases, n_reads):
        have_bases, have_reads = (self._ctx.max_batch_bases, self._ctx.max_batch_reads) if self._ctx else (0, 0)
        if self._ctx and n_bases <= have_bases and n_reads <= have_reads:
            return self._ctx
        if self._ctx:
            self._ctx.close()
        self._ctx = _Context(self._h, max(int(n_bases), have_bases, 1 << 20), max(int(n_reads), have_reads, 1 << 10))
        return self._ctx

    def add(self, bases, offsets):
        bases, offsets, n = _batch(bases, offsets)
        first = C.c_uint32()
        ctx = self._context(int(offsets[-1]) if n > 0 else 0, n)
        N.check(N.lib().dcn_anchor_map_add(self._h, ctx._h, _ptr(bases) if len(bases) else None, _ptr(offsets), n, C.byref(first)))
        return first.value

    def add_records(self, records):
        bases, offsets = concat_reads(list(records))
        return self.add(bases, offsets)

    def info(self):
        r, k, a, p = C.c_uint32(), C.c_uint64(), C.c_uint64(), C.c_uint64()
        N.check(N.lib().dcn_anchor_map_info(self._h, C.byref(r), C.byref(k), C.byref(a), C.byref(p)))
        return {"records": r.value, "keys": k.value, "anchors": a.value, "repeats": p.value}

    def anchors(self):
        n = C.c_uint64()
        rc = N.lib().dcn_anchor_map_anchors(self._h, None, None, None, 0, C.byref(n))
        if rc != N.DCN_ERR_CAPACITY:
            N.check(rc)
        cap = int(n.value)
        keys, rec, pos = np.zeros(max(cap, 1), np.uint64), np.zeros(max(cap, 1), np.uint32), np.zeros(max(cap, 1), np.uint32)
        N.check(N.lib().dcn_anchor_map_anchors(self._h, _ptr(keys), _ptr(rec), _ptr(pos), cap, C.byref(n)))
        return keys[:cap], rec[:cap], pos[:cap]

    def close(self):
        if getattr(self, "_ctx", None):
            self._ctx.close()
            self._ctx = None
        super().close()


class Placer(_Context):

    def __init__(self, anchor_map, max_batch_bases=1 << 26, max_batch_reads=1 << 20, band_bases=256, min_votes=2,
                 prefix_length=0):
        self.anchor_map = anchor_map
        self.band_bases = int(band_bases)
        self.min_votes = int(min_votes)
        self.prefix_length = int(prefix_length)
        super().__init__(anchor_map._h, max_batch_bases, max_batch_reads)

    def _params(self):
        return N.PlaceParams(self.band_bases, self.min_votes, self.prefix_length, (C.c_uint32 * 2)(0, 0))

    def place_batch(self, bases, offsets):
        bases, offsets, n_reads = _batch(bases, offsets)
        out = np.zeros(max(n_reads, 1), PLACEMENT_DTYPE)
        p = self._params()
        N.check(N.lib().dcn_place_batch(self._h, self.anchor_map._h, _ptr(bases) if len(bases) else None, _ptr(offsets),
                                        n_reads, C.byref(p), _ptr(out)))
        return out[:n_reads]

    def place(self, reads):
        bases, offsets = concat_reads(list(reads))
        return self.place_batch(bases, offsets)

    def place_split_batch(self, bases, offsets, max_placements=4, capacity=None):
        bases, offsets, n_reads = _batch(bases, offsets)
        cap = n_reads * int(max_placements) if capacity is None else int(capacity)
        place_offsets = np.zeros(n_reads + 1, np.uint64)
        out = np.zeros(max(cap, 1), SPLIT_PLACEMENT_DTYPE)
        counts = np.zeros((max(n_reads, 1), 2), np.uint32)
        p = N.PlaceSplitParams(self.band_bases, self.min_votes, self.prefix_length, int(max_placements), (C.c_uint32 * 3)(0, 0, 0))
        N.check(N.lib().dcn_place_split_batch(self._h, self.anchor_map._h, _ptr(bases) if len(bases) else None, _ptr(offsets),
                                              n_reads, C.byref(p), _ptr(place_offsets), _ptr(out) if cap else None, cap,
                                              _ptr(counts)))
        return place_offsets, out[:int(place_offsets[n_reads])], counts[:n_reads]

    def place_split(self, reads, max_placements=4):
        reads = list(reads)
        bases, offsets = concat_reads(reads)
        po, rows, _ = self.place_split_batch(bases, offsets, max_placements)
        return [rows[int(po[r]):int(po[r + 1])] for r in range(len(reads))]

    def place_pair_batch(self, bases, offsets, max_placements=4, max_insert=1000, hist_bin_bases=8, want_hist=True):
        bases, offsets, n_reads = _batch(bases, offsets)
        out = np.zeros(max(n_reads, 1), PAIR_PLACEMENT_DTYPE)
        hist = np.zeros(N.PAIR_HIST_BINS, np.uint64) if want_hist else None
        p = N.PlacePairParams(self.band_bases, self.min_votes, self.prefix_length, int(max_placements), int(max_insert),
                              int(hist_bin_bases), (C.c_uint32 * 3)(0, 0, 0))
        N.check(N.lib().dcn_place_pair_batch(self._h, self.anchor_map._h, _ptr(bases) if len(bases) else None, _ptr(offsets),
                                             n_reads, C.byref(p), _ptr(out), _ptr(hist) if want_hist else None))
        return out[:n_reads], hist

    def place_pairs(self, reads1, reads2, **kw):
        reads1, reads2 = list(reads1), list(reads2)
        if len(reads1) != len(reads2):
            raise ValueError("place_pairs: the two lists must have one mate each per pair")
        bases, offsets = concat_reads([m for pair in zip(reads1, reads2) for m in pair])
        return self.place_pair_batch(bases, offsets, **kw)


class FilterProcessor(_Context):

    def __init__(self, index, abs_threshold=2, rel_threshold=0.01, prefix_length=0, deplete=False,
                 max_batch_bases=1 << 26, max_batch_reads=1 << 20):
        self.index = index
        self.abs_threshold = int(abs_threshold)
        self.rel_threshold = float(rel_threshold)
        self.prefix_length = int(prefix_length)
        self.deplete = bool(deplete)
        super().__init__(index._h, max_batch_bases, max_batch_reads)

    def _params(self):
        return Params(self.abs_threshold, self.rel_threshold, self.prefix_length, 1 if self.deplete else 0, 0)

    def filter_batch(self, bases, offsets, unit_id=None, counts=True):
        bases, offsets, n_reads = _batch(bases, offsets)
        if unit_id is not None:
            unit_id = np.ascontiguousarray(unit_id, dtype=np.uint32)
            n_units = int(unit_id[-1]) + 1 if n_reads else 0
        else:
            n_units = n_reads
        keep = np.zeros(max(n_units, 1), np.uint8)
        p = self._params()
        if not counts:
            N.check(N.lib().dcn_filter_batch(self._h, _ptr(bases) if len(bases) else None, _ptr(offsets),
                                             _ptr(unit_id), n_reads, C.byref(p), _ptr(keep), None, None))
            return keep[:n_units].astype(bool)
        hits = np.zeros(max(n_units, 1), np.uint32)
        total = np.zeros(max(n_units, 1), np.uint32)
        N.check(N.lib().dcn_filter_batch(self._h, _ptr(bases) if len(bases) else None, _ptr(offsets),
                                         _ptr(unit_id), n_reads, C.byref(p), _ptr(keep), _ptr(hits), _ptr(total)))
        return keep[:n_units].astype(bool), hits[:n_units], total[:n_units]

    def _outputs(self, offsets, unit_id, counts, out):
        n_reads = len(offsets) - 1
        n_units = (int(unit_id[-1]) + 1 if n_reads else 0) if unit_id is not None else n_reads
        if out is not None:
            keep, hits, total = out
        else:
            keep = np.zeros(max(n_units, 1), np.uint8)
            hits = np.zeros(max(n_units, 1), np.uint32) if counts else None
            total = np.zeros(max(n_units, 1), np.uint32) if counts else None
        return n_reads, n_units, keep, hits, total

    def submit(self, bases, offsets, unit_id=None, counts=True, out=None):
        bases, offsets, _ = _batch(bases, offsets)
        if unit_id is not None:
            unit_id = np.ascontiguousarray(unit_id, dtype=np.uint32)
        n_reads, n_units, keep, hits, total = self._outputs(offsets, unit_id, counts, out)
        p = self._params()
        t = C.c_uint64()
        N.check(N.lib().dcn_filter_batch_submit(self._h, _ptr(bases) if len(bases) else None, _ptr(offsets),
                                                _ptr(unit_id), n_reads, C.byref(p), _ptr(keep), _ptr(hits),
                                                _ptr(total), C.byref(t)))
        return PendingBatch(self, t.value, n_units, keep, hits, total, (bases, offsets, unit_id, p))

    def submit_packed(self, packed, invmask, offsets, unit_id=None, counts=True, out=None):
        packed = np.ascontiguousarray(packed, dtype=np.uint32)
        invmask = np.ascontiguousarray(invmask, dtype=np.uint32)
        offsets = np.ascontiguousarray(offsets, dtype=np.uint64)
        if unit_id is not None:
            unit_id = np.ascontiguousarray(unit_id, dtype=np.uint32)
        n_reads, n_units, keep, hits, total = self._outputs(offsets, unit_id, counts, out)
        g = (int(offsets[-1]) + 31) // 32 if n_reads else 0
        if len(packed) < 2 * g or len(invmask) < g:
            raise ValueError("packed / invmask must hold whole 32-base groups of the batch")
        p = self._params()
        t = C.c_uint64()
        N.check(N.lib().dcn_filter_batch_packed_submit(self._h, _ptr(packed), _ptr(invmask), _ptr(offsets),
                                                       _ptr(unit_id), n_reads, C.byref(p), _ptr(keep), _ptr(hits),
                                                       _ptr(total), C.byref(t)))
        return PendingBatch(self, t.value, n_units, keep, hits, total, (packed, invmask, offsets, unit_id, p))

    def filter_batch_packed(self, packed, invmask, offsets, unit_id=None, counts=True):
        return self.submit_packed(packed, invmask, offsets, unit_id, counts).wait()

    def filter_reads(self, reads, paired=False):
        bases, offsets = concat_reads(reads)
        unit_id = (np.arange(len(reads), dtype=np.uint32) // 2) if paired else None
        return self.filter_batch(bases, offsets, unit_id)

    def filter_batch_device(self, d_bases, d_offsets, n_reads, n_bases, d_keep, d_hits=None, d_total=None,
                            d_unit_id=None, n_units=None):
        p = self._params()
        if n_units is None:
            n_units = n_reads
        N.check(N.lib().dcn_filter_batch_device(self._h, d_bases, d_offsets, d_unit_id, n_reads, n_bases, n_units,
                                                C.byref(p), d_keep, d_hits, d_total))

    def reserve_records(self, n_records):
        N.check(N.lib().dcn_ctx_reserve_records(self._h, int(n_records)))

    def should_keep_sequence(self, seq):
        keep, hits, total = self.filter_reads([seq])
        return bool(keep[0]), int(hits[0]), int(total[0])

    def should_keep_pair(self, seq1, seq2):
        keep, hits, total = self.filter_reads([seq1, seq2], paired=True)
        return bool(keep[0]), int(hits[0]), int(total[0])

    def reset_stats(self):
        N.check(N.lib().dcn_ctx_reset_stats(self._h))

    def set_profiling(self, enable=True):
        N.check(N.lib().dcn_ctx_set_profiling(self._h, 2 if enable == 2 else (1 if enable else 0)))

    def summary(self, elapsed_seconds):
        s = self.stats()
        seqs_in, bp_in = s["total_seqs"], s["total_bp"]
        seqs_out, bp_out = seqs_in - s["filtered_seqs"], s["output_bp"]

        def prop(a, b):
            return a / b if b else 0.0

        return {
            "k": self.index.kmer_length, "w": self.index.window_size,
            "abs_threshold": self.abs_threshold, "rel_threshold": self.rel_threshold,
            "prefix_length": self.prefix_length, "deplete": self.deplete,
            "seqs_in": seqs_in, "seqs_out": seqs_out, "seqs_out_proportion": prop(seqs_out, seqs_in),
            "seqs_removed": s["filtered_seqs"], "seqs_removed_proportion": prop(s["filtered_seqs"], seqs_in),
            "bp_in": bp_in, "bp_out": bp_out, "bp_out_proportion": prop(bp_out, bp_in),
            "bp_removed": s["filtered_bp"], "bp_removed_proportion": prop(s["filtered_bp"], bp_in),
            "time": elapsed_seconds,
            "seqs_per_second": int(seqs_in / elapsed_seconds) if elapsed_seconds > 0 else 0,
            "bp_per_second": int(bp_in / elapsed_seconds) if elapsed_seconds > 0 else 0,
        }

    def minimizer_hashes_batch(self, bases, offsets, prefix_length=None):
        bases, offsets, n_reads = _batch(bases, offsets)
        pl = self.prefix_length if prefix_length is None else int(prefix_length)
        out_off = np.zeros(n_reads + 1, np.uint64)
        cap = max(int(len(bases)), 1)
        hashes = np.zeros(cap, np.uint64)
        pos = np.zeros(cap, np.uint32)
        N.check(N.lib().dcn_minimizer_hashes_batch(self._h, _ptr(bases) if len(bases) else None, _ptr(offsets),
                                                   n_reads, pl, _ptr(out_off), _ptr(hashes), _ptr(pos), cap))
        n = int(out_off[-1])
        return out_off, hashes[:n], pos[:n]

    def should_keep_hashes(self, hashes, hash_offsets):
        hashes = np.ascontiguousarray(hashes, dtype=np.uint64)
        hash_offsets = np.ascontiguousarray(hash_offsets, dtype=np.uint64)
        n_units = len(hash_offsets) - 1
        keep = np.zeros(max(n_units, 1), np.uint8)
        hits = np.zeros(max(n_units, 1), np.uint32)
        total = np.zeros(max(n_units, 1), np.uint32)
        p = self._params()
        N.check(N.lib().dcn_should_keep_hashes(self._h, _ptr(hashes) if len(hashes) else None, _ptr(hash_offsets),
                                               n_units, C.byref(p), _ptr(keep), _ptr(hits), _ptr(total)))
        return keep[:n_units].astype(bool), hits[:n_units], total[:n_units]


def stats_allreduce(processors):
    arr = (C.c_void_p * len(processors))(*[p._h for p in processors])
    c = (C.c_uint64 * N.N_STATS)()
    N.check(N.lib().dcn_stats_allreduce(arr, len(processors), c))
    return dict(zip(N.STAT_NAMES, (int(x) for x in c)))


def get_minimizer_hashes_and_positions(processor, seq, prefix_length=0):
    bases, offsets = concat_reads([seq])
    _, h, p = processor.minimizer_hashes_batch(bases, offsets, prefix_length)
    return h, p


def _should_keep(processor, per_unit_hashes, abs_threshold, rel_threshold, deplete):
    lens = np.fromiter((len(h) for h in per_unit_hashes), dtype=np.uint64, count=len(per_unit_hashes))
    off = np.zeros(len(per_unit_hashes) + 1, np.uint64)
    np.cumsum(lens, out=off[1:])
    flat = (np.concatenate([np.asarray(h, dtype=np.uint64) for h in per_unit_hashes])
            if len(per_unit_hashes) and off[-1] else np.zeros(0, np.uint64))
    saved = (processor.abs_threshold, processor.rel_threshold, processor.deplete)
    processor.abs_threshold, processor.rel_threshold, processor.deplete = int(abs_threshold), float(rel_threshold), bool(deplete)
    try:
        keep, hits, total = processor.should_keep_hashes(flat, off)
    finally:
        processor.abs_threshold, processor.rel_threshold, processor.deplete = saved
    return [(bool(k), int(h), int(t)) for k, h, t in zip(keep, hits, total)]


def unpaired_should_keep(processor, input_minimizers, abs_threshold, rel_threshold, deplete):
    return _should_keep(processor, input_minimizers, abs_threshold, rel_threshold, deplete)


def paired_should_keep(processor, input_minimizers, abs_threshold, rel_threshold, deplete):
    return _should_keep(processor, input_minimizers, abs_threshold, rel_threshold, deplete)
```

### include/deacon_hip.h

```cpp
#ifndef DEACON_HIP_H
#define DEACON_HIP_H

#include <stddef.h>
#include <stdint.h>

#ifdef __cplusplus
extern "C" {
#endif

#define DCN_OK 0
#define DCN_ERR_ARG (-1)
#define DCN_ERR_HIP (-2)
#define DCN_ERR_NOMEM (-3)
#define DCN_ERR_IO (-4)
#define DCN_ERR_FORMAT (-5)
#define DCN_ERR_CAPACITY (-6)
#define DCN_ERR_INTERNAL (-7)

typedef struct dcn_index dcn_index;
typedef struct dcn_ctx dcn_ctx;

typedef struct dcn_params {
    uint64_t abs_threshold;
    double rel_threshold;
    uint64_t prefix_length;
    uint32_t deplete;
    uint32_t reserved;
} dcn_params;

enum {
    DCN_STAT_TOTAL_SEQS = 0,
    DCN_STAT_FILTERED_SEQS = 1,
    DCN_STAT_TOTAL_BP = 2,
    DCN_STAT_OUTPUT_BP = 3,
    DCN_STAT_FILTERED_BP = 4,
    DCN_STAT_OUTPUT_SEQ_COUNTER = 5,
    DCN_N_STATS = 6
};

#define DCN_ABI_MAJOR 1
#define DCN_ABI_MINOR 11
int dcn_abi_version(uint32_t *major, uint32_t *minor);
const char *dcn_version(void);
const char *dcn_last_error(void);
int dcn_device_count(int *count);

int dcn_set_minimizer_variant(uint32_t nt_rot, uint32_t cmp_bits, uint32_t combine );
int dcn_get_minimizer_variant(uint32_t *nt_rot, uint32_t *cmp_bits, uint32_t *combine);


int dcn_index_from_keys(const uint64_t *keys, uint64_t n, uint8_t k, uint8_t w, int device, dcn_index **out);

int dcn_index_from_file(const char *path, int device, dcn_index **out);

int dcn_index_build(const uint8_t *bases, const uint64_t *offsets, uint32_t n_seqs, uint8_t k, uint8_t w,
                    float entropy_threshold, uint64_t capacity_keys, int device, dcn_index **out);

int dcn_index_keys(const dcn_index *index, uint64_t *out, uint64_t capacity, uint64_t *n);

int dcn_index_write_file(const dcn_index *index, const char *path);

int dcn_index_union(const dcn_index *const *inputs, uint32_t n, dcn_index **out);

int dcn_index_diff(const dcn_index *first, const dcn_index *second, dcn_index **out);

int dcn_index_intersect(const dcn_index *const *inputs, uint32_t n, dcn_index **out);

int dcn_index_header(const dcn_index *index, uint8_t *k, uint8_t *w, uint64_t *n_keys);

int dcn_index_device(const dcn_index *index, int *device);

int dcn_index_memory(const dcn_index *index, uint64_t *table_bytes);

int dcn_index_contains(const dcn_index *index, const uint64_t *keys, uint64_t n, uint8_t *out);

int dcn_index_contains_device(const dcn_index *index, const uint64_t *d_keys, uint64_t n, uint8_t *d_out,
                              void *stream);

int dcn_index_probe_ceiling(const dcn_index *index, const uint64_t *d_keys, uint64_t n, uint32_t reps,
                            double *probes_per_s);

int dcn_index_clone(const dcn_index *index, int device, dcn_index **out);

void dcn_index_destroy(dcn_index *index);


int dcn_ctx_create(const dcn_index *index, uint64_t max_batch_bases, uint32_t max_batch_reads, dcn_ctx **out);
void dcn_ctx_destroy(dcn_ctx *ctx);


int dcn_filter_batch(dcn_ctx *ctx, const uint8_t *bases, const uint64_t *offsets, const uint32_t *unit_id,
                     uint32_t n_reads, const dcn_params *params, uint8_t *keep, uint32_t *hits,
                     uint32_t *total);

int dcn_filter_batch_submit(dcn_ctx *ctx, const uint8_t *bases, const uint64_t *offsets, const uint32_t *unit_id,
                            uint32_t n_reads, const dcn_params *params, uint8_t *keep, uint32_t *hits,
                            uint32_t *total, uint64_t *ticket);
int dcn_filter_batch_wait(dcn_ctx *ctx, uint64_t ticket);

int dcn_filter_batch_packed(dcn_ctx *ctx, const uint32_t *packed, const uint32_t *invmask, const uint64_t *offsets,
                            const uint32_t *unit_id, uint32_t n_reads, const dcn_params *params, uint8_t *keep,
                            uint32_t *hits, uint32_t *total);
int dcn_filter_batch_packed_submit(dcn_ctx *ctx, const uint32_t *packed, const uint32_t *invmask,
                                   const uint64_t *offsets, const uint32_t *unit_id, uint32_t n_reads,
                                   const dcn_params *params, uint8_t *keep, uint32_t *hits, uint32_t *total,
                                   uint64_t *ticket);

int dcn_pack_ascii(const uint8_t *bases, uint64_t n_bases, uint32_t *packed, uint32_t *invmask, uint32_t *saw_newline);

int dcn_filter_batch_device(dcn_ctx *ctx, const uint8_t *d_bases, const uint64_t *d_offsets,
                            const uint32_t *d_unit_id, uint32_t n_reads, uint64_t n_bases, uint32_t n_units,
                            const dcn_params *params, uint8_t *d_keep, uint32_t *d_hits, uint32_t *d_total);

int dcn_ctx_synchronize(dcn_ctx *ctx);

int dcn_ctx_reserve_records(dcn_ctx *ctx, uint64_t n_records);

void *dcn_ctx_stream(dcn_ctx *ctx);

int dcn_host_alloc(uint64_t bytes, void **out);
void dcn_host_free(void *p);

int dcn_minimizer_hashes_batch(dcn_ctx *ctx, const uint8_t *bases, const uint64_t *offsets, uint32_t n_reads,
                               uint64_t prefix_length, uint64_t *out_offsets, uint64_t *out_hashes,
                               uint32_t *out_positions, uint64_t capacity);

int dcn_should_keep_hashes(dcn_ctx *ctx, const uint64_t *hashes, const uint64_t *hash_offsets, uint32_t n_units,
                           const dcn_params *params, uint8_t *keep, uint32_t *hits, uint32_t *total);

int dcn_index_set_create(const dcn_index *const *members, uint32_t n, dcn_index **out);
void dcn_index_set_destroy(dcn_index *set);
int dcn_index_set_info(const dcn_index *set, uint32_t *n_members, uint8_t *k, uint8_t *w, uint64_t *n_keys,
                       uint64_t *table_bytes);

int dcn_index_set_select(const dcn_index *set, uint32_t all_of, uint32_t any_of, uint32_t none_of, uint32_t min_members,
                         uint32_t max_members, uint64_t *n_selected, dcn_index **out);
int dcn_index_set_overlap(const dcn_index *set, uint64_t *shared, uint64_t *exclusive, uint64_t *by_count);

int dcn_classify_batch(dcn_ctx *ctx, const dcn_index *set, const uint8_t *bases, const uint64_t *offsets,
                       const uint32_t *unit_id, uint32_t n_reads, const dcn_params *params, uint32_t *match,
                       uint32_t *hits, uint32_t *total);
int dcn_classify_batch_device(dcn_ctx *ctx, const dcn_index *set, const uint8_t *d_bases, const uint64_t *d_offsets,
                              const uint32_t *d_unit_id, uint32_t n_reads, uint64_t n_bases, uint32_t n_units,
                              const dcn_params *params, uint32_t *d_match, uint32_t *d_hits, uint32_t *d_total);

int dcn_index_set_coverage_enable(dcn_index *set, int enable);
int dcn_index_set_coverage_reset(dcn_index *set);
int dcn_index_set_coverage(const dcn_index *set, uint64_t *observed, uint64_t *keys);
int dcn_index_set_coverage_keys(const dcn_index *set, uint32_t member, uint64_t *out, uint64_t capacity, uint64_t *n);

int dcn_index_set_depth_enable(dcn_index *set, int enable);
int dcn_index_set_depth_reset(dcn_index *set);
int dcn_index_set_depth_stats(const dcn_index *set, uint64_t *observed, uint64_t *sum, uint64_t *saturated);
int dcn_index_set_depth_hist(const dcn_index *set, uint32_t member, uint32_t n_bins, uint64_t *hist);
int dcn_index_set_depth_keys(const dcn_index *set, uint32_t member, uint64_t *keys, uint32_t *depths, uint64_t capacity,
                             uint64_t *n);

typedef struct dcn_index_builder dcn_index_builder;
int dcn_index_builder_create(uint8_t k, uint8_t w, float entropy_threshold, uint64_t capacity_keys, int device, void **out);
int dcn_index_builder_add(void *builder, const uint8_t *bases, const uint64_t *offsets, uint32_t n_seqs);
int dcn_index_builder_info(const void *builder, uint64_t *n_keys, uint64_t *n_occurrences, uint64_t *n_bases,
                           uint64_t *device_bytes);
int dcn_index_builder_hist(const void *builder, uint32_t n_bins, uint64_t *hist);
int dcn_index_builder_counts(const void *builder, uint64_t *keys, uint32_t *counts, uint64_t capacity, uint64_t *n);
int dcn_index_builder_finish(const void *builder, uint32_t min_count, uint32_t max_count, uint64_t *n_selected,
                             dcn_index **out);
void dcn_index_builder_destroy(void *builder);

typedef struct dcn_locate_params {
    uint32_t max_gap;
    uint32_t min_hits;
    uint32_t member_mask;
    uint32_t reserved;
    uint64_t prefix_length;
} dcn_locate_params;
typedef struct dcn_segment {
    uint32_t start, end, n_hits, members;
} dcn_segment;

int dcn_locate_batch(dcn_ctx *ctx, const dcn_index *index, const uint8_t *bases, const uint64_t *offsets,
                     uint32_t n_reads, const void *params, uint64_t *seg_offsets, void *segs, uint64_t capacity);

typedef struct dcn_track_params {
    uint32_t bin_bases;
    uint32_t member_mask;
    uint32_t depth_cap;
    uint32_t reserved;
    uint64_t prefix_length;
} dcn_track_params;
typedef struct dcn_track_bin {
    uint32_t n_positions, n_keys, n_observed, max_depth;
    uint64_t sum_depth;
} dcn_track_bin;

int dcn_depth_track_batch(dcn_ctx *ctx, const dcn_index *set, const uint8_t *bases, const uint64_t *offsets,
                          uint32_t n_reads, const void *params, uint64_t *bin_offsets, void *bins, uint64_t capacity);

int dcn_anchor_map_create(const dcn_index *index, dcn_index **out);
int dcn_anchor_map_add(dcn_index *map, dcn_ctx *ctx, const uint8_t *bases, const uint64_t *offsets,
                       uint32_t n_records, uint32_t *first_record);
int dcn_anchor_map_info(const dcn_index *map, uint32_t *n_records, uint64_t *n_keys, uint64_t *n_anchors,
                        uint64_t *n_repeats);
int dcn_anchor_map_anchors(const dcn_index *map, uint64_t *keys, uint32_t *records, uint32_t *positions,
                           uint64_t capacity, uint64_t *n);

typedef struct dcn_place_params {
    uint32_t band_bases;
    uint32_t min_votes;
    uint64_t prefix_length;
    uint32_t reserved[2];
} dcn_place_params;
typedef struct dcn_placement {
    uint32_t record;
    uint32_t reverse;
    uint32_t votes, n_anchors, n_positions;
    uint32_t read_start, read_end;
    uint32_t reserved;
    uint64_t ref_start, ref_end;
} dcn_placement;

int dcn_place_batch(dcn_ctx *ctx, const dcn_index *map, const uint8_t *bases, const uint64_t *offsets,
                    uint32_t n_reads, const void *params, void *placements);

#define DCN_PLACE_SPLIT_MAX 8
typedef struct dcn_place_split_params {
    uint32_t band_bases, min_votes;
    uint64_t prefix_length;
    uint32_t max_placements;
    uint32_t reserved[3];
} dcn_place_split_params;
typedef struct dcn_split_placement {
    uint32_t record;
    uint32_t reverse;
    uint32_t votes, n_anchors, n_positions;
    uint32_t read_start, read_end;
    uint32_t reserved;
    uint64_t ref_start, ref_end;
    uint32_t rank, n_placed, rival_votes, mapq;
} dcn_split_placement;

int dcn_place_split_batch(dcn_ctx *ctx, const dcn_index *map, const uint8_t *bases, const uint64_t *offsets,
                          uint32_t n_reads, const void *params, uint64_t *place_offsets, void *placements,
                          uint64_t capacity, uint32_t *read_counts);

#define DCN_PAIR_HIST_BINS 256
#define DCN_PAIR_PROPER 1u
#define DCN_PAIR_RESCUED 2u
#define DCN_PAIR_MATE_PLACED 4u
typedef struct dcn_place_pair_params {
    uint32_t band_bases, min_votes;
    uint64_t prefix_length;
    uint32_t max_placements;
    uint32_t max_insert;
    uint32_t hist_bin_bases;
    uint32_t reserved[3];
} dcn_place_pair_params;
typedef struct dcn_pair_placement {
    uint32_t record;
    uint32_t reverse;
    uint32_t votes, n_anchors, n_positions;
    uint32_t read_start, read_end;
    uint32_t reserved;
    uint64_t ref_start, ref_end;
    uint32_t rank, n_placed, rival_votes, mapq;
    uint32_t flags;
    uint32_t pair_votes;
    int64_t tlen;
} dcn_pair_placement;

int dcn_place_pair_batch(dcn_ctx *ctx, const dcn_index *map, const uint8_t *bases, const uint64_t *offsets,
                         uint32_t n_reads, const void *params, void *rows, uint64_t *tlen_hist);


int dcn_ctx_stats(dcn_ctx *ctx, uint64_t counters[DCN_N_STATS]);
int dcn_ctx_reset_stats(dcn_ctx *ctx);

int dcn_stats_allreduce(dcn_ctx *const *ctxs, int n_ctx, uint64_t counters[DCN_N_STATS]);

#define DCN_COMM_ID_BYTES 128
typedef struct dcn_comm dcn_comm;
int dcn_comm_available(void);
int dcn_comm_unique_id(uint8_t id[DCN_COMM_ID_BYTES]);
int dcn_comm_create(const uint8_t id[DCN_COMM_ID_BYTES], int world_size, int rank, int device, dcn_comm **out);
int dcn_stats_allreduce_rccl(dcn_comm *comm, dcn_ctx *const *ctxs, int n_ctx, uint64_t counters[DCN_N_STATS]);
void dcn_comm_destroy(dcn_comm *comm);


enum {
    DCN_STAGE_PACK = 0,
    DCN_STAGE_PLAN = 1,
    DCN_STAGE_SCAN = 2,
    DCN_STAGE_DISTINCT = 3,
    DCN_STAGE_FINISH = 4,
    DCN_N_STAGES = 5
};

int dcn_ctx_set_profiling(dcn_ctx *ctx, int enable);

int dcn_ctx_profile(dcn_ctx *ctx, double stage_ms[DCN_N_STAGES], uint64_t *n_batches);

#ifdef __cplusplus
}
#endif
#endif
```

Measured before the change: 399,000.

## Retire long-read units early in scan once distinct hit threshold is reached

```diff
diff --git a/deacon-server_amd/_native.py b/deacon-server_amd/_native.py
--- a/deacon-server_amd/_native.py
+++ b/deacon-server_amd/_native.py
@@ -205,6 +205,7 @@
     "dcn_should_keep_hashes": (C.c_int, [_vp, _vp, _vp, C.c_uint32, C.POINTER(Params), _vp, _vp, _vp]),
     "dcn_ctx_stats": (C.c_int, [_vp, _u64p]),
     "dcn_ctx_reset_stats": (C.c_int, [_vp]),
+    "dcn_ctx_retired_units": (C.c_int, [_vp, _u64p]),
     "dcn_ctx_set_profiling": (C.c_int, [_vp, C.c_int]),
     "dcn_ctx_profile": (C.c_int, [_vp, C.POINTER(C.c_double), _u64p]),
     "dcn_index_set_create": (C.c_int, [C.POINTER(_vp), C.c_uint32, C.POINTER(_vp)]),
@@ -244,7 +245,7 @@
 }
 
 _lib = None
-ABI = (1, 11)
+ABI = (1, 12)
 
 
 def lib():
diff --git a/deacon-server_amd/csrc/ctx.hip b/deacon-server_amd/csrc/ctx.hip
--- a/deacon-server_amd/csrc/ctx.hip
+++ b/deacon-server_amd/csrc/ctx.hip
@@ -62,7 +62,7 @@
     void *dev[] = {c->d_ascii, c->d_offsets, c->d_unit_id, c->d_packed, c->d_invmask,
                    c->d_read_tiles, c->d_read_tile_first, c->d_unit_first_read, c->d_unit_tile_first, c->d_unit_tile_count, c->d_tiles,
                    c->d_keep, c->d_unit_state, c->d_hits, c->d_total, c->d_unit_scratch, c->d_caps,
-                   c->d_set_off, c->d_tile_hits, c->d_pending, c->d_big, c->d_rec_hash, c->d_set_slots, c->d_status, c->d_report, c->d_dump_hash,
+                   c->d_set_off, c->d_tile_hits, c->d_pending, c->d_big, c->d_rec_hash, c->d_set_slots, c->d_status, c->d_report, c->d_retired, c->d_dump_hash,
                    c->d_dump_pos, c->d_dump_count, c->d_dump_valid, c->d_tile_read_pos,
                    c->d_cls_big, c->d_cls_n_big, c->d_cls_match, c->d_cls_hits, c->d_cls_total,
                    c->d_loc_bits, c->d_loc_labels, c->d_loc_counts, c->d_loc_big, c->d_loc_n_big, c->d_loc_block_sums,
@@ -227,6 +227,9 @@
         }
         sa.early_out_max_items = lo;
         sa.early_out_pairs = no_early_out_pairs ? 0u : 1u;
+        static const bool no_early_retire = getenv("DCN_NO_EARLY_RETIRE") != nullptr;
+        sa.early_retire = no_early_retire ? 0u : 1u;
+        sa.retired = c->d_retired;
     }
     sa.keep = v.d_keep;
     sa.hits = v.d_hits;
@@ -707,6 +710,7 @@
     A(d_rec_hash, (max_batch_bases >> c->rec_shift) + 256, "rec_hash");
     A(d_status, 1, "status");
     A(d_report, 1, "report");
+    A(d_retired, 1, "retired");
 #undef A
     }
     uint64_t recs = std::min<uint64_t>(std::max<uint64_t>(max_batch_bases / 16, 1u << 16), 1ull << 29);
@@ -725,6 +729,7 @@
         hipMemset(c->d_status, 0, sizeof(dcn_status)) != hipSuccess ||
         hipMemset(c->d_unit_scratch, 0, (uint64_t)max_batch_reads * 4 * sizeof(uint32_t)) != hipSuccess ||
         hipMemset(c->d_report, 0, sizeof(dcn_batch_report)) != hipSuccess ||
+        hipMemset(c->d_retired, 0, sizeof(unsigned long long)) != hipSuccess ||
         hipDeviceSynchronize() != hipSuccess)
         return fail(dcn_fail(DCN_ERR_HIP, "hipMemset failed"));
     note_ctx_device(c->device, +1);
@@ -816,6 +821,16 @@
     return DCN_OK;
 }
 
+extern "C" int dcn_ctx_retired_units(dcn_ctx *ctx, uint64_t *n_units) {
+    if (!ctx || !n_units) return dcn_fail(DCN_ERR_ARG, "ctx/n_units is NULL");
+    DCN_HIP(hipSetDevice(ctx->device));
+    DCN_HIP(hipStreamSynchronize(ctx->stream));
+    unsigned long long v = 0;
+    DCN_HIP(hipMemcpy(&v, ctx->d_retired, sizeof(v), hipMemcpyDeviceToHost));
+    *n_units = v;
+    return DCN_OK;
+}
+
 extern "C" int dcn_ctx_reset_stats(dcn_ctx *ctx) {
     if (!ctx) return dcn_fail(DCN_ERR_ARG, "ctx is NULL");
     DCN_HIP(hipSetDevice(ctx->device));
diff --git a/deacon-server_amd/csrc/dcn_ctx.h b/deacon-server_amd/csrc/dcn_ctx.h
--- a/deacon-server_amd/csrc/dcn_ctx.h
+++ b/deacon-server_amd/csrc/dcn_ctx.h
@@ -79,6 +79,7 @@
     uint32_t *d_unit_first_read = nullptr, *d_unit_tile_first = nullptr, *d_unit_tile_count = nullptr;
     dcn_tile *d_tiles = nullptr;
     uint8_t *d_keep = nullptr, *d_unit_state = nullptr;
+    unsigned long long *d_retired = nullptr;
     uint32_t *d_hits = nullptr, *d_total = nullptr;
     uint32_t *d_unit_scratch = nullptr;
     bool scratch_dirty = false;
diff --git a/deacon-server_amd/csrc/dcn_internal.h b/deacon-server_amd/csrc/dcn_internal.h
--- a/deacon-server_amd/csrc/dcn_internal.h
+++ b/deacon-server_amd/csrc/dcn_internal.h
@@ -146,6 +146,8 @@
     uint32_t deplete;
     uint32_t early_out_max_items;
     uint32_t early_out_pairs;
+    uint32_t early_retire;
+    unsigned long long *retired;
     uint8_t *keep;
     uint32_t *hits, *total;
     uint8_t *unit_state;
diff --git a/deacon-server_amd/csrc/plan.hip b/deacon-server_amd/csrc/plan.hip
--- a/deacon-server_amd/csrc/plan.hip
+++ b/deacon-server_amd/csrc/plan.hip
@@ -193,6 +193,10 @@
     for (uint32_t i = blockIdx.x; i < NP; i += gridDim.x) {
         const uint32_t u = nu, first = nfirst, count = ncount, H = nH, tot = ntot;
         fetch(i + gridDim.x);
+        if (a.unit_state[u] == 3) {
+            if (lane == 0) a.caps[u] = 0;
+            continue;
+        }
         if (H == 0) {
             if (lane == 0) a.caps[u] = 0;
             continue;
@@ -413,6 +417,12 @@
             bool keep;
             if (state[q]) {
                 keep = kept[q] != 0;
+                if (state[q] == 3) {
+                    a.g_total[u] = 0;
+                    a.g_hitcnt[u] = 0;
+                    a.g_distinct[u] = 0;
+                    a.g_zero[u] = 0;
+                }
             } else {
                 uint32_t tot = a.g_total[u], hc = a.g_distinct[u] + (a.g_zero[u] ? 1u : 0u);
                 a.g_total[u] = 0;
diff --git a/deacon-server_amd/csrc/scan.hip b/deacon-server_amd/csrc/scan.hip
--- a/deacon-server_amd/csrc/scan.hip
+++ b/deacon-server_amd/csrc/scan.hip
@@ -2,6 +2,7 @@
 #include "dcn_probe.h"
 
 #include <atomic>
+#include <type_traits>
 
 namespace {
 
@@ -88,6 +89,17 @@
     uint8_t local[DCN_WAVE];
     uint8_t lok[DCN_WAVE];
 };
+constexpr int DCN_RT_SLOTS = 4;
+struct WaveSharedRetire : WaveShared {
+    uint32_t rt_out[DCN_RT_SLOTS];
+    uint32_t rt_rem[DCN_RT_SLOTS];
+    uint32_t rt_dist[DCN_RT_SLOTS];
+    uint32_t rt_need[DCN_RT_SLOTS];
+    uint32_t rt_dec[DCN_RT_SLOTS];
+    uint32_t rt_slots;
+    uint32_t rt_live;
+};
+static_assert(sizeof(WaveSharedRetire) <= 10240, "sixteen one-wave workgroups per CU: 160 KB of LDS / 16");
 
 #ifndef DCN_EXP
 #define DCN_EXP 0
@@ -123,7 +135,8 @@
 template <int W, bool K128, bool DUMP, bool FAST, bool VAR = false>
 __global__ __launch_bounds__(DCN_WAVE, FAST ? DCN_MIN_WAVES_FAST : DCN_MIN_WAVES) void scan_kernel(dcn_scan_args a) {
     static_assert(!VAR || (W == 0 && !FAST), "the variant path is the generic-w counting / dump kernel");
-    __shared__ WaveShared sh;
+    constexpr bool RETIRE = FAST && !DUMP;
+    __shared__ std::conditional_t<RETIRE, WaveSharedRetire, WaveShared> sh;
     extern __shared__ __align__(16) uint2 dyn_ring[];
 
     const int lane = threadIdx.x;
@@ -153,6 +166,7 @@
     sh.lok[lane] = 0;
     sh.uhits[lane] = 0;
     sh.ucap[lane] = 0;
+    uint32_t unit_tiles = 0;
     if (head) {
         sh.unit_of[uslot] = t.unit;
         sh.run_base[uslot] = (t.scan_start + carry) >> a.rec_shift;
@@ -163,9 +177,22 @@
             } else {
                 uint32_t first = a.unit_tile_first[t.unit], count = a.unit_tile_count[t.unit];
                 loc = count != 0xFFFFFFFFu && first >= wave_first && first + count <= wave_first + DCN_WAVE;
+                unit_tiles = loc ? 0u : count;
             }
         }
         sh.local[uslot] = loc ? 1 : 0;
+    }
+    if constexpr (RETIRE) {
+        const uint32_t n_slots = (uint32_t)__popcll(head_mask);
+        sh.rt_slots = (a.early_retire && n_slots <= (uint32_t)DCN_RT_SLOTS) ? n_slots : 0u;
+        sh.rt_live = (a.early_retire && n_slots <= (uint32_t)DCN_RT_SLOTS) ? n_slots : 1u;
+        if (lane < DCN_RT_SLOTS) {
+            sh.rt_out[lane] = 0;
+            sh.rt_rem[lane] = 0;
+            sh.rt_dist[lane] = 0;
+            sh.rt_need[lane] = 0xFFFFFFFFu;
+            sh.rt_dec[lane] = 0;
+        }
     }
     const uint32_t ROT = VAR ? a.nt_rot : 1u;
     const uint32_t ROTR = (32u - ROT) & 31u;
@@ -184,8 +211,18 @@
         const uint64_t first_win = (uint64_t)__shfl((long long)(t.scan_start + carry), head_lane, 64);
         const uint32_t slack = t.n_windows() < a.tile_windows ? l - 1 : 0u;
         if (have_tile && t.n_windows()) atomicMax(&sh.ucap[uslot], (uint32_t)(t.scan_start + carry + t.n_windows() + slack - first_win));
+        if constexpr (RETIRE) {
+            if (uslot < (uint32_t)DCN_RT_SLOTS && t.n_windows()) atomicAdd(&sh.rt_out[uslot], t.n_windows());
+        }
         __syncthreads();
         if (head) sh.ucap[uslot] = (uint32_t)(((first_win + sh.ucap[uslot]) >> a.rec_shift) - (first_win >> a.rec_shift));
+        if constexpr (RETIRE) {
+            if (uslot < (uint32_t)DCN_RT_SLOTS && head) {
+                const uint64_t all = (uint64_t)unit_tiles * a.tile_windows, here = sh.rt_out[uslot];
+                sh.rt_out[uslot] = unit_tiles == 0xFFFFFFFFu ? 0xFFFFFFFFu
+                                                             : (uint32_t)min(all > here ? all - here : 0ull, 0xFFFFFFFEull);
+            }
+        }
         __syncthreads();
     }
 
@@ -218,14 +255,29 @@
     const uint32_t nk = nwc ? nwc + w - 1 : 0;
     const uint32_t jmax = wave_max_u32(nk);
 
-    auto flush = [&](auto u_tag, bool final_flush) {
+    auto flush = [&](auto u_tag, bool final_flush, const uint32_t jdone) {
         constexpr int U = decltype(u_tag)::value;
 #ifdef DCN_PHASEB_PRIO
         __builtin_amdgcn_s_setprio(DCN_PHASEB_PRIO);
 #endif
         const uint32_t skip0 = (first_pending && cnt > 0) ? 1u : 0u;
         const uint32_t us_skip = uslot | (skip0 << 8);
-        const uint32_t cnt_eff = cnt - skip0;
+        bool trk = false;
+        bool lane_dec = false;
+        if constexpr (RETIRE) {
+            if (sh.rt_slots != 0 && (go_global || !final_flush)) {
+                trk = true;
+                lane_dec = (sh.rt_dec[uslot & 3u] & 1u) != 0;
+                if (!go_global) {
+#pragma unroll
+                    for (int q = 0; q < DCN_RCAP / DCN_WAVE; ++q) sh.ring_hash[q * DCN_WAVE + lane] = 0;
+                }
+                const uint32_t done_w = jdone > w - 1 ? jdone - (w - 1) : 0u;
+                const uint32_t rem = nwc - min(nwc, done_w);
+                if (rem) atomicAdd(&sh.rt_rem[uslot], rem);
+            }
+        }
+        const uint32_t cnt_eff = lane_dec ? 0u : cnt - skip0;
         uint32_t incl = wave_inclusive_scan_u32(cnt_eff, lane);
         uint32_t M = wave_last_u32(incl);
         sh.start[lane] = (uint16_t)(incl - cnt_eff);
@@ -238,6 +290,22 @@
             sh.lok[uslot] = ok ? 1 : 0;
         }
         __syncthreads();
+        if constexpr (RETIRE) {
+            if (trk) {
+                const uint32_t n_slots = sh.rt_slots;
+                if ((uint32_t)lane < n_slots) {
+                    const uint32_t seg_log2 = n_slots == 1 ? 8u : (n_slots == 2 ? 7u : 6u), cap34 = 3u << (seg_log2 - 2);
+                    const uint32_t in_wave = sh.items[lane] + sh.rt_rem[lane], out_ = sh.rt_out[lane];
+                    const uint32_t total_ub = in_wave + out_ < out_ ? 0xFFFFFFFFu : in_wave + out_;
+                    const uint64_t need_ub = dcn_required_hits(a.abs_threshold, a.rel_threshold, total_ub);
+                    const bool tracked = need_ub <= cap34 && need_ub < total_ub;
+                    sh.rt_need[lane] = tracked ? ((uint32_t)need_ub | (seg_log2 << 16)) : 0xFFFFFFFFu;
+                    if (tracked && sh.rt_dist[lane] >= (uint32_t)need_ub && !(atomicOr(&sh.rt_dec[lane], 1u) & 1u))
+                        atomicSub(&sh.rt_live, 1u);
+                }
+                __syncthreads();
+            }
+        }
         constexpr int NPW = K128 ? 5 : 3;
         constexpr int NMW = K128 ? 3 : 2;
         constexpr bool PIPE = DCN_PIPE_B && U == 1;
@@ -272,6 +340,9 @@
             it.rel = sh.DCN_LIST_AT(l_, it.idx + o_skip);
             const long long o_s = __shfl((long long)s, l_, 64);
             it.o_uslot = o_pk & 0xFFu;
+            if constexpr (RETIRE) {
+                if (trk) it.act = it.act && !(*(volatile uint32_t *)&sh.rt_dec[it.o_uslot & 3u] & 1u);
+            }
             it.p = (uint64_t)(o_s + it.rel);
 #ifdef DCN_DEBUG_BOUNDS
             if (it.act && it.p + k > a.stream_bases) {
@@ -344,6 +415,9 @@
                 rel[u] = sh.DCN_LIST_AT(lo[u], idx[u] + o_skip);
                 long long o_s = __shfl((long long)s, lo[u], 64);
                 o_uslot[u] = o_pk & 0xFFu;
+                if constexpr (RETIRE) {
+                    if (trk) act[u] = act[u] && !(*(volatile uint32_t *)&sh.rt_dec[o_uslot[u] & 3u] & 1u);
+                }
                 p[u] = (uint64_t)(o_s + rel[u]);
 #ifdef DCN_DEBUG_BOUNDS
                 if (act[u] && p[u] + k > a.stream_bases) {
@@ -438,6 +512,33 @@
                     }
                 } else if (act[u]) {
                     atomicSub(&sh.total[o_uslot[u]], 1u);
+                }
+            }
+            if constexpr (RETIRE) {
+                if (trk) {
+#pragma unroll
+                    for (int u = 0; u < U; ++u) {
+                        const uint32_t us = o_uslot[u] & 3u;
+                        const uint32_t nd = hit[u] ? *(volatile uint32_t *)&sh.rt_need[us] : 0xFFFFFFFFu;
+                        if (__any(nd != 0xFFFFFFFFu)) {
+                            const uint32_t seg_log2 = (nd >> 16) & 15u, seg_mask = (1u << seg_log2) - 1u;
+                            unsigned long long *const seg = reinterpret_cast<unsigned long long *>(&sh.ring_hash[us << seg_log2]);
+                            uint32_t sl = (uint32_t)(hash[u] >> 40);
+                            uint32_t left = nd != 0xFFFFFFFFu && hash[u] != 0 ? seg_mask + 1u : 0u;
+                            bool fresh = false;
+                            while (left) {
+                                const unsigned long long old = atomicCAS(&seg[sl & seg_mask], 0ull, (unsigned long long)hash[u]);
+                                fresh = old == 0ull;
+                                left = (fresh || old == (unsigned long long)hash[u]) ? 0u : left - 1u;
+                                ++sl;
+                            }
+                            if (nd != 0xFFFFFFFFu && hash[u] == 0) fresh = !(atomicOr(&sh.rt_dec[us], 2u) & 2u);
+                            bool decided = false;
+                            if (fresh) decided = atomicAdd(&sh.rt_dist[us], 1u) + 1u >= (nd & 0xFFFFu);
+                            if (decided) decided = !(atomicOr(&sh.rt_dec[us], 1u) & 1u);
+                            if (decided) atomicSub(&sh.rt_live, 1u);
+                        }
+                    }
                 }
             }
 #pragma unroll
@@ -536,6 +637,9 @@
         emitted_before += cnt_eff;
         if (skip0) first_pending = false;
         cnt = 0;
+        if constexpr (RETIRE) {
+            if (trk && lane < DCN_RT_SLOTS) sh.rt_rem[lane] = 0;
+        }
         __syncthreads();
 #ifdef DCN_PHASEB_PRIO
         __builtin_amdgcn_s_setprio(0);
@@ -704,10 +808,15 @@
 
     if (jmax > 0) {
         block(BoolTag<true>{}, 0);
-        if (__any(cnt > DCN_LCAP - STEP)) flush(IntTag<1>{}, false);
+        if (__any(cnt > DCN_LCAP - STEP)) flush(IntTag<1>{}, false, STEP);
         for (uint32_t jb = STEP; jb < jmax; jb += STEP) {
             block(BoolTag<false>{}, jb);
-            if (__any(cnt > DCN_LCAP - STEP)) flush(IntTag<1>{}, false);
+            if (__any(cnt > DCN_LCAP - STEP)) {
+                flush(IntTag<1>{}, false, jb + STEP);
+                if constexpr (RETIRE) {
+                    if (__builtin_amdgcn_readfirstlane((int)sh.rt_live) == 0) break;
+                }
+            }
         }
     }
     if (FAST && !DUMP && !go_global) {
@@ -836,31 +945,43 @@
             return;
         }
     }
-    flush(IntTag<DCN_U_FINAL>{}, true);
+    flush(IntTag<DCN_U_FINAL>{}, true, 0xFFFFFFFFu);
     if (DUMP) {
         if (have_tile) a.dump_count[tile_idx] = emitted_before;
         return;
     }
 
-    if (any_rec && lane == 0) a.status->any_records = 1;
+    const dcn_scan_args *ap = &a;
+    if constexpr (RETIRE) {
+#if defined(__HIP_DEVICE_COMPILE__)
+        ap = (const dcn_scan_args *)__builtin_amdgcn_kernarg_segment_ptr();
+        asm volatile("" : "+s"(ap));
+#endif
+    }
+    const dcn_scan_args &ae = *ap;
+    bool lane_dec = false;
+    if constexpr (RETIRE) {
+        lane_dec = (sh.rt_dec[uslot & 3u] & 1u) != 0 && sh.rt_slots != 0;
+    }
+    if (any_rec && lane == 0) ae.status->any_records = 1;
     {
-        const bool pending = have_tile && !sh.lok[uslot] && !(DCN_EXP & 1024);
+        const bool pending = have_tile && !sh.lok[uslot] && !lane_dec && !(DCN_EXP & 1024);
         bool enrol = false;
         if (pending) {
             const uint32_t th = head ? sh.uhits[uslot] : 0u;
-            a.tile_hits[tile_idx] = th;
-            if (th) enrol = atomicAdd(&a.g_hitcnt[t.unit], th) == 0u;
+            ae.tile_hits[tile_idx] = th;
+            if (th) enrol = atomicAdd(&ae.g_hitcnt[t.unit], th) == 0u;
         }
         const unsigned long long em = __ballot(enrol);
         if (em) {
             uint32_t base = 0;
-            if (lane == 0) base = atomicAdd(&a.status->n_pending, (uint32_t)__popcll(em));
+            if (lane == 0) base = atomicAdd(&ae.status->n_pending, (uint32_t)__popcll(em));
             base = __shfl(base, 0, 64);
             if (enrol) {
-                a.pending[base + (uint32_t)__popcll(em & ((1ull << lane) - 1))] = t.unit;
+                ae.pending[base + (uint32_t)__popcll(em & ((1ull << lane) - 1))] = t.unit;
                 if (t.whole_unit()) {
-                    a.unit_tile_first[t.unit] = tile_idx;
-                    a.unit_tile_count[t.unit] = 1;
+                    ae.unit_tile_first[t.unit] = tile_idx;
+                    ae.unit_tile_count[t.unit] = 1;
                 }
             }
         }
@@ -868,15 +989,22 @@
 
     if (head && have_tile) {
         uint32_t tot = sh.total[uslot];
-        if (sh.lok[uslot]) {
+        if (lane_dec) {
+            ae.keep[t.unit] = ae.deplete ? 0 : 1;
+            ae.unit_state[t.unit] = 3;
+        } else if (sh.lok[uslot]) {
             uint32_t hc = sh.hits[uslot];
-            a.keep[t.unit] = dcn_decide(hc, tot, a.abs_threshold, a.rel_threshold, a.deplete) ? 1 : 0;
-            if (a.hits) a.hits[t.unit] = hc;
-            if (a.total) a.total[t.unit] = tot;
-            a.unit_state[t.unit] = 1;
+            ae.keep[t.unit] = dcn_decide(hc, tot, ae.abs_threshold, ae.rel_threshold, ae.deplete) ? 1 : 0;
+            if (ae.hits) ae.hits[t.unit] = hc;
+            if (ae.total) ae.total[t.unit] = tot;
+            ae.unit_state[t.unit] = 1;
         } else if (tot) {
-            atomicAdd(&a.g_total[t.unit], tot);
-        }
+            atomicAdd(&ae.g_total[t.unit], tot);
+        }
+    }
+    if constexpr (RETIRE) {
+        const unsigned long long rm = __ballot(head && have_tile && lane_dec);
+        if (rm && lane == 0 && ae.retired) atomicAdd(ae.retired, (unsigned long long)__popcll(rm));
     }
 }
 
diff --git a/deacon-server_amd/filter.py b/deacon-server_amd/filter.py
--- a/deacon-server_amd/filter.py
+++ b/deacon-server_amd/filter.py
@@ -765,6 +765,11 @@
     def reserve_records(self, n_records):
         N.check(N.lib().dcn_ctx_reserve_records(self._h, int(n_records)))
 
+    def retired_units(self):
+        n = C.c_uint64()
+        N.check(N.lib().dcn_ctx_retired_units(self._h, C.byref(n)))
+        return int(n.value)
+
     def should_keep_sequence(self, seq):
         keep, hits, total = self.filter_reads([seq])
         return bool(keep[0]), int(hits[0]), int(total[0])
diff --git a/include/deacon_hip.h b/include/deacon_hip.h
--- a/include/deacon_hip.h
+++ b/include/deacon_hip.h
@@ -39,7 +39,7 @@
 };
 
 #define DCN_ABI_MAJOR 1
-#define DCN_ABI_MINOR 11
+#define DCN_ABI_MINOR 12
 int dcn_abi_version(uint32_t *major, uint32_t *minor);
 const char *dcn_version(void);
 const char *dcn_last_error(void);
@@ -274,6 +274,7 @@
 
 int dcn_ctx_stats(dcn_ctx *ctx, uint64_t counters[DCN_N_STATS]);
 int dcn_ctx_reset_stats(dcn_ctx *ctx);
+int dcn_ctx_retired_units(dcn_ctx *ctx, uint64_t *n_units);
 
 int dcn_stats_allreduce(dcn_ctx *const *ctxs, int n_ctx, uint64_t counters[DCN_N_STATS]);
 
diff --git a/profiles/long_decisions_rate.py b/profiles/long_decisions_rate.py
--- /dev/null
+++ b/profiles/long_decisions_rate.py
@@ -0,0 +1,60 @@
+#!/usr/bin/env python3
+import statistics
+import sys
+import time
+
+import torch
+
+sys.path.insert(0, ".")
+import bench as B
+import deacon_server_amd as dcn
+
+REPS, STEPS = 5, 4
+reads = int(sys.argv[1]) if len(sys.argv) > 1 else 10_000_000
+dev = torch.device("cuda", 0)
+genome = B.make_host_genome(64_000_000, 3, dev)
+index, keys, _, _, build_s = B.build_index(genome, B.PANHUMAN_KEYS, 0)
+del keys
+print(f"index: {index.n_keys:,} keys, built in {build_s:.1f} s; {reads * B.READ_LEN / 1e6:.0f} Mbp per batch", flush=True)
+
+for frac in (0.0, 0.5, 0.95):
+    bases, offsets = B.make_long_reads(genome, reads * B.READ_LEN, 11, dev, host_frac=frac)
+    b = B.Batch(bases, offsets)
+    proc = dcn.FilterProcessor(index, abs_threshold=2, rel_threshold=0.01, deplete=True, max_batch_bases=b.n_bases,
+                               max_batch_reads=b.n_reads)
+    proc.reserve_records(b.n_bases // 6)
+    retired_units = getattr(proc, "retired_units", lambda: 0)
+
+    def run(counts, steps):
+        for _ in range(steps):
+            proc.filter_batch_device(b.d_bases.data_ptr(), b.d_offsets.data_ptr(), b.n_reads, b.n_bases,
+                                     (b.d_keep if counts else b.d_keep2).data_ptr(), b.d_hits.data_ptr() if counts else None,
+                                     b.d_total.data_ptr() if counts else None)
+        proc.synchronize()
+
+    run(True, 2)
+    run(False, 2)
+    ms = {True: [], False: []}
+    r0 = retired_units()
+    for _ in range(REPS):
+        for counts in (True, False):
+            t0 = time.perf_counter()
+            run(counts, STEPS)
+            ms[counts].append((time.perf_counter() - t0) / STEPS * 1e3)
+    retired = (retired_units() - r0) / (REPS * STEPS)
+    scan = {}
+    for counts in (True, False):
+        proc.set_profiling(2)
+        run(counts, STEPS)
+        stage, nb = proc.profile()
+        proc.set_profiling(False)
+        scan[counts] = stage["scan"] / max(nb, 1)
+    same = bool(torch.equal(b.d_keep, b.d_keep2))
+    for counts, name in ((True, "counting"), (False, "decisions_only")):
+        v = ms[counts]
+        print(f"host {frac:4.2f}  {name:15s} ms/step min {min(v):6.3f} median {statistics.median(v):6.3f} max {max(v):6.3f}  "
+              f"{b.n_bases / statistics.median(v) / 1e3:9.0f} Mbp/s  scan {scan[counts]:6.3f} ms", flush=True)
+    print(f"host {frac:4.2f}  {b.n_reads:,} reads, kept {float(b.d_keep.float().mean()):.3f}, retired per step {retired:,.0f}, "
+          f"decisions identical: {same}", flush=True)
+    proc.close()
+    del b, bases, offsets
```

Result: slower. 383,400 (-3.9%).
